# UT-Austin-RPL/FORGE

Measured on AMD Instinct MI355X. Metric: rendered views/sec (5 views, 128^2 px, 64^3 voxel), higher is better.
Workload: dtype f32; 1 GPU; BASELINE configs[1]: FORGE hot path, 1 scene(s)/GPU x 5 input views 256^2 -> 32^3x128 feature grid -> 64^3 render grid -> 5 views x 128^2 rays x 64 samples -> 5 RGB 256^2; HIP rotate, fp32-MFMA implicit-GEMM ResNet-50 trunk / conv1 / ConvGRU (Winograd F(2x2,3x3) x 3 depth taps) / heads / conv_rgb, HIP ray-march (no MIOpen/rocBLAS kernel in the step); eval BN, random-init seeded weights; scenes_per_gpu=1, views_in=5, views_out=5, feature_grid=32, render_grid=64, steps_in_flight=4, launch=hipGraph replay, 4 steps in flight on 4 HIP streams, parallelism=dp1 (scene-sharded, no data-path collective; 4-scalar RCC...

## Files before the change

### forge_amd/convops.py

```python
import collections
import ctypes
import functools
import os
from fractions import Fraction

import torch

from . import _lib, determinism

EPI_BIAS, EPI_AFFINE_ACT, EPI_GRU_GATES, EPI_GRU_OUT = 0, 1, 2, 3


_TAPS_CACHE = {}


def _taps_array(taps):
    key = tuple(tuple(t) for t in taps)
    arr = _TAPS_CACHE.get(key)
    if arr is None:
        flat = [int(v) for t in key for v in t]
        arr = _TAPS_CACHE[key] = (ctypes.c_int * len(flat))(*flat)
    return arr


# ... 23 lines not shown
    out = []
    for pz in ((0, 1) if nd == 3 else (0,)):
        for py in (0, 1):
            for px in (0, 1):
                taps, mats = [], []
                for dz, kz in (per_axis[pz] if nd == 3 else [(0, None)]):
                    for dy, ky in per_axis[py]:
                        for dx, kx in per_axis[px]:
                            taps.append((dz, dy, dx))
                            mats.append((wd[:, :, kz, ky, kx] if nd == 3 else wd[:, :, ky, kx]).t())
                out.append(((pz, py, px), taps, torch.stack(mats).contiguous()))
    return out


def convT_phases_merged(w, pad, nd):
    ph = convT_phases(w, pad, nd)
    taps = [t for _, tp, _ in ph for t in tp]
    return taps, torch.cat([wp for _, _, wp in ph], dim=0).contiguous()


def convT3d_k4s2p1_phases(w):
    return convT_phases(w, 1, 3)


def pack_conv2d_weight(w):
    co, ci, kh, kw = w.shape
    taps = [(0, ky - kh // 2, kx - kw // 2) for ky in range(kh) for kx in range(kw)]
    return w.detach().reshape(co, ci, kh * kw).permute(2, 0, 1).contiguous(), taps


def bn_affine(bn):
    scale = bn.weight.detach() / torch.sqrt(bn.running_var.detach() + bn.eps)
    shift = bn.bias.detach() - bn.running_mean.detach() * scale
    return scale.contiguous(), shift.contiguous()


class PackCache:

    def __init__(self):
        self._key = None
        self.val = None

    def clear(self):
        self._key = None
        self.val = None

    def key_of(self, sources):
        return tuple((t.data_ptr(), t._version, str(t.device)) for t in sources)

    def get(self, sources, build):
        key = self.key_of(sources)
        if key != self._key:
            self.val = build()
            self._key = key
        return self.val


class PackedModule(torch.nn.Module):

    def __init__(self):
        super().__init__()
        self.register_load_state_dict_post_hook(lambda module, incompatible_keys: module.invalidate_packed())

    def invalidate_packed(self):
        for v in self.__dict__.values():
            if isinstance(v, PackCache):
                v.clear()

    def train(self, mode=True):
        self.invalidate_packed()
        return super().train(mode)

    def _apply(self, fn, *args, **kwargs):
        self.invalidate_packed()
        return super()._apply(fn, *args, **kwargs)


def invalidate_packed(module):
    for m in module.modules():
        if isinstance(m, PackedModule):
            m.invalidate_packed()


class _ZeroArena:

    def __init__(self):
        self.task, self.device = -1, None
        self.pools = {}
        self.want = {}

    def _end(self):
        self.want = {k: p[2] for k, p in self.pools.items()}
        self.pools, self.task = {}, -1

    HAVE_HOOKS = hasattr(torch._C, "_current_graph_task_id") and hasattr(getattr(torch.autograd.Variable, "_execution_engine", None), "queue_callback")

    def zeros(self, shape, device):
        n = 1
        for d in shape:
            n *= int(d)
        nbytes = (n * 4 + 255) // 256 * 256
        if not self.HAVE_HOOKS:
            return torch.zeros(shape, dtype=torch.float32, device=device)
        task = torch._C._current_graph_task_id()
        if task < 0:
            return torch.zeros(shape, dtype=torch.float32, device=device)
        if task != self.task:
            if self.task >= 0:
                self._end()
            self.task, self.device = task, device
            torch.autograd.Variable._execution_engine.queue_callback(self._end_of(task))
        if device != self.device:
            return torch.zeros(shape, dtype=torch.float32, device=device)
        key = torch.cuda.current_stream(device).cuda_stream if torch.device(device).type == "cuda" else 0
        pool = self.pools.get(key)
        if pool is None:
            want = self.want.get(key, 0)
            pool = self.pools[key] = [torch.zeros(want // 4 + 64, dtype=torch.float32, device=device) if want else None, 0, 0]
        pool[2] += nbytes
        if pool[0] is None or pool[1] + nbytes > pool[0].numel() * 4:
            return torch.zeros(shape, dtype=torch.float32, device=device)
        out = pool[0][pool[1] // 4:pool[1] // 4 + n].view(shape)
        pool[1] += nbytes
        return out

    def _end_of(self, task):
        def cb():
            if self.task == task:
                self._end()
        return cb


GRAD_ZEROS = _ZeroArena()


def grad_zeros(shape, device, scratch=False):
    if scratch:
        return torch.zeros(tuple(shape), dtype=torch.float32, device=device)
    return GRAD_ZEROS.zeros(tuple(shape), device)


SPLITK_WS_BYTES = 128 << 20

TILE_NAMES = {"A": "128, 128, 8, 1", "B": "64, 128, 8, 1", "C": "128, 64, 8, 1", "D": "64, 64, 4, 1", "E": "128, 32, 4, 1"}

_PLAN_CACHE = {}


class _State:
    plan_override = None
    winograd = True
    wino_depth_nest = os.environ.get("FORGE_WINO_DEPTH_NEST", "1") != "0"
    wino_depth_nest4 = os.environ.get("FORGE_WINO_DEPTH_NEST4", "1") != "0"
    wino_h4 = os.environ.get("FORGE_WINO_H4", "1") != "0"
    conv_fast_epilogue = os.environ.get("FORGE_CONV_FAST_EPILOGUE", "1") != "0"


STATE = _State()


class force_plan:

    def __init__(self, tile=None, ksplit=None):
        self.val = (tile, ksplit)

    def __enter__(self):
        self.prev = STATE.plan_override
        STATE.plan_override = self.val
        return self

    def __exit__(self, *exc):
        STATE.plan_override = self.prev
        return False


_pushed_fast_epilogue = None


def _conv_lib():
    global _pushed_fast_epilogue
    L = _lib.lib()
    want = bool(STATE.conv_fast_epilogue)
    if want is not _pushed_fast_epilogue:
        L.forge_conv_fast_epilogue(int(want))
        _pushed_fast_epilogue = want
    return L


def conv_epilogue_is_direct(M, Cout, ldo, ldr=0, residual=False, ostride=1, same_grid=True, nphase=1, lift=0, ksplit=1, stats=False, epilogue=EPI_BIAS):
    fast = ctypes.c_int(0)
    _lib.check(_conv_lib().forge_conv_igemm_epilogue(int(M), int(Cout), int(ldo), int(ldr), int(bool(residual)), int(ostride), int(bool(same_grid)),
                                                     int(nphase), int(lift), int(ksplit), int(bool(stats)), int(epilogue), ctypes.byref(fast)),
               "forge_conv_igemm_epilogue")
    return bool(fast.value)


def conv_plan(M, Cout, Cin, ntaps, epilogue, ldo, nphase=1):
    key = (int(M), int(Cout), int(Cin), int(ntaps), int(nphase), int(epilogue), int(ldo) % 4 == 0)
    pl = _PLAN_CACHE.get(key)
    if pl is None:
        tile, ks = ctypes.c_int(0), ctypes.c_int(0)
        _lib.check(_lib.lib().forge_conv_igemm_plan(int(M), int(Cout), int(Cin), int(ntaps), int(nphase), int(epilogue), int(ldo), SPLITK_WS_BYTES,
                                                    ctypes.byref(tile), ctypes.byref(ks)), "forge_conv_igemm_plan")
        pl = _PLAN_CACHE[key] = (chr(tile.value), ks.value)
    ov = STATE.plan_override
    if ov is not None and pl[0] != "N":
        tile = ov[0] or pl[0]
        ks = ov[1] if ov[1] is not None else (pl[1] if ov[0] is None else 1)
        can_split = nphase == 1 and epilogue in (EPI_BIAS, EPI_AFFINE_ACT) and Cout % 4 == 0 and ldo % 4 == 0
        if ks > 1 and not (can_split and ks * M * Cout * 4 <= SPLITK_WS_BYTES and ks <= (ntaps // nphase) * (Cin // 32)):
            ks = 1
        return tile, ks
    return pl


MAX_OPERAND_BYTES = (1 << 31) - 1


@_lib.on_tensor_device
def conv_igemm(in1, C1, ld1, in2, C2, ld2, wp, bias, scale, shift, slope, residual, aux_h, aux_z, out, out2,
               grid, in_grid, Cout, ldo, taps, out_grid=None, istride=1, ostride=1, phase=(0, 0, 0), epilogue=EPI_BIAS,
               bs1=0, bs2=0, lift=0, out3=None, stats=None):
    n, D, H, W = grid
    Di, Hi, Wi = in_grid
    Do, Ho, Wo = out_grid if out_grid is not None else (D, H, W)
    if wp.shape != (len(taps), Cout, C1 + C2):
        raise ValueError("packed weight %s does not match taps=%d Cout=%d Cin=%d" % (tuple(wp.shape), len(taps), Cout, C1 + C2))
    in_rows, out_rows = Di * Hi * Wi, Do * Ho * Wo
    b1, b2 = (int(bs1) or in_rows), (int(bs2) or in_rows)
    span = lambda k, br, ld: ((k - 1) * br + in_rows) * ld * 4
    limit = MAX_OPERAND_BYTES
    nc = n
    while nc > 1 and (span(nc, b1, ld1) > limit or (in2 is not None and span(nc, b2, ld2) > limit)):
        nc = (nc + 1) // 2
    L, st, arr = _conv_lib(), _lib.current_stream(), _taps_array(taps)
    nphase = 1
    if tuple(phase) == (-1, -1, -1):
        nphase = 8 if Do == 2 * D else 4

    def off(t, floats):
        return None if t is None else ctypes.c_void_p(t.data_ptr() + 4 * floats)
    gate_w = Cout // 2 if epilogue == EPI_GRU_GATES else Cout
    for s0 in range(0, n, nc):
        k = min(nc, n - s0)
        orow = s0 * out_rows
        tile, ksplit = conv_plan(k * D * H * W, Cout, C1 + C2, len(taps), epilogue, ldo, nphase)
        if stats is not None and (ksplit > 1 or nc < n):
            raise RuntimeError("forge_amd: conv_igemm output statistics need an un-chunked launch without split-K (use conv_stats_buffer)")
        ws = torch.empty(ksplit * k * D * H * W * Cout, dtype=torch.float32, device=out.device) if ksplit > 1 else None
        o_ld = gate_w if epilogue == EPI_GRU_GATES else ldo
        _lib.check(L.forge_conv_igemm(
            off(in1, s0 * b1 * ld1), C1, ld1, int(bs1), off(in2, s0 * b2 * ld2), C2, ld2, int(bs2), _lib.ptr(wp), _lib.ptr(bias), _lib.ptr(scale),
            _lib.ptr(shift), float(slope), off(residual, orow * (Cout if (lift or epilogue in (EPI_GRU_GATES, EPI_GRU_OUT)) else ldo)),
            off(aux_h, orow * gate_w), off(aux_z, orow * Cout),
            off(out, orow * (Cout if lift else o_ld)), off(out2, orow * o_ld), off(out3, orow * o_ld), k, D, H, W, istride, Di, Hi, Wi, Cout, ldo,
            arr, len(taps), ostride, phase[0], phase[1], phase[2], Do, Ho, Wo, epilogue, int(lift), 0 if tile == "N" else ord(tile), ksplit,
            _lib.ptr(ws), 0 if ws is None else ws.numel() * 4, _lib.ptr(stats), st),
            "forge_conv_igemm")
    return out


TILE_BM = {"A": 128, "B": 64, "C": 128, "D": 64, "E": 128}


def stats_blocks(M, tile):
    bm = TILE_BM[tile]
    return ((int(M) + bm - 1) // bm) * (bm // 32)


def conv_stats_buffer(x1, in2, grid, in_grid, Cout, Cin, ntaps, ldo, device):
    n, D, H, W = grid
    M = n * D * H * W
    if Cout <= 16 or Cout % 4:
        return None
    tile, ksplit = conv_plan(M, Cout, Cin, ntaps, EPI_BIAS, ldo, 1)
    if ksplit > 1 or tile == "N":
        return None
    Di, Hi, Wi = in_grid
    if ((n - 1) * (Di * Hi * Wi) + Di * Hi * Wi) * max(x1.shape[-1], 0 if in2 is None else in2.shape[-1]) * 4 > MAX_OPERAND_BYTES:
        return None
    return torch.empty(stats_blocks(M, tile), 2, Cout, dtype=torch.float64, device=device)


def wino_pack_packed(wp, transpose=False):
    return wino_pack(WINO_FORMS["points"], wp, transpose)


def wino_pack_weight(w):
    return wino_pack_packed(pack_conv3d_weight(w))


def wino_conv_rows(x1, x2, U, bias, out, residual=None, V1=None):
    n, D, H, W, C1 = x1.shape
    return _wino_conv(x1, C1, _batch_stride_rows(x1), x2, 0 if x2 is None else x2.shape[-1], 0 if x2 is None else _batch_stride_rows(x2), U, bias, out,
                      residual, (n, D, H, W), V1=V1)


def _wino_conv(x1, C1, bs1, x2, C2, bs2, U, bias, out, residual, grid, V1=None):
    n, D, H, W = grid
    Cout = U.shape[2]
    if V1 is None:
        V1 = wino_input(x1, C1, C1, n, D, H, W, bs=bs1)
    V2 = None if x2 is None else wino_input(x2, C2, C2, n, D, H, W, bs=bs2)
    Mm = wino_gemm(V1, C1, V2, C2, U, None, n, D, H // 2, W // 2, Cout)
    return wino_output(Mm, bias, None, None, 1.0, residual, None, None, out, None, None, n, D, H, W, Cout, Cout, EPI_BIAS)


_ONE_ZERO = {}


def _one_zero(device, C):
    key = (str(device), C)
    v = _ONE_ZERO.get(key)
    if v is None:
        v = _ONE_ZERO[key] = (torch.ones(C, device=device), torch.zeros(C, device=device))
    return v


def conv3_launch(x1, C1, x2, C2, wp, bias, out, grid, Cout, bs1=0, residual=None, dgrad=False, U=None, wT=None):
    n, D, H, W = grid
    if wino_applies(TAPS_3x3x3, 1, n, D, H, W, C1, C2, Cout):
        return _wino_conv(x1, C1, bs1, x2, C2, 0, U if U is not None else wino_pack_packed(wp, transpose=dgrad), bias, out, residual, grid)
    w = (wT if wT is not None else wp.transpose(1, 2).contiguous()) if dgrad else wp
    taps = [(-a, -b, -c) for a, b, c in TAPS_3x3x3] if dgrad else TAPS_3x3x3
    if residual is None:
        return conv_igemm(x1, C1, C1, x2, C2, C2, w, bias, None, None, 1.0, None, None, None, out, None, grid, (D, H, W), Cout, Cout, taps,
                          epilogue=EPI_BIAS, bs1=bs1)
    one, zero = _one_zero(out.device, Cout)
    return conv_igemm(x1, C1, C1, x2, C2, C2, w, bias, one, zero, 1.0, residual, None, None, out, None, grid, (D, H, W), Cout, Cout, taps,
                      epilogue=EPI_AFFINE_ACT, bs1=bs1)


def wino_wgrad_applies(n, D, H, W, C1, C2, Cout, taps=None):
    return (wino_applies(TAPS_3x3x3 if taps is None else taps, 1, n, D, H, W, C1, C2, Cout) and C1 + C2 >= 128 and Cout >= 64 and (C2 == 0 or C1 % 128 == 0)
            and n * D * (H // 2) * (W // 2) * Cout * 4 <= MAX_OPERAND_BYTES)


@_lib.on_tensor_device
def conv3_wgrad(dy, x1, C1, x2, C2, dwp, grid, Cout, bs1=0, taps=None, dM=None):
    n, D, H, W = grid
    taps = TAPS_3x3x3 if taps is None else list(taps)
    if not wino_wgrad_applies(n, D, H, W, C1, C2, Cout, taps):
        return conv_wgrad(dy, x1, C1, x2, C2, dwp, grid, (D, H, W), Cout, taps, bs1=bs1)
    kd = len(taps) // 9
    L, st = _lib.lib(), _lib.current_stream()
    Ht, Wt = H // 2, W // 2
    R = n * D * Ht * Wt
    dev = dy.device
    V1 = wino_input(x1, C1, C1, n, D, H, W, bs=bs1)
    V2 = None if x2 is None else wino_input(x2, C2, C2, n, D, H, W)
    if dM is None:
        dM = torch.empty(16, R, Cout, dtype=torch.float32, device=dev)
        _lib.check(L.forge_wino_dy(_lib.ptr(dy), dy.shape[-1], _lib.ptr(dM), n, D, H, W, Cout, st), "forge_wino_dy")
    dU = grad_zeros((16, kd, Cout, C1 + C2), dev, scratch=True)
    determinism.launch("forge_wino_wgrad", (_lib.ptr(dM), _lib.ptr(V1), C1, 0, 0, _lib.ptr(V2), C2, 0, 0, _lib.ptr(dU), n, D, Ht, Wt, Cout, kd),
                       (C1, C2, n, D, Ht, Wt, Cout, kd), dev)
    _lib.check(L.forge_wino_dw(_lib.ptr(dU), _lib.ptr(dwp), Cout, C1 + C2, kd, st), "forge_wino_dw")
    return dwp


def wino_applies(taps, istride, n, D, H, W, C1, C2, Cout):
    tt = tuple(tuple(t) for t in taps)
    if not (wino_enabled() and istride == 1 and C1 % 32 == 0 and C2 % 32 == 0 and Cout % 8 == 0 and wino_fits(n, D, H, W, max(C1, C2, 1))):
        return False
    if len(tt) == 27 and tt == tuple(TAPS_3x3x3):
        return C1 + C2 >= 64 and Cout >= 32
    if len(tt) == 9 and tt == tuple(TAPS_3x3) and D == 1:
        return C2 == 0 and C1 >= WINO2D_MIN_C and Cout >= WINO2D_MIN_C
    return False


def wino_enabled():
    return STATE.winograd


class winograd:

    def __init__(self, on):
        self.on = bool(on)

    def __enter__(self):
        self.prev = STATE.winograd
        STATE.winograd = self.on
        return self

    def __exit__(self, *exc):
        STATE.winograd = self.prev
        return False


def wino_scene_chunk(b, D, H, W, C, views=1):
    nb = b
    while nb >= 1 and not wino_fits(nb, D, H, W, C, views=views):
        nb = (nb + 1) // 2 if nb > 1 else 0
    return nb


def wino_fits(n, D, H, W, C, views=1, nest4=False, form=None):
    form = form or WINO_FORMS["dn4" if nest4 else "points"]
    rows = n * views * D * (H // form.th) * (W // 2) * form.rows
    return H % form.th == 0 and W % 2 == 0 and rows * C * 4 <= MAX_OPERAND_BYTES


@_lib.on_tensor_device
def wino_input_dy(dy, C, n, D, H, W):
    R = n * D * (H // 2) * (W // 2)
    V = torch.empty(16, R, C, dtype=torch.float32, device=dy.device)
    dM = torch.empty(16, R, C, dtype=torch.float32, device=dy.device)
    _lib.check(_lib.lib().forge_wino_input_dy(_lib.ptr(dy), C, _lib.ptr(V), _lib.ptr(dM), n, D, H, W, C, _lib.current_stream()), "forge_wino_input_dy")
    return V, dM


def wino_half_applies(R, Cout, Cin):
    return STATE.plan_override is None and wino_gemm_tile(R, Cout, Cin) == "B"


def wino_depth_nest_applies(R, D, Ht, Wt, Cout, Cin):
    return (STATE.wino_depth_nest and STATE.plan_override is None and D % 2 == 0 and (Ht * Wt) % 64 == 0 and Cin % 32 == 0
            and R * Cout * 4 <= MAX_OPERAND_BYTES and wino_gemm_tile(R, Cout, Cin) == "B")


def wino_depth_nest4_applies(R, D, Ht, Wt, Cout, Cin):
    return STATE.wino_depth_nest4 and D % 4 == 0 and D >= 8 and wino_depth_nest_applies(R, D, Ht, Wt, Cout, Cin)


def wino_depth_nest4h_applies(R, D, Ht, Wt, Cout, Cin):
    return STATE.wino_h4 and wino_depth_nest4_applies(R, D, Ht, Wt, Cout, Cin)


WinoForm = collections.namedtuple("WinoForm", "name P gemm weights ushape input rows kloops applies tile metered points th", defaults=(16, 2))
_U4 = lambda kd, co_, ci_: (16, kd, co_, ci_)
WINO_FORMS = {f.name: f for f in (
    WinoForm("points", 16, "forge_wino_gemm", "forge_wino_weights", _U4, "forge_wino_input", 1, None, lambda R, D, Ht, Wt, Cout, Cin: True,
             True, True),
    WinoForm("half", 8, "forge_wino_gemm_half", "forge_wino_weights", _U4, "forge_wino_input", 1, None,
             lambda R, D, Ht, Wt, Cout, Cin: wino_half_applies(R, Cout, Cin), False, True),
    WinoForm("dn", 16, "forge_wino_gemm_dn", "forge_wino_weights_dn", lambda kd, co_, ci_: (16, 2, 2, co_, ci_), "forge_wino_input", 1, 2,
             lambda *a: wino_depth_nest_applies(*a), False, True),
    WinoForm("dn4", 16, "forge_wino_gemm_dn4", "forge_wino_weights_dn4", lambda kd, co_, ci_: (16, 6, co_, ci_), "forge_wino_input_dn4", Fraction(3, 2),
             Fraction(3, 2), lambda *a: wino_depth_nest4_applies(*a), False, False),
)}

WINO_DN4H = WinoForm("dn4h", 24, "forge_wino_gemm_dn4h", "forge_wino_weights_dn4h", lambda kd, co_, ci_: (24, 6, co_, ci_), "forge_wino_input_dn4h",
                     Fraction(3, 2), Fraction(3, 2), lambda *a: wino_depth_nest4h_applies(*a), False, False, 24, 4)


def wino_calls(form):
    if not form.metered:
        return functools.partial(wino_form_input, form), functools.partial(wino_form_gemm, form)
    return (lambda *a, **kw: wino_input(*a, **kw)), (lambda *a, **kw: wino_gemm(*a, **kw))


@_lib.on_tensor_device
def wino_pack(form, wp, transpose=False):
    T, co_, ci_ = wp.shape
    nest = form.kloops is not None
    assert T == 27 or (T == 9 and not nest)
    assert not (nest and transpose)
    kd = T // 9
    wp = wp.detach()
    wp = wp if wp.is_contiguous() else wp.contiguous()
    U = torch.empty(form.ushape(kd, ci_, co_) if transpose else form.ushape(kd, co_, ci_), dtype=torch.float32, device=wp.device)
    own = () if nest else (kd, 1 if transpose else 0)
    _lib.check(getattr(_lib.lib(), form.weights)(_lib.ptr(wp), _lib.ptr(U), co_, ci_, *own, _lib.current_stream()), form.weights)
    return U


@_lib.on_tensor_device
def wino_form_input(form, x, C, ld, n, D, H, W, bs=0, out=None, nsum=1, sum_stride=0):
    rows = int(n * D * (H // form.th) * (W // 2) * form.rows)
    V = out if out is not None else torch.empty(form.points, rows, C, dtype=torch.float32, device=x.device)
    if form.rows != 1 and (V.shape != (form.points, rows, C) or not V.is_contiguous()):
        raise ValueError("depth-nest operand buffer %s is not [%d][%d][%d]" % (tuple(V.shape), form.points, rows, C))
    _lib.check(getattr(_lib.lib(), form.input)(_lib.ptr(x), ld, int(bs), _lib.ptr(V), C, 0, n, D, H, W, C, int(nsum), int(sum_stride), _lib.current_stream()),
               form.input)
    return V


def wino_input(x, C, ld, n, D, H, W, bs=0, out=None, nsum=1, sum_stride=0):
    return wino_form_input(WINO_FORMS["points"], x, C, ld, n, D, H, W, bs=bs, out=out, nsum=nsum, sum_stride=sum_stride)


def _point_products(Mm, P, R, Cout, device):
    if Mm is None:
        Mm = torch.empty(P, R, Cout, dtype=torch.float32, device=device)
    if not (Mm.is_contiguous() and Mm.dtype == torch.float32 and Mm.numel() >= P * R * Cout):
        raise ValueError("point-product buffer %s %s%s cannot hold %d x %d x %d float32" % (
            tuple(Mm.shape), Mm.dtype, "" if Mm.is_contiguous() else " (not contiguous)", P, R, Cout))
    if Mm.shape != (P, R, Cout):
        Mm = Mm.as_strided((P, R, Cout), (R * Cout, Cout, 1))
    return Mm


@_lib.on_tensor_device
def wino_form_gemm(form, V1, C1, V2, C2, U, Mm, n, D, Ht, Wt, Cout, view=0, views=1):
    R = n * D * Ht * Wt
    vol = int(D * Ht * Wt * form.rows)
    nest = form.kloops is not None
    kd = 3 if nest else U.shape[1]
    if U.shape != form.ushape(kd, Cout, C1 + C2) or (kd not in (1, 3)) or (nest and not U.is_contiguous()):
        raise ValueError("%s weight %s does not match Cout=%d Cin=%d" % ("depth-nest" if nest else "transformed", tuple(U.shape), Cout, C1 + C2))
    if form.rows != 1 and (V1.shape[1] != n * views * vol or (V2 is not None and V2.shape[1] != n * vol)):
        raise ValueError("depth-nest operands %s / %s are not %s's %d (x %d views) rows per point" % (
            tuple(V1.shape), None if V2 is None else tuple(V2.shape), form.input, n * vol, views))
    Mm = _point_products(Mm, form.P, R, Cout, V1.device)
    tile = (ord(wino_gemm_tile(R, Cout, C1 + C2)),) if form.tile else ()
    p1 = ctypes.c_void_p(V1.data_ptr() + 4 * view * vol * C1)
    _lib.check(getattr(_conv_lib(), form.gemm)(p1, C1, C1, views * vol if views > 1 else 0, V1.shape[1] * C1, _lib.ptr(V2), C2, C2, 0,
                                               0 if V2 is None else V2.shape[1] * C2, _lib.ptr(U), _lib.ptr(Mm), n, D, Ht, Wt, Cout, kd,
                                               *tile, _lib.current_stream()), form.gemm)
    return Mm


def wino_gemm(V1, C1, V2, C2, U, Mm, n, D, Ht, Wt, Cout, view=0, views=1, half=None):
    if U.dim() == 5:
        form = "dn"
    else:
        if half is None:
            half = WINO_FORMS["half"].applies(n * D * Ht * Wt, D, Ht, Wt, Cout, C1 + C2)
        form = "half" if half else "points"
    return wino_form_gemm(WINO_FORMS[form], V1, C1, V2, C2, U, Mm, n, D, Ht, Wt, Cout, view=view, views=views)


def wino_gemm_tile(R, Cout, Cin):
    ov = STATE.plan_override
    if ov is not None and ov[0]:
        return ov[0]
    return chr(_lib.lib().forge_wino_gemm_tile(int(R), int(Cout), int(Cin)))


@_lib.on_tensor_device
def wino_output(Mm, bias, scale, shift, slope, residual, aux_h, aux_z, out, out2, out3, n, D, H, W, Cout, ldo, epilogue, Mm2=None, view=0, views=1):
    P = Mm.shape[0] if Mm.dim() == 3 else 0
    vol = D * (H // (WINO_DN4H.th if P == WINO_DN4H.P else 2)) * (W // 2)
    if P not in (8, 16, WINO_DN4H.P) or Mm.shape[1:] != (n * vol, Cout) or not Mm.is_contiguous():
        raise ValueError("point products %s do not match [8 | 16][%d][%d] (or the 24 points' rows)" % (tuple(Mm.shape), n * vol, Cout))
    if P == WINO_DN4H.P:
        if Mm2 is not None or residual is not None or H % 4 or epilogue not in (EPI_GRU_GATES, EPI_GRU_OUT):
            raise ValueError("24-point products take the GRU tails only, without a second addend or a residual, on H %% 4 == 0 (H=%d epilogue=%d)" % (H, epilogue))
        _lib.check(_lib.lib().forge_wino_output_dn4h(_lib.ptr(Mm), _lib.ptr(bias), _lib.ptr(scale), _lib.ptr(shift), _lib.ptr(aux_h), _lib.ptr(aux_z),
                                                     _lib.ptr(out), _lib.ptr(out2), _lib.ptr(out3), n, D, H, W, Cout, ldo, epilogue, _lib.current_stream()),
                   "forge_wino_output_dn4h")
        return out
    if Mm2 is not None and (Mm2.shape != (P, n * views * vol, Cout) or not Mm2.is_contiguous()):
        raise ValueError("second addend %s does not match [%d][%d][%d] (the form of Mm)" % (tuple(Mm2.shape), P, n * views * vol, Cout))
    p2 = None if Mm2 is None else ctypes.c_void_p(Mm2.data_ptr() + 4 * view * vol * Cout)
    fn, name = (_lib.lib().forge_wino_output_half, "forge_wino_output_half") if P == 8 else (_lib.lib().forge_wino_output, "forge_wino_output")
    _lib.check(fn(_lib.ptr(Mm), p2, views * vol, 0 if Mm2 is None else Mm2.shape[1] * Cout, _lib.ptr(bias), _lib.ptr(scale), _lib.ptr(shift), float(slope),
                  _lib.ptr(residual), _lib.ptr(aux_h), _lib.ptr(aux_z), _lib.ptr(out), _lib.ptr(out2), _lib.ptr(out3), n, D, H, W, Cout, ldo, epilogue,
                  _lib.current_stream()), name)
    return out


@_lib.on_tensor_device
def conv_wgrad(dy, x1, C1, x2, C2, dwp, grid, in_grid, Cout, taps, istride=1, bs1=0, bs2=0):
    if x2 is not None and C1 % 128:
        x1 = torch.cat([x1[..., :C1], x2[..., :C2]], dim=-1)
        C1, x2, C2, bs1, bs2 = C1 + C2, None, 0, 0, 0
    n, D, H, W = grid
    Di, Hi, Wi = in_grid
    in_rows, out_rows = Di * Hi * Wi, D * H * W
    ldy, ld1, ld2 = dy.shape[-1], x1.shape[-1], (0 if x2 is None else x2.shape[-1])
    b1, b2 = (int(bs1) or in_rows), (int(bs2) or in_rows)
    span = lambda k, br, ld, rows: ((k - 1) * br + rows) * ld * 4
    nc = n
    while nc > 1 and (span(nc, out_rows, ldy, out_rows) > MAX_OPERAND_BYTES or span(nc, b1, ld1, in_rows) > MAX_OPERAND_BYTES
                      or (x2 is not None and span(nc, b2, ld2, in_rows) > MAX_OPERAND_BYTES)):
        nc = (nc + 1) // 2
    off = lambda t, floats: None if t is None else ctypes.c_void_p(t.data_ptr() + 4 * floats)
    ta = _taps_array(taps)
    for s0 in range(0, n, nc):
        k = min(nc, n - s0)
        determinism.launch("forge_conv_wgrad", (off(dy, s0 * out_rows * ldy), ldy, off(x1, s0 * b1 * ld1), C1, ld1, int(bs1), off(x2, s0 * b2 * ld2), C2, ld2,
                                                int(bs2), _lib.ptr(dwp), k, D, H, W, istride, Di, Hi, Wi, Cout, ta, len(taps)),
                           (C1, C2, k, D, H, W, istride, Di, Hi, Wi, Cout, ta, len(taps)), dwp.device)
    return dwp


def _batch_stride_rows(x):
    n, D, H, W, C = x.shape
    if x.stride()[1:] != (H * W * C, W * C, C, 1):
        raise ValueError("conv_rows needs channels-last rows [n,D,H,W,C] dense within a batch element; got strides %s" % (x.stride(),))
    return 0 if (n == 1 or x.stride(0) == D * H * W * C) else x.stride(0) // C


@_lib.on_tensor_device
def colsum(x):
    C = x.shape[-1]
    rows = x.reshape(-1, C)
    if not (rows.is_cuda and rows.dtype == torch.float32):
        raise RuntimeError("forge_amd: colsum runs only on the MI355X HIP kernels (float32 cuda tensor); got %s on %s" % (rows.dtype, rows.device))
    if C % 4:
        if C > 32:
            raise RuntimeError("forge_amd: colsum needs C %% 4 == 0 or C <= 32 (got %d)" % C)
        rows = rows if rows.is_contiguous() else rows.contiguous()
    else:
        rows = rows if (rows.stride(1) == 1 and rows.stride(0) >= C and rows.stride(0) % 4 == 0) else rows.contiguous()
    out = torch.empty(C, dtype=torch.float32, device=rows.device)
    ws = torch.empty(_lib.lib().forge_bn_ws_doubles(C), dtype=torch.float64, device=rows.device)
    _lib.check(_lib.lib().forge_colsum(_lib.ptr(rows), rows.stride(0), _lib.ptr(out), _lib.ptr(ws), rows.shape[0], C, _lib.current_stream()), "forge_colsum")
    return out


class _ConvTapsRows(torch.autograd.Function):

    @staticmethod
    def forward(ctx, x1, x2, wp, bias, taps, istride, out_spatial, want_stats=False):
        n, Di, Hi, Wi, C1 = x1.shape
        C2 = 0 if x2 is None else x2.shape[-1]
        T, Cout, Cin = wp.shape
        D, H, W = out_spatial
        wpc = wp.detach().contiguous()
        out = torch.empty(n, D, H, W, Cout, dtype=torch.float32, device=x1.device)
        bs1 = _batch_stride_rows(x1)
        bs2 = 0 if x2 is None else _batch_stride_rows(x2)
        stats = None
        if (D, H, W) == (Di, Hi, Wi) and wino_applies(taps, istride, n, D, H, W, C1, C2, Cout):
            wino_conv_rows(x1, x2, wino_pack_packed(wpc), bias, out)
        else:
            if want_stats and bs1 == 0 and bs2 == 0:
                stats = conv_stats_buffer(x1, x2, (n, D, H, W), (Di, Hi, Wi), Cout, Cin, T, Cout, x1.device)
            conv_igemm(x1, C1, C1, x2, C2, C2, wpc, bias, None, None, 1.0, None, None, None, out, None,
                       (n, D, H, W), (Di, Hi, Wi), Cout, Cout, taps, istride=istride, epilogue=EPI_BIAS, bs1=bs1, bs2=bs2, stats=stats)
        ctx.save_for_backward(x1, x2, wpc)
        ctx.meta = (tuple(taps), istride, (D, H, W), bias is not None)
        if not want_stats:
            return out
        if stats is None:
            stats = torch.empty(0, dtype=torch.float64, device=x1.device)
        ctx.mark_non_differentiable(stats)
        return out, stats

    @staticmethod
    def backward(ctx, dy, _dstats=None):
        x1, x2, wp = ctx.saved_tensors
        taps, istride, (D, H, W), has_bias = ctx.meta
        n, Di, Hi, Wi, C1 = x1.shape
        C2 = 0 if x2 is None else x2.shape[-1]
        T, Cout, Cin = wp.shape
        dy = dy.contiguous()
        dx1 = dx2 = dwp = db = None
        need_dx = ctx.needs_input_grad[0] or ctx.needs_input_grad[1]
        same = (D, H, W) == (Di, Hi, Wi)
        wino_dx = need_dx and istride == 1 and Cout > 16 and same and wino_applies(taps, istride, n, D, H, W, Cout, 0, Cin)
        wino_dw = (ctx.needs_input_grad[2] and same and wino_applies(taps, istride, n, D, H, W, C1, C2, Cout)
                   and (x2 is None or _batch_stride_rows(x2) == 0) and wino_wgrad_applies(n, D, H, W, C1, C2, Cout, taps))
        Vdy = dMdy = None
        if wino_dx and wino_dw:
            Vdy, dMdy = wino_input_dy(dy.reshape(-1, Cout), Cout, n, D, H, W)
        if need_dx:
            wd = wp.transpose(1, 2).contiguous()
            if istride == 1 and Cout <= 16:
                assert (D, H, W) == (Di, Hi, Wi)
                if Cout < 16:
                    dyk = torch.nn.functional.pad(dy, (0, 16 - Cout))
                    wd = torch.nn.functional.pad(wd, (0, 16 - Cout))
                else:
                    dyk = dy
                dx = torch.empty(n, Di, Hi, Wi, Cin, dtype=torch.float32, device=dy.device)
                ntaps_ = [(-a, -b, -c) for a, b, c in taps]
                for j in range(0, Cin, 16):
                    nb = min(16, Cin - j)
                    conv_igemm(dyk, 16, 16, None, 0, 0, wd[:, j:j + nb].contiguous(), None, None, None, 1.0, None, None, None, dx[..., j:], None,
                               (n, D, H, W), (D, H, W), nb, Cin, ntaps_, epilogue=EPI_BIAS)
            elif istride == 1 and (D, H, W) == (Di, Hi, Wi) and wino_applies(taps, istride, n, D, H, W, Cout, 0, Cin):
                dx = torch.empty(n, Di, Hi, Wi, Cin, dtype=torch.float32, device=dy.device)
                wino_conv_rows(dy, None, wino_pack_packed(wp, transpose=True), None, dx, V1=Vdy)
            elif istride == 1:
                assert (D, H, W) == (Di, Hi, Wi)
                dx = torch.empty(n, Di, Hi, Wi, Cin, dtype=torch.float32, device=dy.device)
                conv_igemm(dy, Cout, Cout, None, 0, 0, wd, None, None, None, 1.0, None, None, None, dx, None, (n, D, H, W), (D, H, W), Cin, Cin,
                           [(-a, -b, -c) for a, b, c in taps], epilogue=EPI_BIAS)
            else:
                flat = D == 1 and Di == 1 and all(t[0] == 0 for t in taps)
                assert istride == 2 and Hi == 2 * H and Wi == 2 * W and (flat or Di == 2 * D), (istride, (D, H, W), (Di, Hi, Wi))
                dx = torch.zeros(n, Di, Hi, Wi, Cin, dtype=torch.float32, device=dy.device)
                for ph_z in ((0,) if flat else (0, 1)):
                    for ph_y in (0, 1):
                        for ph_x in (0, 1):
                            sel = [i for i, (tz, ty, tx) in enumerate(taps) if (flat or (tz - ph_z) % 2 == 0) and (ty - ph_y) % 2 == 0 and (tx - ph_x) % 2 == 0]
                            if not sel:
                                continue
                            ptaps = [(0 if flat else (ph_z - taps[i][0]) // 2, (ph_y - taps[i][1]) // 2, (ph_x - taps[i][2]) // 2) for i in sel]
                            conv_igemm(dy, Cout, Cout, None, 0, 0, torch.stack([wd[i] for i in sel]), None, None, None, 1.0, None, None, None, dx, None,
                                       (n, D, H, W), (D, H, W), Cin, Cin, ptaps, out_grid=(Di, Hi, Wi), ostride=2, phase=(ph_z, ph_y, ph_x),
                                       epilogue=EPI_BIAS)
            dx1 = dx[..., :C1] if ctx.needs_input_grad[0] else None
            dx2 = dx[..., C1:] if (x2 is not None and ctx.needs_input_grad[1]) else None
        if ctx.needs_input_grad[2]:
            dwp = grad_zeros(wp.shape, wp.device)
            if (D, H, W) == (Di, Hi, Wi) and wino_applies(taps, istride, n, D, H, W, C1, C2, Cout) and (x2 is None or _batch_stride_rows(x2) == 0):
                conv3_wgrad(dy, x1, C1, x2, C2, dwp, (n, D, H, W), Cout, bs1=_batch_stride_rows(x1), taps=taps, dM=dMdy)
            else:
                conv_wgrad(dy, x1, C1, x2, C2, dwp, (n, D, H, W), (Di, Hi, Wi), Cout, list(taps), istride=istride, bs1=_batch_stride_rows(x1),
                           bs2=0 if x2 is None else _batch_stride_rows(x2))
# ... 239 lines not shown
```

### forge_amd/csrc/conv_igemm.hip

```cpp
#include "common.h"
#include <cmath>
#include <type_traits>

namespace forge {

enum ConvEpilogue : int {
    EPI_BIAS = 0,
    EPI_AFFINE_ACT = 1,
    EPI_GRU_GATES = 2,
    EPI_GRU_OUT = 3,
};

constexpr int MAX_TAPS = 64;

struct ConvArgs {
    const float* in1; const float* in2;
    int C1, C2, ld1, ld2;
    long long bs1r, bs2r;
    long long span1, span2;
    const float* wp;
    const float* bias;
    const float* scale; const float* shift; float slope;
    const float* aux_h; const float* aux_z;
    float* out; float* out2; float* out3;
// ... 1064 lines not shown
        hipLaunchKernelGGL((conv_igemm_kernel<BMv, BNv, NWv>), dim3((unsigned)grid), dim3(NWv * 64), lds, st, a);          \
    } while (0)
    switch (tile) {
        case 'A': FORGE_LAUNCH_CONV(128, 128, 8); break;
        case 'B': FORGE_LAUNCH_CONV(64, 128, 8); break;
        case 'C': FORGE_LAUNCH_CONV(128, 64, 8); break;
        case 'E': FORGE_LAUNCH_CONV(128, 32, 4); break;
        default: FORGE_LAUNCH_CONV(64, 64, 4); break;
    }
#undef FORGE_LAUNCH_CONV
    return 0;
}

}

using namespace forge;

extern "C" int forge_conv_igemm_plan(long long M, int Cout, int Cin, int ntaps, int nphase, int epilogue, int ldo, long long splitk_ws_bytes,
                                     int* tile, int* ksplit) {
    FORGE_REQUIRE(tile && ksplit && M > 0 && Cout > 0 && Cin > 0 && ntaps > 0 && (nphase == 1 || nphase == 4 || nphase == 8) && ntaps % nphase == 0,
                  FORGE_EINVAL, "forge_conv_igemm_plan: bad argument");
    if (Cout <= 16) { *tile = 'N'; *ksplit = 1; return 0; }
    const ConvPlan pl = plan_conv(M * nphase, Cout, Cin, ntaps / nphase,
                                  nphase == 1 && splitk_ws_bytes > 0 && (epilogue == EPI_BIAS || epilogue == EPI_AFFINE_ACT) && Cout % 4 == 0 && ldo % 4 == 0,
                                  splitk_ws_bytes);
    *tile = pl.tile; *ksplit = pl.ksplit;
    return 0;
}

extern "C" int forge_conv_fast_epilogue(int on) {
    const int prev = g_conv_fast_epilogue;
    if (on >= 0) g_conv_fast_epilogue = on != 0;
    return prev;
}

extern "C" int forge_conv_igemm_epilogue(long long M, int Cout, int ldo, int ldr, int has_residual, int os, int same_grid, int nphase, int lift, int ksplit,
                                         int has_stats, int epilogue, int* fast) {
    FORGE_REQUIRE(fast && M > 0 && Cout > 0 && ldo > 0 && os >= 1 && nphase >= 1 && lift >= 0 && ksplit >= 1 && epilogue >= 0 && epilogue <= 3, FORGE_EINVAL,
                  "forge_conv_igemm_epilogue: bad argument");
    *fast = Cout > 16 && g_conv_fast_epilogue &&
            conv_fast_epilogue_applies(M, Cout, ldo, ldr, has_residual != 0, os, same_grid != 0, nphase, lift, ksplit, has_stats != 0, epilogue);
    return 0;
}

extern "C" int forge_conv_igemm(const float* in1, int C1, int ld1, long long bs1, const float* in2, int C2, int ld2, long long bs2,
                                const float* wp,
                                const float* bias, const float* scale, const float* shift, float slope, const float* residual,
                                const float* aux_h, const float* aux_z, float* out, float* out2, float* out3,
                                int n, int D, int H, int W, int is, int Di, int Hi, int Wi, int Cout, int ldo,
                                const int* taps, int ntaps, int os, int pz, int py, int px, int Do, int Ho, int Wo,
                                int epilogue, int lift, int tile, int ksplit, float* splitk_ws, long long splitk_ws_bytes, double* stats,
                                forge_stream_t stream) {
    FORGE_REQUIRE(in1 && wp && out && taps, FORGE_EINVAL, "forge_conv_igemm: null pointer argument");
    FORGE_REQUIRE(stats == nullptr || (epilogue == EPI_BIAS && ksplit <= 1 && Cout > 16 && !(pz < 0) && lift == 0), FORGE_EINVAL,
                  "forge_conv_igemm: output statistics need the plain bias epilogue of the wide kernel without split-K, phases or lift");
    FORGE_REQUIRE(n > 0 && D > 0 && H > 0 && W > 0 && Cout > 0 && ntaps > 0 && ntaps <= MAX_TAPS, FORGE_EINVAL,
                  "forge_conv_igemm: bad dims n=%d D=%d H=%d W=%d Cout=%d ntaps=%d", n, D, H, W, Cout, ntaps);
    const int kstep = Cout <= 16 ? 16 : 32;
    FORGE_REQUIRE(C1 > 0 && C1 % kstep == 0 && C2 >= 0 && C2 % kstep == 0, FORGE_ESHAPE,
                  "forge_conv_igemm: C1=%d / C2=%d must be multiples of the K-step %d (16 for Cout <= 16, else 32)", C1, C2, kstep);
    FORGE_REQUIRE((C2 == 0) == (in2 == nullptr), FORGE_EINVAL, "forge_conv_igemm: in2/C2 mismatch");
    FORGE_REQUIRE(epilogue >= 0 && epilogue <= 3, FORGE_EINVAL, "forge_conv_igemm: unknown epilogue %d", epilogue);
    FORGE_REQUIRE(epilogue != EPI_AFFINE_ACT || (scale && shift), FORGE_EINVAL, "forge_conv_igemm: affine epilogue needs scale/shift");
    FORGE_REQUIRE(epilogue != EPI_GRU_GATES || (aux_h && out2 && Cout % 2 == 0), FORGE_EINVAL, "forge_conv_igemm: GRU gate epilogue needs aux_h, out2");
    FORGE_REQUIRE(epilogue != EPI_GRU_OUT || (aux_h && aux_z), FORGE_EINVAL, "forge_conv_igemm: GRU out epilogue needs aux_h, aux_z");
    FORGE_REQUIRE(os >= 1 && Do > 0 && Ho > 0 && Wo > 0, FORGE_EINVAL, "forge_conv_igemm: bad output mapping");
    FORGE_REQUIRE(is >= 1 && Di > 0 && Hi > 0 && Wi > 0, FORGE_EINVAL, "forge_conv_igemm: bad input mapping");
    FORGE_REQUIRE(lift == 0 || (lift > 0 && epilogue == EPI_AFFINE_ACT && Cout % lift == 0 && D == 1 && os == 1 && Cout > 64), FORGE_EINVAL,
                  "forge_conv_igemm: lift needs the affine epilogue on a 2-D (D=1) conv with Cout %% lift == 0 and Cout > 64");
    FORGE_REQUIRE(ld1 >= C1 && ld1 % 4 == 0 && (C2 == 0 || (ld2 >= C2 && ld2 % 4 == 0)) && ldo >= 1, FORGE_EINVAL,
                  "forge_conv_igemm: row strides must cover the channels and keep 16-byte alignment");
    ConvArgs a;
    a.in1 = in1; a.in2 = in2; a.C1 = C1; a.C2 = C2; a.ld1 = ld1; a.ld2 = ld2;
    a.bs1r = bs1 > 0 ? bs1 : (long long)Di * Hi * Wi; a.bs2r = bs2 > 0 ? bs2 : (long long)Di * Hi * Wi;
    a.span1 = ((long long)(n - 1) * a.bs1r + (long long)Di * Hi * Wi) * ld1 * 4;
    a.span2 = in2 ? ((long long)(n - 1) * a.bs2r + (long long)Di * Hi * Wi) * ld2 * 4 : 0;
    FORGE_REQUIRE(a.span1 < (1ll << 31) && a.span2 < (1ll << 31) && (long long)ntaps * Cout * (C1 + C2) * 4 < (1ll << 31), FORGE_ESHAPE,
                  "forge_conv_igemm: an operand spans >= 2 GiB (32-bit buffer offsets); split the batch");
    a.is = is; a.Di = Di; a.Hi = Hi; a.Wi = Wi; a.residual = residual;
    a.ldr = (lift > 0 || epilogue == EPI_GRU_GATES || epilogue == EPI_GRU_OUT) ? Cout : ldo;
    a.lift = lift; a.ws = nullptr; a.ksplit = 1; a.stats = stats; a.flat_rows = a.fast_epi = 0;
    a.wp = wp; a.bias = bias; a.scale = scale; a.shift = shift; a.slope = slope;
    a.aux_h = aux_h; a.aux_z = aux_z; a.out = out; a.out2 = out2; a.out3 = out3; a.n = n; a.D = D; a.H = H; a.W = W; a.Cout = Cout; a.ldo = ldo;
    a.ntaps = ntaps; a.os = os; a.pz = pz; a.py = py; a.px = px; a.Do = Do; a.Ho = Ho; a.Wo = Wo; a.epi = epilogue;
    a.nphase = 1; a.tpp = ntaps; a.nbat = 1; a.pt1 = a.pt2 = a.ptw = a.pto = 0;
    if (pz < 0) {
        FORGE_REQUIRE(os == 2 && py < 0 && px < 0 && Ho == 2 * H && Wo == 2 * W && (Do == 2 * D || Do == D), FORGE_EINVAL,
                      "forge_conv_igemm: merged phases (pz = py = px = -1) need os = 2 and a doubled output grid");
        a.nphase = Do == 2 * D ? 8 : 4;
        FORGE_REQUIRE(ntaps % a.nphase == 0, FORGE_EINVAL, "forge_conv_igemm: merged phases need ntaps %% %d == 0", a.nphase);
        a.tpp = ntaps / a.nphase;
        a.pz = a.py = a.px = 0;
    }
    for (int k = 0; k < 3 * ntaps; ++k)
        FORGE_REQUIRE(taps[k] >= -128 && taps[k] <= 127, FORGE_EINVAL, "forge_conv_igemm: tap %d component %d = %d outside [-128, 127]", k / 3, k % 3, taps[k]);
    for (int t = 0; t < MAX_TAPS; ++t) {
        for (int k = 0; k < 3; ++k) a.tap[t][k] = (signed char)(t < ntaps ? taps[t * 3 + k] : 0);
        a.tap[t][3] = 0;
    }
    const long long M = (long long)n * D * H * W;
    FORGE_REQUIRE(M < (1ll << 31), FORGE_ESHAPE, "forge_conv_igemm: more than 2^31 GEMM rows; split the batch");
    FORGE_REQUIRE(out3 == nullptr || epilogue == EPI_GRU_GATES || epilogue == EPI_GRU_OUT, FORGE_EINVAL, "forge_conv_igemm: out3 is a GRU-epilogue output");
    hipStream_t st = (hipStream_t)stream;
    if (Cout <= 16) {
        FORGE_REQUIRE(epilogue == EPI_BIAS || epilogue == EPI_AFFINE_ACT, FORGE_EINVAL, "forge_conv_igemm: GRU epilogues need Cout > 16");
        const long long grid = (M + BM16 - 1) / BM16 * a.nphase;
        FORGE_REQUIRE(grid < (1ll << 31), FORGE_ESHAPE, "forge_conv_igemm: grid too large");
        int lines_r = 0;
        if (a.nphase == 1 && is == 1 && os == 1 && lift == 0 && Do == D && Ho == H && Wo == W && Di == D && Hi == H && Wi == W && pz == 0 && py == 0 && px == 0) {
            for (int r = 1; r <= 2 && !lines_r; ++r) {
                const int nt = 2 * r + 1;
                bool ok = ntaps % nt == 0 && W > r;
                for (int t = 0; ok && t < ntaps; ++t)
                    ok = taps[t * 3 + 2] == (t % nt) - r && taps[t * 3] == taps[(t - t % nt) * 3] && taps[t * 3 + 1] == taps[(t - t % nt) * 3 + 1];
                if (ok) lines_r = r;
            }
        }
        if (lines_r == 1) hipLaunchKernelGGL(conv_igemm_n16_lines_kernel<1>, dim3((unsigned)grid), dim3(NTHREADS), 0, st, a);
        else if (lines_r == 2) hipLaunchKernelGGL(conv_igemm_n16_lines_kernel<2>, dim3((unsigned)grid), dim3(NTHREADS), 0, st, a);
        else hipLaunchKernelGGL(conv_igemm_n16_kernel, dim3((unsigned)grid), dim3(NTHREADS), 0, st, a);
    } else {
        const bool can_split = a.nphase == 1 && splitk_ws && (epilogue == EPI_BIAS || epilogue == EPI_AFFINE_ACT) && Cout % 4 == 0 && ldo % 4 == 0;
        ConvPlan pl;
        if (tile == 0) {
            pl = plan_conv(M * a.nphase, Cout, C1 + C2, a.tpp, can_split, splitk_ws_bytes);
        } else {
            pl = ConvPlan{(char)tile, ksplit > 1 ? ksplit : 1};
            FORGE_REQUIRE(tile >= 'A' && tile <= 'E', FORGE_EINVAL, "forge_conv_igemm: tile '%c' is not one of A..E (0 = planned here)", (char)tile);
            FORGE_REQUIRE(pl.ksplit == 1 || (can_split && pl.ksplit <= 8 && (long long)pl.ksplit * M * Cout * 4 <= splitk_ws_bytes &&
                                             pl.ksplit <= a.tpp * ((C1 + C2) / BK)), FORGE_EINVAL,
                          "forge_conv_igemm: ksplit=%d needs epilogue 0/1 without phases, Cout, ldo %% 4 == 0 and a workspace of ksplit M Cout floats", pl.ksplit);
        }
        FORGE_REQUIRE(stats == nullptr || (tile != 0 && pl.ksplit == 1), FORGE_EINVAL,
                      "forge_conv_igemm: output statistics need an explicit tile ('A'..'E' from forge_conv_igemm_plan) and a plan without split-K");
        if (pl.ksplit > 1) { a.ksplit = pl.ksplit; a.ws = splitk_ws; }
        if (int rc = launch_conv_tile(a, pl.tile, st)) return rc;
        if (a.ksplit > 1) {
            const long long total = M * (Cout / 4);
            hipLaunchKernelGGL(conv_splitk_epilogue_kernel, dim3((unsigned)((total + 255) / 256)), dim3(256), 0, st, a);
        }
    }
    FORGE_LAUNCH_CHECK("forge_conv_igemm");
    return 0;
}

extern "C" int forge_wino_gemm_tile(long long R, int Cout, int Cin) {
    (void)Cin;
    if (Cout <= 64) return R < 2048 ? 'D' : 'C';
    return R < 2048 ? 'D' : 'B';
}

static int wino_gemm_impl(const float* V1, int C1, int ld1, long long bs1, long long pt1, const float* V2, int C2, int ld2, long long bs2,
                          long long pt2, const float* U, float* Mm, int n, int D, int Ht, int Wt, int Cout, int kd, int tile, int form, forge_stream_t stream) {
    const bool half = form == 1, dn = form == 2, dn4h = form == 4, dn4 = form == 3 || dn4h;
    const char* const name4 = dn4h ? "forge_wino_gemm_dn4h" : "forge_wino_gemm_dn4";
    FORGE_REQUIRE(tile == 0 || (tile >= 'A' && tile <= 'E'), FORGE_EINVAL, "forge_wino_gemm: tile must be 0 (default rule) or 'A'..'E'");
    FORGE_REQUIRE(V1 && U && Mm && (kd == 1 || kd == 3), FORGE_EINVAL, "forge_wino_gemm: null pointer argument / kd not 1 or 3");
    FORGE_REQUIRE(n > 0 && D > 0 && Ht > 0 && Wt > 0 && Cout > 16, FORGE_EINVAL, "forge_wino_gemm: bad dims n=%d D=%d Ht=%d Wt=%d Cout=%d (Cout > 16)", n,
                  D, Ht, Wt, Cout);
    FORGE_REQUIRE(C1 > 0 && C1 % BK == 0 && C2 >= 0 && C2 % BK == 0 && (C2 == 0) == (V2 == nullptr), FORGE_ESHAPE,
                  "forge_wino_gemm: C1=%d / C2=%d must be multiples of %d, V2 given iff C2 > 0", C1, C2, BK);
    FORGE_REQUIRE(ld1 >= C1 && ld1 % 4 == 0 && (C2 == 0 || (ld2 >= C2 && ld2 % 4 == 0)), FORGE_EINVAL, "forge_wino_gemm: bad row strides");
    FORGE_REQUIRE(!dn || (kd == 3 && D % 2 == 0 && ((long long)Ht * Wt) % 64 == 0), FORGE_EINVAL,
                  "forge_wino_gemm_dn: needs three depth taps, an even D and Ht Wt %% 64 == 0 (kd=%d D=%d Ht=%d Wt=%d)", kd, D, Ht, Wt);
    FORGE_REQUIRE(!dn4 || (kd == 3 && D % 4 == 0 && ((long long)Ht * Wt) % 64 == 0), FORGE_EINVAL,
                  "%s: needs three depth taps, D %% 4 == 0 and Ht Wt %% 64 == 0 (kd=%d D=%d Ht=%d Wt=%d)", name4, kd, D, Ht, Wt);
    FORGE_REQUIRE(!dn4h || D >= 8, FORGE_EINVAL, "forge_wino_gemm_dn4h: D=%d must be at least 8", D);
    ConvArgs a;
    memset(&a, 0, sizeof(a));
    const long long vol = (long long)D * Ht * Wt, R = (long long)n * vol, rows = dn4 ? vol / 4 * 6 : vol, Cin = C1 + C2;
    const int npos = dn4 ? 6 : dn ? 4 : kd;
    a.in1 = V1; a.in2 = V2; a.C1 = C1; a.C2 = C2; a.ld1 = ld1; a.ld2 = ld2; a.bs1r = bs1 > 0 ? bs1 : rows; a.bs2r = bs2 > 0 ? bs2 : rows;
    a.span1 = ((long long)(n - 1) * a.bs1r + rows) * ld1 * 4;
    a.span2 = V2 ? ((long long)(n - 1) * a.bs2r + rows) * ld2 * 4 : 0;
    if (dn4) {
        FORGE_REQUIRE(a.span1 < (1ll << 31) && a.span2 < (1ll << 31) && R * Cout * 4 < (1ll << 31) && 6ll * Cout * Cin * 4 < (1ll << 31), FORGE_EINVAL,
                      "%s: an operand or an output plane spans >= 2 GiB (32-bit buffer offsets); split the batch", name4);
    } else {
        FORGE_REQUIRE(a.span1 < (1ll << 31) && a.span2 < (1ll << 31) && R < (1ll << 31), FORGE_ESHAPE,
                      "forge_wino_gemm: an operand spans >= 2 GiB per Winograd point (32-bit buffer offsets); split the batch");
        FORGE_REQUIRE(!dn || (R * Cout * 4 < (1ll << 31) && 4ll * Cout * Cin * 4 < (1ll << 31)), FORGE_ESHAPE,
                      "forge_wino_gemm_dn: an output plane spans >= 2 GiB (32-bit buffer offsets); split the batch");
    }
    a.wp = U; a.slope = 1.f; a.out = Mm; a.n = n; a.D = D; a.H = Ht; a.W = Wt; a.is = 1; a.Di = D; a.Hi = Ht; a.Wi = Wt;
    a.Cout = Cout; a.ldo = Cout; a.ldr = Cout; a.ntaps = a.tpp = npos; a.os = 1; a.Do = D; a.Ho = Ht; a.Wo = Wt; a.nphase = 1; a.epi = EPI_BIAS;
    a.ksplit = 1; a.nbat = half ? 4 : dn4h ? 24 : 16;
    a.pt1 = pt1 > 0 ? pt1 : (long long)n * rows * ld1; a.pt2 = V2 ? (pt2 > 0 ? pt2 : (long long)n * rows * ld2) : 0;
    a.ptw = (long long)npos * Cout * Cin; a.pto = R * Cout;
    if (form == 0 || half) {
        if (kd == 3) { a.tap[0][0] = -1; a.tap[2][0] = 1; }
        if (!tile) tile = forge_wino_gemm_tile(R, Cout, C1 + C2);
    }
    if (int rc = launch_conv_tile(a, (char)tile, (hipStream_t)stream, dn4h ? 3 : form)) return rc;
    FORGE_LAUNCH_CHECK(dn4 ? name4 : dn ? "forge_wino_gemm_dn" : "forge_wino_gemm");
    return 0;
}

extern "C" int forge_wino_gemm(const float* V1, int C1, int ld1, long long bs1, long long pt1, const float* V2, int C2, int ld2, long long bs2,
                               long long pt2, const float* U, float* Mm, int n, int D, int Ht, int Wt, int Cout, int kd, int tile, forge_stream_t stream) {
    return wino_gemm_impl(V1, C1, ld1, bs1, pt1, V2, C2, ld2, bs2, pt2, U, Mm, n, D, Ht, Wt, Cout, kd, tile, 0, stream);
}

extern "C" int forge_wino_gemm_half(const float* V1, int C1, int ld1, long long bs1, long long pt1, const float* V2, int C2, int ld2, long long bs2,
                                    long long pt2, const float* U, float* Mm8, int n, int D, int Ht, int Wt, int Cout, int kd, forge_stream_t stream) {
    return wino_gemm_impl(V1, C1, ld1, bs1, pt1, V2, C2, ld2, bs2, pt2, U, Mm8, n, D, Ht, Wt, Cout, kd, 'B', 1, stream);
}

extern "C" int forge_wino_gemm_dn(const float* V1, int C1, int ld1, long long bs1, long long pt1, const float* V2, int C2, int ld2, long long bs2,
                                  long long pt2, const float* Ud, float* Mm, int n, int D, int Ht, int Wt, int Cout, int kd, forge_stream_t stream) {
    FORGE_REQUIRE(C1 > 0 && C1 % BK == 0 && C2 >= 0 && C2 % BK == 0, FORGE_EINVAL, "forge_wino_gemm_dn: C1=%d / C2=%d must be multiples of %d", C1, C2, BK);
    return wino_gemm_impl(V1, C1, ld1, bs1, pt1, V2, C2, ld2, bs2, pt2, Ud, Mm, n, D, Ht, Wt, Cout, kd, 'B', 2, stream);
}

extern "C" int forge_wino_gemm_dn4(const float* V1, int C1, int ld1, long long bs1, long long pt1, const float* V2, int C2, int ld2, long long bs2,
                                   long long pt2, const float* Ud, float* Mm, int n, int D, int Ht, int Wt, int Cout, int kd, forge_stream_t stream) {
    FORGE_REQUIRE(C1 > 0 && C1 % BK == 0 && C2 >= 0 && C2 % BK == 0, FORGE_EINVAL, "forge_wino_gemm_dn4: C1=%d / C2=%d must be multiples of %d", C1, C2, BK);
    return wino_gemm_impl(V1, C1, ld1, bs1, pt1, V2, C2, ld2, bs2, pt2, Ud, Mm, n, D, Ht, Wt, Cout, kd, 'B', 3, stream);
}

extern "C" int forge_wino_gemm_dn4h(const float* V1, int C1, int ld1, long long bs1, long long pt1, const float* V2, int C2, int ld2, long long bs2,
                                    long long pt2, const float* Ud, float* Mm, int n, int D, int Ht, int Wt, int Cout, int kd, forge_stream_t stream) {
    FORGE_REQUIRE(C1 > 0 && C1 % BK == 0 && C2 >= 0 && C2 % BK == 0, FORGE_EINVAL, "forge_wino_gemm_dn4h: C1=%d / C2=%d must be multiples of %d", C1, C2, BK);
    return wino_gemm_impl(V1, C1, ld1, bs1, pt1, V2, C2, ld2, bs2, pt2, Ud, Mm, n, D, Ht, Wt, Cout, kd, 'B', 4, stream);
}
```

### forge_amd/csrc/winograd.hip

```cpp
#include "common.h"

namespace forge {

__device__ __forceinline__ float4 add(float4 a, float4 b) { return make_float4(a.x + b.x, a.y + b.y, a.z + b.z, a.w + b.w); }
__device__ __forceinline__ float4 sub(float4 a, float4 b) { return make_float4(a.x - b.x, a.y - b.y, a.z - b.z, a.w - b.w); }
__device__ __forceinline__ float add(float a, float b) { return a + b; }
__device__ __forceinline__ float sub(float a, float b) { return a - b; }
__device__ __forceinline__ float4 fma4(float k, float4 a, float4 b) { return make_float4(fmaf(k, a.x, b.x), fmaf(k, a.y, b.y), fmaf(k, a.z, b.z), fmaf(k, a.w, b.w)); }

__device__ __forceinline__ void f43_six_lines(float p0, float p1, float p2, float p3, float p4, float p5, float& q0, float& q1, float& q2, float& q3, float& q4,
                                              float& q5) {
    const float a02 = p0 - p2, a24 = p2 - p4, s34 = p3 + p4, s12 = p1 + p2, d43 = p4 - p3, d12 = p1 - p2;
    const float d42 = p4 - p2, d31 = p3 - p1, d13 = p1 - p3, d35 = p3 - p5;
    q0 = fmaf(4.f, a02, -a24);
    q1 = fmaf(-4.f, s12, s34);
    q2 = fmaf(4.f, d12, d43);
    q3 = fmaf(2.f, d31, d42);
    q4 = fmaf(-2.f, d31, d42);
    q5 = fmaf(4.f, d13, -d35);
}

__device__ __forceinline__ void tile_decode(long long idx, int per, int cs, int Ht, int Wt, unsigned& r, int& c, int& tw, int& th, unsigned& t) {
    r = (unsigned)(idx / per);
    c = (int)(idx - (long long)r * per) << cs;
    unsigned q = r;
    t = q / (unsigned)Wt;
    tw = (int)(q - t * (unsigned)Wt); q = t; t = q / (unsigned)Ht;
    th = (int)(q - t * (unsigned)Ht);
}

template <typename T>
__device__ __forceinline__ void bt_cols_store(const T (&w)[4], float* vp, int i, long long ptv) {
    *reinterpret_cast<T*>(vp + (4 * i + 0) * ptv) = sub(w[0], w[2]);
    *reinterpret_cast<T*>(vp + (4 * i + 1) * ptv) = add(w[1], w[2]);
    *reinterpret_cast<T*>(vp + (4 * i + 2) * ptv) = sub(w[2], w[1]);
    *reinterpret_cast<T*>(vp + (4 * i + 3) * ptv) = sub(w[1], w[3]);
}

template <typename T, typename I>
__device__ __forceinline__ void bt_d_b_store(const T (&d)[4][4], float* V, I row, int ld, int c, long long ptv) {
    T w[4][4];
#pragma unroll
    for (int j = 0; j < 4; ++j) {
        w[0][j] = sub(d[0][j], d[2][j]);
        w[1][j] = add(d[1][j], d[2][j]);
        w[2][j] = sub(d[2][j], d[1][j]);
        w[3][j] = sub(d[1][j], d[3][j]);
    }
    float* vp = V + (long long)row * ld + c;
#pragma unroll
    for (int i = 0; i < 4; ++i) bt_cols_store(w[i], vp, i, ptv);
}

__device__ __forceinline__ void a_y_at_store(float4 y00, float4 y01, float4 y10, float4 y11, float* mp, long long ptm) {
    const float4 zero = make_float4(0.f, 0.f, 0.f, 0.f);
    const float4 s[4][2] = {{y00, y01}, {add(y00, y10), add(y01, y11)}, {sub(y00, y10), sub(y01, y11)}, {sub(zero, y10), sub(zero, y11)}};
#pragma unroll
    for (int i = 0; i < 4; ++i) {
        *reinterpret_cast<float4*>(mp + (4 * i + 0) * ptm) = s[i][0];
        *reinterpret_cast<float4*>(mp + (4 * i + 1) * ptm) = add(s[i][0], s[i][1]);
        *reinterpret_cast<float4*>(mp + (4 * i + 2) * ptm) = sub(s[i][0], s[i][1]);
        *reinterpret_cast<float4*>(mp + (4 * i + 3) * ptm) = sub(zero, s[i][1]);
    }
}

__device__ __forceinline__ double depth_row_f23(int k, double w0, double w1, double w2) {
    return k == 0 ? w0 : k == 1 ? 0.5 * (w0 + w1 + w2) : k == 2 ? 0.5 * (w0 - w1 + w2) : w2;
}
__device__ __forceinline__ double depth_row_f43(int k, double w0, double w1, double w2) {
    return k == 0 ? 0.25 * w0 : k == 1 ? -((w0 + w2) + w1) / 6.0 : k == 2 ? -((w0 + w2) - w1) / 6.0
         : k == 3 ? ((0.25 * w0 + w2) + 0.5 * w1) / 6.0 : k == 4 ? ((0.25 * w0 + w2) - 0.5 * w1) / 6.0 : w2;
}

template <int NH = 4, double (*HROW)(int, double, double, double) = depth_row_f23>
__device__ __forceinline__ void g_d_gt_store(const double (&d)[3][3], float* up, long long pt) {
    double g[NH][3];
#pragma unroll
    for (int b = 0; b < 3; ++b)
#pragma unroll
        for (int i = 0; i < NH; ++i) g[i][b] = HROW(i, d[0][b], d[1][b], d[2][b]);
#pragma unroll
    for (int i = 0; i < NH; ++i) {
        up[(4 * i + 0) * pt] = (float)g[i][0];
        up[(4 * i + 1) * pt] = (float)(0.5 * (g[i][0] + g[i][1] + g[i][2]));
        up[(4 * i + 2) * pt] = (float)(0.5 * (g[i][0] - g[i][1] + g[i][2]));
        up[(4 * i + 3) * pt] = (float)g[i][2];
    }
}

struct WinoInArgs {
    const float* in; int ld; long long bs;
    float* V; int ldv; long long ptv;
    int n, D, H, W, C;
    int nsum; long long ss;
    float* dM; long long ptm;
};

template <bool DY>
__global__ __launch_bounds__(256) void wino_input_kernel(const WinoInArgs a) {
    const int C4 = a.C >> 2, Ht = a.H >> 1, Wt = a.W >> 1;
    const long long idx = (long long)xcd_remap(blockIdx.x, gridDim.x) * 256 + threadIdx.x;
    const long long R = (long long)a.n * a.D * Ht * Wt;
    if (idx >= R * C4) return;
    unsigned r, t;
    int c, tw, th;
    tile_decode(idx, C4, 2, Ht, Wt, r, c, tw, th, t);
    const unsigned q = t; t = q / (unsigned)a.D;
    const int z = (int)(q - t * (unsigned)a.D);
    const float* base = a.in + ((long long)t * a.bs + (long long)z * a.H * a.W) * a.ld + c;
    float4 d[4][4];
#pragma unroll
    for (int i = 0; i < 4; ++i) {
        const int y = 2 * th - 1 + i;
#pragma unroll
        for (int j = 0; j < 4; ++j) {
            const int x = 2 * tw - 1 + j;
            const bool ok = (unsigned)y < (unsigned)a.H && (unsigned)x < (unsigned)a.W;
            float4 v = make_float4(0.f, 0.f, 0.f, 0.f);
            if (ok) {
                const float* p = base + ((long long)y * a.W + x) * a.ld;
                v = *reinterpret_cast<const float4*>(p);
                if (a.nsum > 1) {
                    for (int k = 1; k < a.nsum; ++k) v = add(v, *reinterpret_cast<const float4*>(p + (long long)k * a.ss * a.ld));
                    const float inv = 1.f / (float)a.nsum;
                    v = make_float4(v.x * inv, v.y * inv, v.z * inv, v.w * inv);
                }
            }
            d[i][j] = v;
        }
    }
    if constexpr (DY) a_y_at_store(d[1][1], d[1][2], d[2][1], d[2][2], a.dM + (long long)r * a.C + c, a.ptm);
    bt_d_b_store(d, a.V, r, a.ldv, c, a.ptv);
}

template <int TH>
__global__ __launch_bounds__(256) void wino_input_dn4_kernel(const WinoInArgs a) {
    constexpr int NR = TH + 2;
    const int Ht = TH == 4 ? a.H >> 2 : a.H >> 1, Wt = a.W >> 1, Dg = a.D >> 2;
    const long long idx = (long long)xcd_remap(blockIdx.x, gridDim.x) * 256 + threadIdx.x;
    const long long RG = (long long)a.n * Dg * Ht * Wt;
    if (idx >= RG * a.C) return;
    unsigned r, t;
    int c, tw, th;
    tile_decode(idx, a.C, 0, Ht, Wt, r, c, tw, th, t);
    const unsigned q = t; t = q / (unsigned)Dg;
    const int g = (int)(q - t * (unsigned)Dg);
    const long long HW = (long long)a.H * a.W;
    const float* base = a.in + (long long)t * a.bs * a.ld + c;
    const float inv = 1.f / (float)a.nsum;
    float d[6][NR][4];
#pragma unroll
    for (int i = 0; i < NR; ++i) {
        const int y = TH * th - 1 + i;
#pragma unroll
        for (int j = 0; j < 4; ++j) {
            const int x = 2 * tw - 1 + j;
            const bool ok = (unsigned)y < (unsigned)a.H && (unsigned)x < (unsigned)a.W;
            float p[6];
#pragma unroll
            for (int e = 0; e < 6; ++e) {
                const int z = 4 * g - 1 + e;
                float v = 0.f;
                if (ok && (unsigned)z < (unsigned)a.D) {
                    const float* s = base + ((long long)z * HW + (long long)y * a.W + x) * a.ld;
                    v = *s;
                    if (a.nsum > 1) {
                        for (int k = 1; k < a.nsum; ++k) v += s[(long long)k * a.ss * a.ld];
                        v *= inv;
                    }
                }
                p[e] = v;
            }
            f43_six_lines(p[0], p[1], p[2], p[3], p[4], p[5], d[0][i][j], d[1][i][j], d[2][i][j], d[3][i][j], d[4][i][j], d[5][i][j]);
        }
    }
    const long long HWt = (long long)Ht * Wt;
    float* vp = a.V + ((((long long)t * Dg + g) * 6) * HWt + (long long)th * Wt + tw) * a.ldv + c;
    if constexpr (TH == 4) {
#pragma unroll
        for (int k = 0; k < 6; ++k) {
#pragma unroll
            for (int j = 0; j < 4; ++j)
                f43_six_lines(d[k][0][j], d[k][1][j], d[k][2][j], d[k][3][j], d[k][4][j], d[k][5][j], d[k][0][j], d[k][1][j], d[k][2][j], d[k][3][j], d[k][4][j], d[k][5][j]);
#pragma unroll
            for (int i = 0; i < 6; ++i) bt_cols_store(d[k][i], vp + k * HWt * a.ldv, i, a.ptv);
        }
    } else {
#pragma unroll
        for (int k = 0; k < 6; ++k) bt_d_b_store(d[k], vp, k * HWt, a.ldv, 0, a.ptv);
    }
}

__global__ __launch_bounds__(256) void wino_weight_kernel(const float* __restrict__ wp, float* __restrict__ U, int Cout, int Cin, int KD, int transpose) {
    const int No = transpose ? Cin : Cout, Nc = transpose ? Cout : Cin;
    const long long idx = (long long)blockIdx.x * 256 + threadIdx.x, per = (long long)No * Nc;
    if (idx >= KD * per) return;
    const int kd = (int)(idx / per);
    const long long oc = idx - kd * per;
    const int o = (int)(oc / Nc), c = (int)(oc - (long long)o * Nc);
    double w[3][3];
#pragma unroll
    for (int a = 0; a < 3; ++a)
#pragma unroll
        for (int b = 0; b < 3; ++b) {
            const int tap = transpose ? ((KD - 1 - kd) * 3 + (2 - a)) * 3 + (2 - b) : (kd * 3 + a) * 3 + b;
            w[a][b] = (double)wp[((long long)tap * Cout + (transpose ? c : o)) * Cin + (transpose ? o : c)];
        }
    g_d_gt_store(w, U + ((long long)kd * No + o) * Nc + c, KD * per);
}

template <int K, double (*ROW)(int, double, double, double), int NH = 4, double (*HROW)(int, double, double, double) = depth_row_f23>
__global__ __launch_bounds__(256) void wino_weight_nest_kernel(const float* __restrict__ wp, float* __restrict__ U, int Cout, int Cin) {
    const long long idx = (long long)blockIdx.x * 256 + threadIdx.x, per = (long long)Cout * Cin;
    if (idx >= per) return;
    double w[3][3][3];
#pragma unroll
    for (int t = 0; t < 27; ++t) w[t / 9][(t / 3) % 3][t % 3] = (double)wp[t * per + idx];
#pragma unroll
    for (int k = 0; k < K; ++k) {
        double d[3][3];
#pragma unroll
        for (int a = 0; a < 3; ++a)
#pragma unroll
            for (int b = 0; b < 3; ++b) d[a][b] = ROW(k, w[0][a][b], w[1][a][b], w[2][a][b]);
        g_d_gt_store<NH, HROW>(d, U + k * per + idx, K * per);
    }
}

enum WinoEpilogue : int { W_BIAS = 0, W_AFFINE_ACT = 1, W_GRU_GATES = 2, W_GRU_OUT = 3 };

struct WinoOutArgs {
    const float* Mm; long long ptm;
    const float* Mm2; long long ptm2, bs2;
    const float* bias; const float* scale; const float* shift; float slope;
    const float* residual;
    const float* aux_h; const float* aux_z;
    float* out; float* out2; float* out3; int ldo;
    int n, D, H, W, Cout, epi;
};

template <int ROWS>
__device__ __forceinline__ void load_planes(float4 (&m)[ROWS][4], const float* Mm, long long ptm, const float* Mm2, long long ptm2, long long bs2, int Cout, unsigned R1, unsigned r, int c) {
    const float* mp = Mm + (long long)r * Cout + c;
#pragma unroll
    for (int i = 0; i < ROWS; ++i)
#pragma unroll
        for (int j = 0; j < 4; ++j) m[i][j] = *reinterpret_cast<const float4*>(mp + (4 * i + j) * ptm);
    if (Mm2) {
        const unsigned nn = r / R1;
        const float* mp2 = Mm2 + ((long long)nn * bs2 + (r - nn * R1)) * Cout + c;
#pragma unroll
        for (int i = 0; i < ROWS; ++i)
#pragma unroll
            for (int j = 0; j < 4; ++j) m[i][j] = add(m[i][j], *reinterpret_cast<const float4*>(mp2 + (4 * i + j) * ptm2));
    }
}

template <int EPI, bool HALF = false, int TH = 2>
__global__ __launch_bounds__(256) void wino_output_kernel(const WinoOutArgs a) {
    static_assert(TH == 2 || (TH == 4 && !HALF), "tiles of 2 x 2 voxels, or of 4 x 2 from the 24 points");
    const int C4 = a.Cout >> 2, Ht = TH == 4 ? a.H >> 2 : a.H >> 1, Wt = a.W >> 1;
    const long long idx = (long long)blockIdx.x * 256 + threadIdx.x;
    const long long R = (long long)a.n * a.D * Ht * Wt;
    if (idx >= R * C4) return;
    unsigned r, t;
    int c, tw, th;
    tile_decode(idx, C4, 2, Ht, Wt, r, c, tw, th, t);
    float4 s[TH][4];
    if constexpr (TH == 4) {
        const float* mp = a.Mm + (long long)r * a.Cout + c;
#pragma unroll
        for (int j = 0; j < 4; ++j) {
            float4 m[6];
#pragma unroll
            for (int i = 0; i < 6; ++i) m[i] = *reinterpret_cast<const float4*>(mp + (4 * i + j) * a.ptm);
            const float4 sl = add(m[1], m[2]), dl = sub(m[1], m[2]), Sl = add(m[3], m[4]), Dl = sub(m[3], m[4]);
            s[0][j] = add(add(sl, Sl), m[0]);
            s[1][j] = fma4(2.f, Dl, dl);
            s[2][j] = fma4(4.f, Sl, sl);
            s[3][j] = add(fma4(8.f, Dl, dl), m[5]);
        }
    } else if constexpr (HALF) {
        load_planes<2>(s, a.Mm, a.ptm, a.Mm2, a.ptm2, a.bs2, a.Cout, (unsigned)(a.D * Ht * Wt), r, c);
    } else {
        float4 m[4][4];
        load_planes<4>(m, a.Mm, a.ptm, a.Mm2, a.ptm2, a.bs2, a.Cout, (unsigned)(a.D * Ht * Wt), r, c);
#pragma unroll
        for (int j = 0; j < 4; ++j) {
            s[0][j] = add(add(m[0][j], m[1][j]), m[2][j]);
            s[1][j] = sub(sub(m[1][j], m[2][j]), m[3][j]);
        }
    }
    float4 y[TH][2];
#pragma unroll
    for (int i = 0; i < TH; ++i) {
        y[i][0] = add(add(s[i][0], s[i][1]), s[i][2]);
        y[i][1] = sub(sub(s[i][1], s[i][2]), s[i][3]);
    }
    float4 bias = make_float4(0.f, 0.f, 0.f, 0.f), sc = make_float4(1.f, 1.f, 1.f, 1.f), sh = bias;
    if (a.bias) bias = *reinterpret_cast<const float4*>(a.bias + c);
    if ((EPI == W_AFFINE_ACT || (EPI == W_GRU_OUT && a.out2)) && a.scale) {
        sc = *reinterpret_cast<const float4*>(a.scale + c);
        sh = *reinterpret_cast<const float4*>(a.shift + c);
    }
    const int Ch = a.Cout >> 1;
    const long long plane = (long long)t * a.H * a.W;
#pragma unroll
    for (int i = 0; i < TH; ++i)
#pragma unroll
        for (int j = 0; j < 2; ++j) {
            const long long orow = plane + (long long)(TH * th + i) * a.W + (2 * tw + j);
            float v[4] = {y[i][j].x + bias.x, y[i][j].y + bias.y, y[i][j].z + bias.z, y[i][j].w + bias.w};
            if (a.residual) {
                const float4 rr = *reinterpret_cast<const float4*>(a.residual + orow * a.Cout + c);
                v[0] += rr.x; v[1] += rr.y; v[2] += rr.z; v[3] += rr.w;
            }
            const float scv[4] = {sc.x, sc.y, sc.z, sc.w}, shv[4] = {sh.x, sh.y, sh.z, sh.w};
            if constexpr (EPI == W_BIAS) {
                *reinterpret_cast<float4*>(a.out + orow * a.ldo + c) = make_float4(v[0], v[1], v[2], v[3]);
            } else if constexpr (EPI == W_AFFINE_ACT) {
#pragma unroll
                for (int k = 0; k < 4; ++k) {
                    const float u = fmaf(v[k], scv[k], shv[k]);
                    v[k] = u > 0.f ? u : u * a.slope;
                }
                *reinterpret_cast<float4*>(a.out + orow * a.ldo + c) = make_float4(v[0], v[1], v[2], v[3]);
            } else if constexpr (EPI == W_GRU_GATES) {
                float g[4];
#pragma unroll
                for (int k = 0; k < 4; ++k) g[k] = 1.f / (1.f + expf(-v[k]));
                if (c < Ch) {
                    *reinterpret_cast<float4*>(a.out + orow * Ch + c) = make_float4(g[0], g[1], g[2], g[3]);
                } else {
                    const float4 h = *reinterpret_cast<const float4*>(a.aux_h + orow * Ch + (c - Ch));
                    *reinterpret_cast<float4*>(a.out2 + orow * Ch + (c - Ch)) = make_float4(h.x * g[0], h.y * g[1], h.z * g[2], h.w * g[3]);
                    if (a.out3) *reinterpret_cast<float4*>(a.out3 + orow * Ch + (c - Ch)) = make_float4(g[0], g[1], g[2], g[3]);
                }
            } else {
                const float4 z4 = *reinterpret_cast<const float4*>(a.aux_z + orow * a.Cout + c);
                const float4 h4 = *reinterpret_cast<const float4*>(a.aux_h + orow * a.Cout + c);
                const float zv[4] = {z4.x, z4.y, z4.z, z4.w}, hv[4] = {h4.x, h4.y, h4.z, h4.w};
                float cand[4], hn[4];
#pragma unroll
                for (int k = 0; k < 4; ++k) {
                    cand[k] = tanhf(v[k]);
                    hn[k] = hv[k] * (1.f - zv[k]) + cand[k] * zv[k];
                }
                *reinterpret_cast<float4*>(a.out + orow * a.ldo + c) = make_float4(hn[0], hn[1], hn[2], hn[3]);
                if (a.out2)
                    *reinterpret_cast<float4*>(a.out2 + orow * a.ldo + c) =
                        make_float4(fmaf(hn[0], scv[0], shv[0]), fmaf(hn[1], scv[1], shv[1]), fmaf(hn[2], scv[2], shv[2]), fmaf(hn[3], scv[3], shv[3]));
                if (a.out3) *reinterpret_cast<float4*>(a.out3 + orow * a.ldo + c) = make_float4(cand[0], cand[1], cand[2], cand[3]);
            }
        }
}

struct WinoDyArgs {
    const float* dy; int ldy;
    float* dM; long long ptm;
    int n, D, H, W, Cout;
};

__global__ __launch_bounds__(256) void wino_dy_kernel(const WinoDyArgs a) {
    const int C4 = a.Cout >> 2, Ht = a.H >> 1, Wt = a.W >> 1;
    const long long idx = (long long)blockIdx.x * 256 + threadIdx.x;
    const long long R = (long long)a.n * a.D * Ht * Wt;
    if (idx >= R * C4) return;
    unsigned r, t;
    int c, tw, th;
    tile_decode(idx, C4, 2, Ht, Wt, r, c, tw, th, t);
    const float* yp = a.dy + ((long long)t * a.H * a.W + (long long)(2 * th) * a.W + 2 * tw) * a.ldy + c;
    float4 y[2][2];
#pragma unroll
    for (int i = 0; i < 2; ++i)
#pragma unroll
        for (int j = 0; j < 2; ++j) y[i][j] = *reinterpret_cast<const float4*>(yp + ((long long)i * a.W + j) * a.ldy);
    a_y_at_store(y[0][0], y[0][1], y[1][0], y[1][1], a.dM + (long long)r * a.Cout + c, a.ptm);
}

__global__ __launch_bounds__(256) void wino_dw_kernel(const float* __restrict__ dU, float* __restrict__ dw, int Cout, int Cin, int KD) {
    const long long idx = (long long)blockIdx.x * 256 + threadIdx.x, per = (long long)Cout * Cin;
    if (idx >= KD * per) return;
    const int kd = (int)(idx / per);
    const long long oc = idx - kd * per;
    const long long pt = KD * per;
    float u[4][4];
#pragma unroll
    for (int i = 0; i < 4; ++i)
#pragma unroll
        for (int j = 0; j < 4; ++j) u[i][j] = dU[(4 * i + j) * pt + kd * per + oc];
    float g[3][4];
#pragma unroll
    for (int j = 0; j < 4; ++j) {
        g[0][j] = u[0][j] + 0.5f * (u[1][j] + u[2][j]);
        g[1][j] = 0.5f * (u[1][j] - u[2][j]);
        g[2][j] = 0.5f * (u[1][j] + u[2][j]) + u[3][j];
    }
#pragma unroll
    for (int a_ = 0; a_ < 3; ++a_) {
        float* o = dw + ((long long)((kd * 3 + a_) * 3) * per) + oc;
        o[0 * per] += g[a_][0] + 0.5f * (g[a_][1] + g[a_][2]);
        o[1 * per] += 0.5f * (g[a_][1] - g[a_][2]);
        o[2 * per] += 0.5f * (g[a_][1] + g[a_][2]) + g[a_][3];
    }
}

}

using namespace forge;

extern "C" int forge_wino_dy(const float* dy, int ldy, float* dM, int n, int D, int H, int W, int Cout, forge_stream_t stream) {
    FORGE_REQUIRE(dy && dM, FORGE_EINVAL, "forge_wino_dy: null pointer argument");
    FORGE_REQUIRE(n > 0 && D > 0 && H > 0 && W > 0 && H % 2 == 0 && W % 2 == 0 && Cout > 0 && Cout % 4 == 0 && ldy >= Cout && ldy % 4 == 0, FORGE_ESHAPE,
                  "forge_wino_dy: n=%d D=%d H=%d W=%d Cout=%d ldy=%d (H, W even; Cout, ldy multiples of 4)", n, D, H, W, Cout, ldy);
    WinoDyArgs a;
    const long long R = (long long)n * D * (H / 2) * (W / 2);
    a.dy = dy; a.ldy = ldy; a.dM = dM; a.ptm = R * Cout; a.n = n; a.D = D; a.H = H; a.W = W; a.Cout = Cout;
    FORGE_REQUIRE(R < (1ll << 31), FORGE_ESHAPE, "forge_wino_dy: more than 2^31 tiles; split the batch");
    const long long total = R * (Cout / 4), grid = (total + 255) / 256;
    FORGE_REQUIRE(grid < (1ll << 31), FORGE_ESHAPE, "forge_wino_dy: grid too large");
    hipLaunchKernelGGL(wino_dy_kernel, dim3((unsigned)grid), dim3(256), 0, (hipStream_t)stream, a);
    FORGE_LAUNCH_CHECK("forge_wino_dy");
    return 0;
}

extern "C" int forge_wino_dw(const float* dU, float* dw, int Cout, int Cin, int kd, forge_stream_t stream) {
    FORGE_REQUIRE(dU && dw && Cout > 0 && Cin > 0 && (kd == 1 || kd == 3), FORGE_EINVAL, "forge_wino_dw: bad argument (kd = 1 or 3)");
    const long long total = (long long)kd * Cout * Cin;
    hipLaunchKernelGGL(wino_dw_kernel, dim3((unsigned)((total + 255) / 256)), dim3(256), 0, (hipStream_t)stream, dU, dw, Cout, Cin, kd);
    FORGE_LAUNCH_CHECK("forge_wino_dw");
    return 0;
}

template <typename K, typename... A>
static int wino_weights_launch(const char* name, K kernel, long long total, forge_stream_t stream, A... args) {
    hipLaunchKernelGGL(kernel, dim3((unsigned)((total + 255) / 256)), dim3(256), 0, (hipStream_t)stream, args...);
    FORGE_LAUNCH_CHECK(name);
    return 0;
}

extern "C" int forge_wino_weights(const float* wp, float* U, int Cout, int Cin, int kd, int transpose, forge_stream_t stream) {
    FORGE_REQUIRE(wp && U && Cout > 0 && Cin > 0 && (kd == 1 || kd == 3), FORGE_EINVAL, "forge_wino_weights: bad argument (kd = 1 or 3)");
    return wino_weights_launch("forge_wino_weights", wino_weight_kernel, (long long)kd * Cout * Cin, stream, wp, U, Cout, Cin, kd, transpose);
}

extern "C" int forge_wino_weights_dn(const float* wp, float* Ud, int Cout, int Cin, forge_stream_t stream) {
    FORGE_REQUIRE(wp && Ud && Cout > 0 && Cin > 0, FORGE_EINVAL, "forge_wino_weights_dn: bad argument");
    return wino_weights_launch("forge_wino_weights_dn", wino_weight_nest_kernel<4, depth_row_f23>, (long long)Cout * Cin, stream, wp, Ud, Cout, Cin);
}

extern "C" int forge_wino_weights_dn4(const float* wp, float* Ud, int Cout, int Cin, forge_stream_t stream) {
    FORGE_REQUIRE(wp && Ud && Cout > 0 && Cin > 0, FORGE_EINVAL, "forge_wino_weights_dn4: bad argument");
    return wino_weights_launch("forge_wino_weights_dn4", wino_weight_nest_kernel<6, depth_row_f43>, (long long)Cout * Cin, stream, wp, Ud, Cout, Cin);
}

extern "C" int forge_wino_weights_dn4h(const float* wp, float* Ud, int Cout, int Cin, forge_stream_t stream) {
    FORGE_REQUIRE(wp && Ud && Cout > 0 && Cin > 0, FORGE_EINVAL, "forge_wino_weights_dn4h: bad argument");
    return wino_weights_launch("forge_wino_weights_dn4h", wino_weight_nest_kernel<6, depth_row_f43, 6, depth_row_f43>, (long long)Cout * Cin, stream, wp, Ud, Cout, Cin);
}

enum WinoInKind { IN_PLAIN, IN_DN4, IN_DY, IN_DN4H };

static int wino_input_impl(const char* name, WinoInKind kind, const float* in, int ld, long long bs, float* V, int ldv, long long ptv, float* dM, int n, int D, int H,
                           int W, int C, int nsum, long long sum_stride, forge_stream_t stream) {
    const bool dn4 = kind == IN_DN4 || kind == IN_DN4H;
    const int th = kind == IN_DN4H ? 4 : 2;
    FORGE_REQUIRE(in && V && (kind != IN_DY || dM), FORGE_EINVAL, "%s: null pointer argument", name);
    FORGE_REQUIRE(nsum >= 1 && (nsum == 1 || sum_stride > 0), FORGE_EINVAL, "%s: nsum >= 1, and a positive sum_stride (rows) with nsum > 1", name);
    FORGE_REQUIRE(!dn4 || (D > 0 && D % 4 == 0), FORGE_EINVAL, "%s: D=%d must be a multiple of 4", name, D);
    FORGE_REQUIRE(kind != IN_DN4H || (D >= 8 && H > 0 && H % 4 == 0), FORGE_EINVAL, "%s: D=%d H=%d (D >= 8; H a multiple of 4)", name, D, H);
    const bool ok = n > 0 && D > 0 && H > 0 && W > 0 && H % 2 == 0 && W % 2 == 0 && C > 0 && C % 4 == 0 && ld >= C && ld % 4 == 0 && ldv >= C && ldv % 4 == 0;
    if (kind == IN_DY)
        FORGE_REQUIRE(ok, FORGE_ESHAPE, "%s: n=%d D=%d H=%d W=%d C=%d ld=%d (H, W even; C, ld multiples of 4)", name, n, D, H, W, C, ld);
    FORGE_REQUIRE(ok, FORGE_ESHAPE, "%s: n=%d D=%d H=%d W=%d C=%d ld=%d ldv=%d (H, W even; C, ld, ldv multiples of 4)", name, n, D, H, W, C, ld, ldv);
    WinoInArgs a;
    a.in = in; a.ld = ld; a.bs = bs > 0 ? bs : (long long)D * H * W; a.V = V; a.ldv = ldv; a.n = n; a.D = D; a.H = H; a.W = W; a.C = C;
    a.nsum = nsum; a.ss = sum_stride;
    const long long R = (long long)n * (dn4 ? D / 4 : D) * (H / th) * (W / 2), rows = dn4 ? 6 * R : R;
    a.ptv = ptv > 0 ? ptv : rows * ldv;
    a.dM = dM; a.ptm = dM ? R * C : 0;
    FORGE_REQUIRE(rows < (1ll << 31), FORGE_ESHAPE, dn4 ? "%s: more than 2^31 operand rows; split the batch" : "%s: more than 2^31 tiles; split the batch", name);
    const long long total = R * (dn4 ? C : C / 4), grid = (total + 255) / 256;
    FORGE_REQUIRE(grid < (1ll << 31), FORGE_ESHAPE, "%s: grid too large", name);
    const dim3 g((unsigned)grid), b(256);
    if (kind == IN_DN4H) hipLaunchKernelGGL(wino_input_dn4_kernel<4>, g, b, 0, (hipStream_t)stream, a);
    else if (dn4) hipLaunchKernelGGL(wino_input_dn4_kernel<2>, g, b, 0, (hipStream_t)stream, a);
    else if (kind == IN_DY) hipLaunchKernelGGL(wino_input_kernel<true>, g, b, 0, (hipStream_t)stream, a);
    else hipLaunchKernelGGL(wino_input_kernel<false>, g, b, 0, (hipStream_t)stream, a);
    FORGE_LAUNCH_CHECK(name);
    return 0;
}

extern "C" int forge_wino_input(const float* in, int ld, long long bs, float* V, int ldv, long long ptv, int n, int D, int H, int W, int C,
                                int nsum, long long sum_stride, forge_stream_t stream) {
    return wino_input_impl("forge_wino_input", IN_PLAIN, in, ld, bs, V, ldv, ptv, nullptr, n, D, H, W, C, nsum, sum_stride, stream);
}

extern "C" int forge_wino_input_dn4(const float* in, int ld, long long bs, float* V6, int ldv, long long ptv, int n, int D, int H, int W, int C,
                                    int nsum, long long sum_stride, forge_stream_t stream) {
    return wino_input_impl("forge_wino_input_dn4", IN_DN4, in, ld, bs, V6, ldv, ptv, nullptr, n, D, H, W, C, nsum, sum_stride, stream);
}

extern "C" int forge_wino_input_dn4h(const float* in, int ld, long long bs, float* V, int ldv, long long ptv, int n, int D, int H, int W, int C,
                                     int nsum, long long sum_stride, forge_stream_t stream) {
    return wino_input_impl("forge_wino_input_dn4h", IN_DN4H, in, ld, bs, V, ldv, ptv, nullptr, n, D, H, W, C, nsum, sum_stride, stream);
}

extern "C" int forge_wino_input_dy(const float* dy, int ld, float* V, float* dM, int n, int D, int H, int W, int C, forge_stream_t stream) {
    return wino_input_impl("forge_wino_input_dy", IN_DY, dy, ld, 0, V, C, 0, dM, n, D, H, W, C, 1, 0, stream);
}

static int wino_output_impl(const float* Mm, const float* Mm2, long long bs2, long long pt2, const float* bias, const float* scale, const float* shift, float slope, const float* residual,
                            const float* aux_h, const float* aux_z, float* out, float* out2, float* out3, int n, int D, int H, int W, int Cout,
                            int ldo, int epilogue, bool half, forge_stream_t stream) {
    FORGE_REQUIRE(Mm && out, FORGE_EINVAL, "forge_wino_output: null pointer argument");
    FORGE_REQUIRE(n > 0 && D > 0 && H > 0 && W > 0 && H % 2 == 0 && W % 2 == 0 && Cout > 0 && Cout % 8 == 0 && ldo % 4 == 0, FORGE_ESHAPE,
                  "forge_wino_output: n=%d D=%d H=%d W=%d Cout=%d ldo=%d (H, W even; Cout multiple of 8; ldo of 4)", n, D, H, W, Cout, ldo);
    FORGE_REQUIRE(epilogue >= 0 && epilogue <= 3, FORGE_EINVAL, "forge_wino_output: unknown epilogue %d", epilogue);
    FORGE_REQUIRE(epilogue == W_GRU_GATES ? ldo == Cout / 2 : ldo >= Cout, FORGE_ESHAPE,
                  "forge_wino_output: ldo=%d (epilogues 0, 1, 3: ldo >= Cout=%d; epilogue 2: ldo == Cout / 2)", ldo, Cout);
    FORGE_REQUIRE(epilogue != W_AFFINE_ACT || (scale && shift), FORGE_EINVAL, "forge_wino_output: affine epilogue needs scale/shift");
    FORGE_REQUIRE(epilogue != W_GRU_GATES || (aux_h && out2), FORGE_EINVAL, "forge_wino_output: GRU gate epilogue needs aux_h, out2");
    FORGE_REQUIRE(epilogue != W_GRU_OUT || (aux_h && aux_z && (!out2 || (scale && shift))), FORGE_EINVAL,
                  "forge_wino_output: GRU out epilogue needs aux_h, aux_z (and scale/shift with out2)");
    FORGE_REQUIRE(out3 == nullptr || epilogue == W_GRU_GATES || epilogue == W_GRU_OUT, FORGE_EINVAL, "forge_wino_output: out3 is a GRU-epilogue output");
    WinoOutArgs a;
    const long long R = (long long)n * D * (H / 2) * (W / 2);
    a.Mm = Mm; a.ptm = R * Cout; a.Mm2 = Mm2; a.bs2 = bs2 > 0 ? bs2 : (long long)D * (H / 2) * (W / 2); a.ptm2 = pt2 > 0 ? pt2 : R * Cout; a.bias = bias; a.scale = scale; a.shift = shift; a.slope = slope; a.residual = residual; a.aux_h = aux_h; a.aux_z = aux_z;
    a.out = out; a.out2 = out2; a.out3 = out3; a.ldo = ldo; a.n = n; a.D = D; a.H = H; a.W = W; a.Cout = Cout; a.epi = epilogue;
    FORGE_REQUIRE(R < (1ll << 31), FORGE_ESHAPE, "forge_wino_output: more than 2^31 tiles; split the batch");
    const long long total = R * (Cout / 4), grid = (total + 255) / 256;
    FORGE_REQUIRE(grid < (1ll << 31), FORGE_ESHAPE, "forge_wino_output: grid too large");
    const dim3 g((unsigned)grid), b(256);
    hipStream_t st = (hipStream_t)stream;
    if (half) {
        switch (epilogue) {
            case W_BIAS: hipLaunchKernelGGL((wino_output_kernel<W_BIAS, true>), g, b, 0, st, a); break;
            case W_AFFINE_ACT: hipLaunchKernelGGL((wino_output_kernel<W_AFFINE_ACT, true>), g, b, 0, st, a); break;
            case W_GRU_GATES: hipLaunchKernelGGL((wino_output_kernel<W_GRU_GATES, true>), g, b, 0, st, a); break;
            default: hipLaunchKernelGGL((wino_output_kernel<W_GRU_OUT, true>), g, b, 0, st, a); break;
        }
    } else {
        switch (epilogue) {
            case W_BIAS: hipLaunchKernelGGL(wino_output_kernel<W_BIAS>, g, b, 0, st, a); break;
            case W_AFFINE_ACT: hipLaunchKernelGGL(wino_output_kernel<W_AFFINE_ACT>, g, b, 0, st, a); break;
            case W_GRU_GATES: hipLaunchKernelGGL(wino_output_kernel<W_GRU_GATES>, g, b, 0, st, a); break;
            default: hipLaunchKernelGGL(wino_output_kernel<W_GRU_OUT>, g, b, 0, st, a); break;
        }
    }
    FORGE_LAUNCH_CHECK("forge_wino_output");
    return 0;
}

extern "C" int forge_wino_output(const float* Mm, const float* Mm2, long long bs2, long long pt2, const float* bias, const float* scale, const float* shift, float slope, const float* residual,
                                 const float* aux_h, const float* aux_z, float* out, float* out2, float* out3, int n, int D, int H, int W, int Cout,
                                 int ldo, int epilogue, forge_stream_t stream) {
    return wino_output_impl(Mm, Mm2, bs2, pt2, bias, scale, shift, slope, residual, aux_h, aux_z, out, out2, out3, n, D, H, W, Cout, ldo, epilogue, false, stream);
}

extern "C" int forge_wino_output_half(const float* Mm8, const float* Mm2_8, long long bs2, long long pt2, const float* bias, const float* scale, const float* shift, float slope,
                                      const float* residual, const float* aux_h, const float* aux_z, float* out, float* out2, float* out3, int n, int D, int H, int W,
                                      int Cout, int ldo, int epilogue, forge_stream_t stream) {
    return wino_output_impl(Mm8, Mm2_8, bs2, pt2, bias, scale, shift, slope, residual, aux_h, aux_z, out, out2, out3, n, D, H, W, Cout, ldo, epilogue, true, stream);
}

extern "C" int forge_wino_output_dn4h(const float* Mm, const float* bias, const float* scale, const float* shift, const float* aux_h, const float* aux_z, float* out,
                                      float* out2, float* out3, int n, int D, int H, int W, int Cout, int ldo, int epilogue, forge_stream_t stream) {
    FORGE_REQUIRE(Mm && out && aux_h, FORGE_EINVAL, "forge_wino_output_dn4h: null pointer argument");
    FORGE_REQUIRE(n > 0 && D > 0 && H > 0 && W > 0 && H % 4 == 0 && W % 2 == 0 && Cout > 0 && Cout % 8 == 0 && ldo % 4 == 0, FORGE_ESHAPE,
                  "forge_wino_output_dn4h: n=%d D=%d H=%d W=%d Cout=%d ldo=%d (H multiple of 4, W even; Cout multiple of 8; ldo of 4)", n, D, H, W, Cout, ldo);
    FORGE_REQUIRE(epilogue == W_GRU_GATES || epilogue == W_GRU_OUT, FORGE_EINVAL, "forge_wino_output_dn4h: epilogue %d is not a GRU tail (2, 3)", epilogue);
    FORGE_REQUIRE(epilogue == W_GRU_GATES ? ldo == Cout / 2 : ldo >= Cout, FORGE_ESHAPE,
                  "forge_wino_output_dn4h: ldo=%d (epilogue 3: ldo >= Cout=%d; epilogue 2: ldo == Cout / 2)", ldo, Cout);
    FORGE_REQUIRE(epilogue != W_GRU_GATES || out2, FORGE_EINVAL, "forge_wino_output_dn4h: GRU gate epilogue needs out2");
    FORGE_REQUIRE(epilogue != W_GRU_OUT || (aux_z && (!out2 || (scale && shift))), FORGE_EINVAL,
                  "forge_wino_output_dn4h: GRU out epilogue needs aux_z (and scale/shift with out2)");
    WinoOutArgs a;
    const long long R = (long long)n * D * (H / 4) * (W / 2);
    a.Mm = Mm; a.ptm = R * Cout; a.Mm2 = nullptr; a.bs2 = 0; a.ptm2 = 0; a.bias = bias; a.scale = scale; a.shift = shift; a.slope = 1.f; a.residual = nullptr;
    a.aux_h = aux_h; a.aux_z = aux_z; a.out = out; a.out2 = out2; a.out3 = out3; a.ldo = ldo; a.n = n; a.D = D; a.H = H; a.W = W; a.Cout = Cout; a.epi = epilogue;
    FORGE_REQUIRE(R < (1ll << 31), FORGE_ESHAPE, "forge_wino_output_dn4h: more than 2^31 tiles; split the batch");
    const long long total = R * (Cout / 4), grid = (total + 255) / 256;
    FORGE_REQUIRE(grid < (1ll << 31), FORGE_ESHAPE, "forge_wino_output_dn4h: grid too large");
    const dim3 g((unsigned)grid), b(256);
    if (epilogue == W_GRU_GATES) hipLaunchKernelGGL((wino_output_kernel<W_GRU_GATES, false, 4>), g, b, 0, (hipStream_t)stream, a);
    else hipLaunchKernelGGL((wino_output_kernel<W_GRU_OUT, false, 4>), g, b, 0, (hipStream_t)stream, a);
    FORGE_LAUNCH_CHECK("forge_wino_output_dn4h");
    return 0;
}
```

### forge_amd/flopmeter.py

```python
import torch

from . import _lib
from .convops import WINO_DN4H, WINO_FORMS


def _v(a):
    return a.value if hasattr(a, "value") else a


def _igemm(a):
    C1, C2 = _v(a[1]), _v(a[5])
    n, D, H, W, Cout, ntaps = _v(a[19]), _v(a[20]), _v(a[21]), _v(a[22]), _v(a[27]), _v(a[30])
    return 2.0 * n * D * H * W * Cout * ntaps * (C1 + C2)


def _wino_counter(form):
    def count(a):
        loops = _v(a[17]) if form.kloops is None else form.kloops
        return float(2 * form.points * _v(a[12]) * _v(a[13]) * _v(a[14]) * _v(a[15]) * _v(a[16]) * loops * (_v(a[1]) + _v(a[6])))
    return count


def _wgrad(a):
    return 2.0 * _v(a[11]) * _v(a[12]) * _v(a[13]) * _v(a[14]) * _v(a[19]) * _v(a[21]) * (_v(a[3]) + _v(a[7]))


def _wino_wgrad(a):
    return 2.0 * 16 * _v(a[10]) * _v(a[11]) * _v(a[12]) * _v(a[13]) * _v(a[14]) * _v(a[15]) * (_v(a[2]) + _v(a[6]))


def _attention(a):
    return 4.0 * _v(a[5]) * _v(a[6]) * _v(a[7]) * _v(a[8])


def _attention_lse(a):
    return 4.0 * _v(a[6]) * _v(a[7]) * _v(a[8]) * _v(a[9])


def _attention_bwd(a):
    dv = _v(a[9])
    return (16.0 if dv else 14.0) * _v(a[11]) * _v(a[12]) * _v(a[13]) * _v(a[14])


def _attention_mh(a):
    return 4.0 * _v(a[5]) * _v(a[6]) * _v(a[7]) * _v(a[8]) * _v(a[9])


def _attention_mh_bwd(a):
    return (16.0 if _v(a[8]) else 14.0) * _v(a[10]) * _v(a[11]) * _v(a[12]) * _v(a[13]) * _v(a[14])


def _token_fwd(a):
    return 2.0 * _v(a[13]) * _v(a[14]) * _v(a[15])


def _token_bwd(a):
    dxn = _v(a[9]) or _v(a[12]) or _v(a[13])
    return 2.0 * _v(a[16]) * _v(a[17]) * _v(a[18]) * ((1 if dxn else 0) + (1 if _v(a[10]) else 0))


_ENTRIES = {"forge_conv_igemm": _igemm, **{f.gemm: _wino_counter(f) for f in (*WINO_FORMS.values(), WINO_DN4H)}, "forge_conv_wgrad": _wgrad, "forge_wino_wgrad": _wino_wgrad,
            "forge_attention_fwd": _attention, "forge_attention_fwd_lse": _attention_lse, "forge_attention_bwd": _attention_bwd,
            "forge_attention_mh_fwd": _attention_mh, "forge_attention_mh_bwd": _attention_mh_bwd,
            "forge_token_linear_fwd": _token_fwd, "forge_token_linear_bwd": _token_bwd}
_wino_gemm, _wino_gemm_dn, _wino_gemm_dn4 = (_ENTRIES[WINO_FORMS[k].gemm] for k in ("points", "dn", "dn4"))


class FlopMeter:
    def __init__(self):
        self.flops = {k: 0.0 for k in _ENTRIES}
        self.launches = {k: 0 for k in _ENTRIES}

    def __enter__(self):
        self._lib = _lib.lib()
        self._orig = {}
        for name, fn in _ENTRIES.items():
            orig = getattr(self._lib, name)
            self._orig[name] = orig

            def wrapped(*a, _orig=orig, _fn=fn, _name=name):
                self.flops[_name] += _fn(a)
                self.launches[_name] += 1
                return _orig(*a)
            setattr(self._lib, name, wrapped)
        return self

    def __exit__(self, *exc):
        for name, orig in self._orig.items():
            setattr(self._lib, name, orig)
        return False

    @property
    def gflop(self):
        return sum(self.flops.values()) / 1e9

    def summary(self):
        return {"executed_gflop": self.gflop, "launches": dict(self.launches), "gflop_by_entry": {k: v / 1e9 for k, v in self.flops.items()}}


def stage_replay_ms(model, sample, dev, iters=20):
    from . import geo_utils
    from .graph import GraphedCall
    """{stage: ms per replay} for FORGE's inference step on `sample` (b scenes, 5 input views, V cameras)."""
    e3 = model.encoder_3d
    b = sample["images"].shape[0]
    t = 5
    with torch.no_grad():
        img = sample["images"][:, :t].reshape(b * t, 3, 256, 256).contiguous()
        lifted = e3._trunk_hip(img)
        feats = e3._conv1_hip(lifted).reshape(b, t, 128, 32, 32, 32)
        poses = sample["cam_poses_cv2_canonicalized"][:, :t].contiguous()
        rotated = model.rotate(voxels=feats, camPoses_cv2=poses, grid_size=32, order="distance")
        fused = e3.fuse(rotated)
        fv, dv = e3.heads(fused)
        V = sample["K_cv2"].shape[1]
        cams = geo_utils.camera_dict(sample["cam_extrinsics_cv2_canonicalized"], sample["K_cv2"])
        v2v = model._view2vol(b, V, dev)
    stages = {
        "encoder_resnet": lambda: e3._trunk_hip(img),
        "encoder_conv1": lambda: e3._conv1_hip(lifted),
        "rotate": lambda: model.rotate(voxels=feats, camPoses_cv2=poses, grid_size=32, order="distance"),
        "fuse": lambda: e3.fuse(rotated),
        "heads": lambda: e3.heads(fused),
        "render(+conv_rgb)": lambda: model.render(cams, fv, dv, return_origin_proj=True, view2vol=v2v),
    }
    out = {}
    for name, fn in stages.items():
        def call(fn=fn):
            with torch.no_grad():
                return fn()
        g = GraphedCall(call, dev, warmup=2)
        g()
        torch.cuda.synchronize()
        a, bq = torch.cuda.Event(enable_timing=True), torch.cuda.Event(enable_timing=True)
        a.record()
        for _ in range(iters):
            g()
        bq.record()
        torch.cuda.synchronize()
        out[name] = a.elapsed_time(bq) / iters
        del g
    return out
```

### forge_amd/fusion.py

```python
import torch
import torch.nn as nn

from . import _lib, convops as co, determinism


def hip_inference(module, x):
    return x.is_cuda and x.dtype == torch.float32 and not module.training and not torch.is_grad_enabled()


def frozen_eval(module, x):
    return (x.is_cuda and x.dtype == torch.float32 and not module.training and torch.is_grad_enabled()
            and not any(p.requires_grad for p in module.parameters()))


def affine_act_bwd(dy, y, scale, slope, out=None):
    C = dy.shape[-1]
    M = dy.numel() // C
    if out is None:
        out = torch.empty(dy.shape, dtype=torch.float32, device=dy.device)
    _lib.check(_lib.lib().forge_affine_act_bwd(_lib.ptr(dy), dy.stride(-2), _lib.ptr(y), y.stride(-2), _lib.ptr(scale), float(slope), _lib.ptr(out),
                                               out.stride(-2), M, C, _lib.current_stream()), "forge_affine_act_bwd")
    return out


# ... 23 lines not shown
        ws = stats if pre else torch.empty(L.forge_bn_ws_doubles(C), dtype=torch.float64, device=dev)
        _lib.check(L.forge_bn_train_fwd(p(x), x.stride(0), p(gamma), p(beta), float(eps), float(slope), p(y), C, p(mean), p(invstd), p(running_mean),
                                        p(running_var), float(momentum), p(ws), M, C, p(res), ldres, p(nbt), pre, st()), "forge_bn_train_fwd")
    else:
        import torch.distributed as tdist
        if pre:
            ws = stats.reshape(-1)
        else:
            ws = torch.empty(L.forge_bn_ws_doubles(C) + 1, dtype=torch.float64, device=dev)
        _lib.check(L.forge_bn_sync_stats(p(x), x.stride(0), p(ws), M, C, pre, st()), "forge_bn_sync_stats")
        tot = ws[:2 * C + 1]
        tot[2 * C:].fill_(float(M))
        tdist.all_reduce(tot, op=tdist.ReduceOp.SUM, group=group)
        _lib.check(L.forge_bn_sync_fwd_apply(p(x), x.stride(0), p(gamma), p(beta), float(eps), float(slope), p(y), C, p(mean), p(invstd),
                                             p(running_mean), p(running_var), float(momentum), p(tot), 0, M, C, p(res), ldres, p(nbt), st()),
                   "forge_bn_sync_fwd_apply")
        count = tot[2 * C:].clone()
    return y, (x, gamma, beta, mean, invstd, y if res is not None else None, count, float(slope), group)


@_lib.on_tensor_device
def bn_rows_bwd(saved, dy, need_dres=False):
    x, gamma, beta, mean, invstd, y, count, slope, group = saved
    M, C = x.shape
    dev = x.device
    L, p, st = _lib.lib(), _lib.ptr, _lib.current_stream
    dy = dy if _rows_ok(dy, C) else dy.contiguous()
    dx = torch.empty(M, C, dtype=torch.float32, device=dev)
    dres = torch.empty(M, C, dtype=torch.float32, device=dev) if (y is not None and need_dres) else None
    dg = torch.empty(C, dtype=torch.float32, device=dev) if gamma is not None else None
    db = torch.empty(C, dtype=torch.float32, device=dev) if beta is not None else None
    if group is None:
        ws = torch.empty(L.forge_bn_ws_doubles(C), dtype=torch.float64, device=dev)
        _lib.check(L.forge_bn_train_bwd(p(dy), dy.stride(0), p(x), x.stride(0), p(gamma), p(beta), p(mean), p(invstd), slope, p(dx), C, p(dg), p(db), p(ws),
                                        M, C, p(y), C, p(dres), C, st()), "forge_bn_train_bwd")
    else:
        import torch.distributed as tdist
        ws = torch.empty(L.forge_bn_ws_doubles(C) + 1, dtype=torch.float64, device=dev)
        _lib.check(L.forge_bn_sync_bwd_reduce(p(dy), dy.stride(0), p(x), x.stride(0), p(gamma), p(beta), p(mean), p(invstd), slope, p(dg), p(db), p(ws),
                                              M, C, p(y), C, st()), "forge_bn_sync_bwd_reduce")
        tot = ws[:2 * C]
        tdist.all_reduce(tot, op=tdist.ReduceOp.SUM, group=group)
        ws[2 * C:2 * C + 1].copy_(count)
        _lib.check(L.forge_bn_sync_bwd_apply(p(dy), dy.stride(0), p(x), x.stride(0), p(gamma), p(beta), p(mean), p(invstd), slope, p(dx), C, p(ws),
                                             0, M, C, p(y), C, p(dres), C, st()), "forge_bn_sync_bwd_apply")
    return dx, dg, db, dres


class _BNTrainRows(torch.autograd.Function):

    @staticmethod
    def forward(ctx, x, gamma, beta, running_mean, running_var, momentum, eps, slope, residual, nbt, group, stats=None):
        y, saved = bn_rows_fwd(x, gamma, beta, running_mean, running_var, momentum, eps, slope, residual, nbt, group, stats)
        tensors = tuple(saved[:7])
        ctx.save_for_backward(*tensors)
        ctx.slope, ctx.group = saved[7], saved[8]
        return y

    @staticmethod
    def backward(ctx, dy):
        dx, dg, db, dres = bn_rows_bwd(tuple(ctx.saved_tensors) + (ctx.slope, ctx.group), dy, need_dres=ctx.needs_input_grad[8])
        return dx, dg, db, None, None, None, None, None, dres, None, None, None


class _BNEvalRows(torch.autograd.Function):

    @staticmethod
    @_lib.on_tensor_device
    def forward(ctx, x, gamma, beta, running_mean, running_var, eps, slope, residual):
        M, C = x.shape
        L, p = _lib.lib(), _lib.ptr
        y = torch.empty(M, C, dtype=torch.float32, device=x.device)
        mean, invstd = torch.empty(C, dtype=torch.float32, device=x.device), torch.empty(C, dtype=torch.float32, device=x.device)
        res = None if residual is None else (residual if _rows_ok(residual, C) else residual.contiguous())
        _lib.check(L.forge_bn_eval_fwd(p(x), x.stride(0), p(gamma), p(beta), p(running_mean), p(running_var), float(eps), float(slope), p(y), C, p(mean),
                                       p(invstd), M, C, p(res), 0 if res is None else res.stride(0), _lib.current_stream()), "forge_bn_eval_fwd")
        ctx.save_for_backward(x, gamma, beta, mean, invstd, y if res is not None else None)
        ctx.slope = float(slope)
        return y

    @staticmethod
    @_lib.on_tensor_device
    def backward(ctx, dy):
        x, gamma, beta, mean, invstd, y = ctx.saved_tensors
        M, C = x.shape
        L, p, st = _lib.lib(), _lib.ptr, _lib.current_stream
        dy = dy if _rows_ok(dy, C) else dy.contiguous()
        dx = torch.empty(M, C, dtype=torch.float32, device=x.device)
        dres = torch.empty(M, C, dtype=torch.float32, device=x.device) if (y is not None and ctx.needs_input_grad[7]) else None
        dg = torch.empty(C, dtype=torch.float32, device=x.device) if gamma is not None else None
        db = torch.empty(C, dtype=torch.float32, device=x.device) if beta is not None else None
        if dg is not None or db is not None:
            ws = torch.empty(L.forge_bn_ws_doubles(C), dtype=torch.float64, device=x.device)
            _lib.check(L.forge_bn_sync_bwd_reduce(p(dy), dy.stride(0), p(x), x.stride(0), p(gamma), p(beta), p(mean), p(invstd), ctx.slope, p(dg), p(db), p(ws),
                                                  M, C, p(y), C, st()), "forge_bn_sync_bwd_reduce")
        zero = torch.zeros(2 * C, dtype=torch.float64, device=x.device)
        _lib.check(L.forge_bn_sync_bwd_apply(p(dy), dy.stride(0), p(x), x.stride(0), p(gamma), p(beta), p(mean), p(invstd), ctx.slope, p(dx), C, p(zero),
                                             M, M, C, p(y), C, p(dres), C, st()), "forge_bn_sync_bwd_apply")
        return dx, dg, db, None, None, None, None, dres


def _sync_world(bn):
    import torch.distributed as tdist
    if not (isinstance(bn, nn.SyncBatchNorm) and tdist.is_available() and tdist.is_initialized()):
        return 1
    return tdist.get_world_size(bn.process_group)


def _bn_group(bn):
    if _sync_world(bn) <= 1:
        return None
    import torch.distributed as tdist
    return bn.process_group if bn.process_group is not None else tdist.group.WORLD


def bn_hip_train(bn, rows):
    return (bn.training and rows.is_cuda and rows.dtype == torch.float32 and rows.shape[-1] % 4 == 0
            and (bn.momentum is not None or not bn.track_running_stats))


def bn_module_args(bn):
    track = bn.track_running_stats and bn.running_mean is not None
    return (bn.running_mean if track else None, bn.running_var if track else None, bn.momentum if bn.momentum is not None else 0.0, bn.eps,
            bn.num_batches_tracked if (track and bn.num_batches_tracked is not None) else None, _bn_group(bn))


def bn_act_rows(bn, rows, slope=1.0, residual=None, stats=None):
    C = rows.shape[-1]
    require_hip_input("BatchNorm on channels-last rows", rows)
    if C % 4:
        raise RuntimeError("forge_amd: the HIP BatchNorm kernels need a channel count that is a multiple of 4 (got %d)" % C)
    if bn.training and bn.momentum is None and bn.track_running_stats:
        raise RuntimeError("forge_amd: BatchNorm with momentum=None (cumulative moving average) is not implemented by the HIP kernels "
                           "(the reference's modules use the default momentum 0.1)")
    if not bn.training and bn.track_running_stats and bn.running_mean is not None:
        x = rows.reshape(-1, C)
        x = x if _rows_ok(x, C) else x.contiguous()
        res = None if residual is None else residual.reshape(-1, C)
        return _BNEvalRows.apply(x, bn.weight, bn.bias, bn.running_mean, bn.running_var, bn.eps, slope, res).reshape(rows.shape)
    if bn_hip_train(bn, rows) or not bn.track_running_stats or bn.running_mean is None:
        x = rows.reshape(-1, C)
        x = x if _rows_ok(x, C) else x.contiguous()
        rm, rv, mom, eps, nbt, group = bn_module_args(bn)
        res = None if residual is None else residual.reshape(-1, C)
        args = (x, bn.weight, bn.bias, rm, rv, mom, eps, slope, res, nbt)
        y = _BNTrainRows.apply(*args, group, stats if (stats is not None and stats.numel() and x.data_ptr() == rows.data_ptr()) else None)
        return y.reshape(rows.shape)
    raise RuntimeError("forge_amd: unsupported BatchNorm configuration %r" % (bn,))


def _step_scratch(R, C, dev, form=None, conv0=None):
    F = co.WINO_FORMS
    P2, P1 = ((form or F["half" if co.wino_half_applies(R, c, C) else "points"]) for c in (2 * C, C))
    need = [f.P * (R * 2 // f.th) * c for f, c in ((P2, 2 * C), (P1, C))]
    if form is not None:
        need.append((conv0 or F["half" if co.wino_half_applies(R, C, C) else "points"]).P * R * C)
    return torch.empty(max(need), dtype=torch.float32, device=dev)


def require_hip_input(what, x, channels=None):
    if not (torch.is_tensor(x) and x.is_cuda and x.dtype == torch.float32):
        raise RuntimeError("forge_amd: %s runs only on the MI355X HIP kernels and needs a float32 tensor on a cuda/HIP device (got %s on %s); "
                           "there is no CPU or stock-PyTorch path" % (what, getattr(x, "dtype", type(x)), getattr(x, "device", "?")))
    if channels is not None and channels % 32:
        raise RuntimeError("forge_amd: %s needs a channel count that is a multiple of the GEMM K-step 32 (got %d)" % (what, channels))


class _GRUCellRows(torch.autograd.Function):

    @staticmethod
    @_lib.on_tensor_device
    def forward(ctx, x, h, wg, bg, wo, bo):
        b, D, H, W, C = h.shape
        Cx = x.shape[-1]
        M = b * D * H * W
        dev = h.device
        h = h.contiguous()
        wgc, woc = wg.detach().contiguous(), wo.detach().contiguous()
        bsx = co._batch_stride_rows(x)
        grid = (b, D, H, W)
        new = lambda c: torch.empty(b, D, H, W, c, dtype=torch.float32, device=dev)
        g = new(2 * C)
        co.conv3_launch(x, Cx, h, C, wgc, bg, g, grid, 2 * C, bs1=bsx)
        z, r, hr = new(C), new(C), new(C)
        L, p, st = _lib.lib(), _lib.ptr, _lib.current_stream
        _lib.check(L.forge_gru_gates_fwd(p(g), p(h), p(z), p(r), p(hr), M, C, st()), "forge_gru_gates_fwd")
        cand = new(C)
        co.conv3_launch(x, Cx, hr, C, woc, bo, cand, grid, C, bs1=bsx)
        hn = new(C)
        _lib.check(L.forge_gru_state_fwd(p(cand), p(h), p(z), p(hn), M, C, st()), "forge_gru_state_fwd")
        ctx.save_for_backward(x, h, z, r, hr, cand, wgc, woc)
        ctx.has_bias = (bg is not None, bo is not None)
        return hn

    @staticmethod
    @_lib.on_tensor_device
    def backward(ctx, dhn):
        x, h, z, r, hr, cand, wg, wo = ctx.saved_tensors
        b, D, H, W, C = h.shape
        Cx = x.shape[-1]
        M = b * D * H * W
        dev = h.device
        grid = (b, D, H, W)
        bsx = co._batch_stride_rows(x)
        new = lambda c: torch.empty(b, D, H, W, c, dtype=torch.float32, device=dev)
        L, p, st = _lib.lib(), _lib.ptr, _lib.current_stream
        dhn = dhn.contiguous()
        dh, dz, dc = new(C), new(C), new(C)
        _lib.check(L.forge_gru_state_bwd(p(dhn), C, p(h), p(z), p(cand), p(dh), p(dz), p(dc), M, C, None, 0, 0, 0, st()), "forge_gru_state_bwd")
        dxh = new(Cx + C)
        co.conv3_launch(dc, C, None, 0, wo, None, dxh, grid, Cx + C, dgrad=True)
        dwo = dbo = dwg = dbg = None
        if ctx.needs_input_grad[4]:
            dwo = co.grad_zeros(wo.shape, wo.device)
            co.conv3_wgrad(dc, x, Cx, hr, C, dwo, grid, C, bs1=bsx)
        if ctx.has_bias[1] and ctx.needs_input_grad[5]:
            dbo = co.colsum(dc.reshape(M, C))
        dg = new(2 * C)
        _lib.check(L.forge_gru_gates_bwd(p(dz), _lib.ptr(dxh[..., Cx:]), Cx + C, p(h), p(z), p(r), p(dg), p(dh), None, 0, M, C, None, 0, 0, 0, st()), "forge_gru_gates_bwd")
        dxh2 = new(Cx + C)
        co.conv3_launch(dg, 2 * C, None, 0, wg, None, dxh2, grid, Cx + C, dgrad=True)
        if ctx.needs_input_grad[2]:
            dwg = co.grad_zeros(wg.shape, wg.device)
            co.conv3_wgrad(dg, x, Cx, h, C, dwg, grid, 2 * C, bs1=bsx)
        if ctx.has_bias[0] and ctx.needs_input_grad[3]:
            dbg = co.colsum(dg.reshape(M, 2 * C))
        dx = (dxh[..., :Cx] + dxh2[..., :Cx]) if ctx.needs_input_grad[0] else None
        dh_total = (dh + dxh2[..., Cx:]) if ctx.needs_input_grad[1] else None
        return dx, dh_total, dwg, dbg, dwo, dbo


class _GRUCellPreRows(torch.autograd.Function):

    @staticmethod
    @_lib.on_tensor_device
    def forward(ctx, gx, cx, h, wgh, bg, woh, bo):
        b, D, H, W, C = h.shape
        M = b * D * H * W
        dev = h.device
        h, gx, cx = h.contiguous(), gx.contiguous(), cx.contiguous()
        wg, wo = wgh.detach().contiguous(), woh.detach().contiguous()
        grid = (b, D, H, W)
        new = lambda c: torch.empty(b, D, H, W, c, dtype=torch.float32, device=dev)
        L, p, st = _lib.lib(), _lib.ptr, _lib.current_stream
        g = new(2 * C)
        co.conv3_launch(h, C, None, 0, wg, bg, g, grid, 2 * C, residual=gx)
        z, r, hr = new(C), new(C), new(C)
        _lib.check(L.forge_gru_gates_fwd(p(g), p(h), p(z), p(r), p(hr), M, C, st()), "forge_gru_gates_fwd")
        cand = new(C)
        co.conv3_launch(hr, C, None, 0, wo, bo, cand, grid, C, residual=cx)
        hn = new(C)
        _lib.check(L.forge_gru_state_fwd(p(cand), p(h), p(z), p(hn), M, C, st()), "forge_gru_state_fwd")
        ctx.save_for_backward(h, z, r, hr, cand, wg, wo)
        ctx.has_bias = (bg is not None, bo is not None)
        return hn

    @staticmethod
    @_lib.on_tensor_device
    def backward(ctx, dhn):
        h, z, r, hr, cand, wg, wo = ctx.saved_tensors
        b, D, H, W, C = h.shape
        M = b * D * H * W
        dev = h.device
        grid = (b, D, H, W)
        new = lambda c: torch.empty(b, D, H, W, c, dtype=torch.float32, device=dev)
        L, p, st = _lib.lib(), _lib.ptr, _lib.current_stream
        dhn = dhn.contiguous()
        dh, dz, dc = new(C), new(C), new(C)
        _lib.check(L.forge_gru_state_bwd(p(dhn), C, p(h), p(z), p(cand), p(dh), p(dz), p(dc), M, C, None, 0, 0, 0, st()), "forge_gru_state_bwd")
        dhr = new(C)
        co.conv3_launch(dc, C, None, 0, wo, None, dhr, grid, C, dgrad=True)
        dwo = dbo = dwg = dbg = None
        if ctx.needs_input_grad[5]:
            dwo = co.grad_zeros(wo.shape, wo.device)
            co.conv3_wgrad(dc, hr, C, None, 0, dwo, grid, C)
        if ctx.has_bias[1] and ctx.needs_input_grad[6]:
            dbo = co.colsum(dc.reshape(M, C))
        dg = new(2 * C)
        _lib.check(L.forge_gru_gates_bwd(p(dz), p(dhr), C, p(h), p(z), p(r), p(dg), p(dh), None, 0, M, C, None, 0, 0, 0, st()), "forge_gru_gates_bwd")
        dh_total = new(C)
        co.conv3_launch(dg, 2 * C, None, 0, wg, None, dh_total, grid, C, residual=dh, dgrad=True)
        if ctx.needs_input_grad[3]:
            dwg = co.grad_zeros(wg.shape, wg.device)
            co.conv3_wgrad(dg, h, C, None, 0, dwg, grid, 2 * C)
        if ctx.has_bias[0] and ctx.needs_input_grad[4]:
            dbg = co.colsum(dg.reshape(M, 2 * C))
        return (dg if ctx.needs_input_grad[0] else None), (dc if ctx.needs_input_grad[1] else None), dh_total, dwg, dbg, dwo, dbo


def view_run(g):
    g = list(g)
    return g == list(range(g[0], g[0] + len(g)))


def _view_mean(xr, grp):
    C = xr.shape[-1]
    if view_run(grp):
        return xr[:, grp[0]:grp[0] + len(grp)].mean(dim=1).reshape(-1, C)
    return torch.stack([xr[:, ti] for ti in grp], dim=1).mean(dim=1).reshape(-1, C)


def _wino_view_mean(xr, grp, out):
    b, t, D, H, W, C = xr.shape
    vol = D * H * W
    if view_run(grp):
        return co.wino_input(xr[:, grp[0]:], C, C, b, D, H, W, bs=t * vol, out=out, nsum=len(grp), sum_stride=vol)
    return co.wino_input(_view_mean(xr, grp), C, C, b, D, H, W, out=out)


def _input_products(Vx, U, n, geo, Cout):
    b, D, H, W = geo
    C = Vx.shape[-1]
    R = b * D * (H // 2) * (W // 2)
    return co.wino_gemm(Vx, C, None, 0, U, None, n, D, H // 2, W // 2, Cout, half=co.wino_half_applies(R, Cout, C))


def _h0_wino(p, xr, grp, V, Mm, t0, h, wk="_U"):
    b, t, D, H, W, C = xr.shape
    gemm = lambda k: co.wino_gemm(V, C, None, 0, p[k + wk], Mm, b, D, H // 2, W // 2, C)
    _wino_view_mean(xr, grp, V)
    Mp = gemm("fc0")
    co.wino_output(Mp, p["fc0_b"], *p["bn1"], 0.01, None, None, None, t0, None, None, b, D, H, W, C, C, co.EPI_AFFINE_ACT)
    co.wino_input(t0, C, C, b, D, H, W, out=V)
    Mp = gemm("fc3")
    co.wino_output(Mp, p["fc3_b"], *p["bn4"], 0.01, None, None, None, h, None, None, b, D, H, W, C, C, co.EPI_AFFINE_ACT)


def _h0_direct(p, xr, grp, t0, h):
    b, t, D, H, W, C = xr.shape
    grid, taps = (b, D, H, W), co.TAPS_3x3x3
    co.conv_igemm(_view_mean(xr, grp), C, C, None, 0, 0, p["fc0_w"], p["fc0_b"], *p["bn1"], 0.01, None, None, None, t0, None, grid, grid[1:], C, C,
                  taps, epilogue=co.EPI_AFFINE_ACT)
    co.conv_igemm(t0, C, C, None, 0, 0, p["fc3_w"], p["fc3_b"], *p["bn4"], 0.01, None, None, None, h, None, grid, grid[1:], C, C, taps,
                  epilogue=co.EPI_AFFINE_ACT)


def _wino_step(geo, x, view, views, wg, wo, V, Mm, h, z, hr, hn, out=None, r=None, cand=None, calls=None, th=2):
    b, D, H, W = geo
    C = h.shape[-1]
    transform, gemm = calls or co.wino_calls(co.WINO_FORMS["points"])

    def conv(src, U, Cout, i):
        Vs = transform(src, C, C, b, D, H, W, out=V)
        if isinstance(x, tuple):
            return Vs, gemm(Vs, C, None, 0, U, Mm, b, D, H // th, W // 2, Cout), dict(Mm2=x[i], view=view, views=views)
        return Vs, gemm(x, C, Vs, C, U, Mm, b, D, H // th, W // 2, Cout, view=view, views=views), {}

    Vh, G, add = conv(h, wg[0], 2 * C, 0)
    co.wino_output(G, wg[1], None, None, 1.0, None, h, None, z, hr, r, *geo, 2 * C, C, co.EPI_GRU_GATES, **add)
    Vhr, S, add = conv(hr, wo[0], C, 1)
    co.wino_output(S, *wo[1:], 1.0, None, h, z, hn, out, cand, *geo, C, C, co.EPI_GRU_OUT, **add)
    return Vh, Vhr


def _direct_step(grid, x, wg, wo, h, z, hr, hn, out=None, r=None, cand=None, bs=0):
    C = h.shape[-1]
    ig, taps = grid[1:], co.TAPS_3x3x3
    split = isinstance(x, tuple)
    operands = lambda src, i: ((src, C, C, None, 0, 0), x[i]) if split else ((x, C, C, src, C, C), None)
    ops, res = operands(h, 0)
    co.conv_igemm(*ops, *wg, None, None, 1.0, res, h, None, z, hr, grid, ig, 2 * C, C, taps, epilogue=co.EPI_GRU_GATES, bs1=bs, out3=r)
    ops, res = operands(hr, 1)
    co.conv_igemm(*ops, *wo, 1.0, res, h, z, hn, out, grid, ig, C, C, taps, epilogue=co.EPI_GRU_OUT, bs1=bs, out3=cand)


_WKEY = {None: "_U", co.WINO_FORMS["dn"]: "_Ud", co.WINO_FORMS["dn4"]: "_Ud4", co.WINO_DN4H: "_Ud4h"}
_PACKS = ((None, ("gate", "out", "fc0", "fc3")), (co.WINO_FORMS["dn"], ("gate", "out", "fc0", "fc3")), (co.WINO_FORMS["dn4"], ("gate", "out")),
          (co.WINO_DN4H, ("gate", "out")))


def _fuse_eval(gru, xr, groups, wino, split, h0=None, keep=None, const0=None):
    b, t, D, H, W, C = xr.shape
    dev, M, vol = xr.device, b * D * H * W, D * H * W
    geo = (b, D, H, W)
    new = lambda c=C: torch.empty(M, c, dtype=torch.float32, device=dev)
    step, conv0 = None, None
    if wino:
        R = b * D * (H // 2) * (W // 2)
        F = co.WINO_FORMS
        both = lambda form: H % form.th == 0 and all(form.applies(R * 2 // form.th, D, H // form.th, W // 2, c, 2 * C) for c in (2 * C, C))
        fits = lambda form: co.wino_fits(b, D, H, W, C, views=t, form=form)
        if not split and keep is None and const0 is None and both(F["dn"]):
            step = F["dn4"] if both(F["dn4"]) and fits(F["dn4"]) else F["dn"]
            if step is F["dn4"] and both(co.WINO_DN4H) and fits(co.WINO_DN4H):
                step = co.WINO_DN4H
            conv0 = F["dn"] if F["dn"].applies(R, D, H // 2, W // 2, C, C) else None
    p = gru._packed_halves(wino) if (split or const0 is not None) else gru._packed_wino(step) if wino else gru._packed()
    wk = _WKEY[step] if wino else "_w"
    weights = lambda half: ((p["gate" + wk + half], p["gate_b"]), (p["out" + wk + half], p["out_b"], *p["norm"]))
    wg, wo = weights("h" if split else "")
    if wino:
        calls = co.wino_calls(step or F["points"])
        X = calls[0](xr, C, C, b * t, D, H, W)
        if split:
            X = (_input_products(X, p["gate_Ux"], b * t, geo, 2 * C), _input_products(X, p["out_Ux"], b * t, geo, C))
        Vs = torch.empty(step.points, int(R * 2 // step.th * step.rows), C, dtype=torch.float32, device=dev) if step else torch.empty(16, R, C, dtype=torch.float32, device=dev)
        V = Vs.reshape(-1)[:16 * R * C].view(16, R, C)
        Mm = _step_scratch(R, C, dev, step, conv0)
    elif split:
        X = {}
        for ti in sorted({ti for g in groups for ti in g}):
            X[ti] = (new(2 * C), new())
            for k, dst in zip(("gate_wx", "out_wx"), X[ti]):
                co.conv_igemm(xr[:, ti], C, C, None, 0, 0, p[k], None, None, None, 1.0, None, None, None, dst, None, geo, geo[1:], dst.shape[1],
                              dst.shape[1], co.TAPS_3x3x3, epilogue=co.EPI_BIAS, bs1=t * vol)
    outs = []
    for grp in groups:
        grp = list(grp)
        t0, h, out = new(), new(), new()
        if h0 is not None:
            h.copy_(h0.permute(0, 2, 3, 4, 1).reshape(M, C))
        elif wino:
            _h0_wino(p, xr, grp, V, Mm, t0, h, _WKEY[conv0])
        else:
            _h0_direct(p, xr, grp, t0, h)
        if keep is not None:
            keep.append(t0)
        if const0 is not None and "MXg0" not in const0:
            Vx0 = co.wino_input(xr[:, 0], C, C, b, D, H, W, bs=t * vol)
            const0["MXg0"], const0["MXc0"] = _input_products(Vx0, p["gate_Ux"], b, geo, 2 * C), _input_products(Vx0, p["out_Ux"], b, geo, C)
        z, hr, hn, r, cand = new(), new(), t0, None, None
        for k, ti in enumerate(grp):
            if keep is not None:
                z, hr, r, hn, cand = new(), new(), new(), new(), new()
            last = out if k == len(grp) - 1 else None
            if not wino:
                _direct_step(geo, X[ti] if split else xr[:, ti], wg, wo, h, z, hr, hn, last, r, cand, bs=0 if split else t * vol)
            elif const0 is not None and k == 0:
                _wino_step(geo, (const0["MXg0"], const0["MXc0"]), 0, 1, *weights("h"), V, Mm, h, z, hr, hn, last, r, cand)
            else:
                _wino_step(geo, X, ti, t, wg, wo, Vs, Mm, h, z, hr, hn, last, r, cand, calls=calls, th=step.th if step else 2)
            if keep is not None:
                keep += [h, z, r, cand]
            h, hn = hn, h
        outs.append(out.reshape(b, D, H, W, C).permute(0, 4, 1, 2, 3))
    return outs


def _eval_chunks(x, fuse):
    b, t, C, D, H, W = x.shape
    xr = x.permute(0, 1, 3, 4, 5, 2)
    xr = xr if xr.is_contiguous() else xr.contiguous()
    nb = co.wino_scene_chunk(b, D, H, W, C, views=t) if co.wino_enabled() else 0
    parts = [fuse(xr[i:i + (nb or b)], nb > 0, i, i + (nb or b)) for i in range(0, b, nb or b)]
    return parts[0] if len(parts) == 1 else [torch.cat(o, dim=0) for o in zip(*parts)]


class _FuseFrozen(torch.autograd.Function):

    @staticmethod
    @_lib.on_tensor_device
    def forward(ctx, x, gru, skip_dx0=False, const0=None):
        ctx.skip_dx0 = bool(skip_dx0)
        b, t, C, D, H, W = x.shape
        xr = x.permute(0, 1, 3, 4, 5, 2)
        xr = xr if xr.is_contiguous() else xr.contiguous()
        wino = co.wino_enabled() and co.wino_fits(b, D, H, W, C, views=t)
        saved = []
        out = _fuse_eval(gru, xr, [range(t)], wino, False, keep=saved, const0=const0 if (wino and skip_dx0) else None)[0]
        ctx.gru, ctx.shape = gru, (b, t, C, D, H, W)
        ctx.save_for_backward(*saved)
        return out

    @staticmethod
    @_lib.on_tensor_device
    def backward(ctx, dout):
        gru = ctx.gru
        b, t, C, D, H, W = ctx.shape
        saved = ctx.saved_tensors
        t0, steps = saved[0], [saved[1 + 4 * i:5 + 4 * i] for i in range(t)]
        p = gru._packed_T()
        dev, M = dout.device, b * D * H * W
        grid = (b, D, H, W)
        new = lambda c=C: torch.empty(M, c, dtype=torch.float32, device=dev)
        L, ptr, st = _lib.lib(), _lib.ptr, _lib.current_stream
        dgrad = lambda dy, Cdy, k, dst, Cdst, residual=None: co.conv3_launch(dy, Cdy, None, 0, p[k + "_w"], None, dst, grid, Cdst, residual=residual,
                                                                           dgrad=True, U=p[k + "_UT"], wT=p[k + "_wT"])
        dr = dout.permute(0, 2, 3, 4, 1)
        dr = (dr if dr.is_contiguous() else dr.contiguous()).reshape(M, C)
        dhn = dr * p["norm_scale"]
        ld_dhn = C
        dx = torch.empty(b, t, D, H, W, C, dtype=torch.float32, device=dev)
        for ti in reversed(range(t)):
            h, z, r, cand = steps[ti]
            dh, dz, dc, dg = new(), new(), new(), new(2 * C)
            _lib.check(L.forge_gru_state_bwd(ptr(dhn), ld_dhn, ptr(h), ptr(z), ptr(cand), ptr(dh), ptr(dz), ptr(dc), M, C, None, 0, 0, 0, st()), "forge_gru_state_bwd")
            if ti == 0 and ctx.skip_dx0:
                dhr = dgrad(dc, C, "out_h", new(), C)
                dhp = new()
                _lib.check(L.forge_gru_gates_bwd(ptr(dz), ptr(dhr), C, ptr(h), ptr(z), ptr(r), ptr(dg), ptr(dh), ptr(dhp), C, M, C, None, 0, 0, 0, st()),
                           "forge_gru_gates_bwd")
                toth = dgrad(dg, 2 * C, "gate_h", new(), C, residual=dhp)
                dx[:, 0].zero_()
                dhn, ld_dhn = toth, C
                continue
            dxh = new(2 * C)
            dgrad(dc, C, "out", dxh, 2 * C)
            _lib.check(L.forge_gru_gates_bwd(ptr(dz), ptr(dxh[:, C:]), 2 * C, ptr(h), ptr(z), ptr(r), ptr(dg), ptr(dh), ptr(dxh[:, C:]), 2 * C, M, C,
                                             None, 0, 0, 0, st()), "forge_gru_gates_bwd")
            tot = new(2 * C)
            dgrad(dg, 2 * C, "gate", tot, 2 * C, residual=dxh)
            dx[:, ti] = tot.view(b, D, H, W, 2 * C)[..., :C]
            dhn, ld_dhn = tot[:, C:], 2 * C
        h0 = steps[0][0]
        g = torch.empty(M, C, dtype=torch.float32, device=dev)
        affine_act_bwd(dhn, h0, p["bn4_scale"], 0.01, out=g)
        g2 = new()
        dgrad(g, C, "fc3", g2, C)
        affine_act_bwd(g2, t0, p["bn1_scale"], 0.01, out=g)
        dgrad(g, C, "fc0", g2, C)
        dx.add_(g2.reshape(b, 1, D, H, W, C), alpha=1.0 / t)
        return dx.permute(0, 1, 5, 2, 3, 4), None, None, None


def _flatten_saved(obj, tensors):
    if torch.is_tensor(obj):
        tensors.append(obj)
        return ("t", len(tensors) - 1)
    if isinstance(obj, (list, tuple)):
        return ("l" if isinstance(obj, list) else "u", [_flatten_saved(o, tensors) for o in obj])
    if isinstance(obj, dict):
        return ("d", [(k, _flatten_saved(v, tensors)) for k, v in obj.items()])
    return ("c", obj)


def _unflatten_saved(spec, tensors):
    kind, val = spec
    if kind == "t":
        return tensors[val]
    if kind in ("l", "u"):
        items = [_unflatten_saved(v, tensors) for v in val]
        return items if kind == "l" else tuple(items)
    if kind == "d":
        return {k: _unflatten_saved(v, tensors) for k, v in val}
    return val


class _FuseGroupsTrain(torch.autograd.Function):

    @staticmethod
    @_lib.on_tensor_device
    def forward(ctx, x, Wg, bg, Wo, bo, w0, b0, g1, be1, w3, b3, g4, be4, gn, bn_, gru, groups):
        b, t, C, D, H, W = x.shape
        xr = x.detach().permute(0, 1, 3, 4, 5, 2)
        xr = xr if xr.is_contiguous() else xr.contiguous()
        dev, M, Ht, Wt = x.device, b * D * H * W, H // 2, W // 2
        R1 = D * Ht * Wt
        R = b * R1
        geo = (b, D, H, W)
        fc, norm = gru.fusion_conv, gru.fusion_norm
        new = lambda c=C: torch.empty(M, c, dtype=torch.float32, device=dev)
        pk = lambda w: co.pack_conv3d_weight(w)
        wpg, wpo = pk(Wg), pk(Wo)
        packs = {"gx": wpg[:, :, :C].contiguous(), "gh": wpg[:, :, C:].contiguous(), "ox": wpo[:, :, :C].contiguous(), "oh": wpo[:, :, C:].contiguous(),
                 "f0": pk(w0), "f3": pk(w3)}
        U = {k: co.wino_pack_packed(v) for k, v in packs.items()}
        Vx = co.wino_input(xr, C, C, b * t, D, H, W)
        MX = (_input_products(Vx, U["gx"], b * t, geo, 2 * C), _input_products(Vx, U["ox"], b * t, geo, C))
        Mm = _step_scratch(R, C, dev)
        bnargs = lambda m: bn_module_args(m)
        outs, saved_groups = [], []
        for grp in groups:
            grp = list(grp)
            Vm = _wino_view_mean(xr, grp, torch.empty(16, R, C, dtype=torch.float32, device=dev))
            a0 = new()
            Mp = co.wino_gemm(Vm, C, None, 0, U["f0"], Mm, b, D, Ht, Wt, C)
            co.wino_output(Mp, b0, None, None, 1.0, None, None, None, a0, None, None, *geo, C, C, co.EPI_BIAS)
            rm, rv, mom, eps, nbt, group = bnargs(fc[1])
            t0, sv1 = bn_rows_fwd(a0, g1, be1, rm, rv, mom, eps, 0.01, None, nbt, group)
            Vt0 = co.wino_input(t0, C, C, b, D, H, W)
            a1 = new()
            Mp = co.wino_gemm(Vt0, C, None, 0, U["f3"], Mm, b, D, Ht, Wt, C)
            co.wino_output(Mp, b3, None, None, 1.0, None, None, None, a1, None, None, *geo, C, C, co.EPI_BIAS)
            rm, rv, mom, eps, nbt, group = bnargs(fc[4])
            h, sv4 = bn_rows_fwd(a1, g4, be4, rm, rv, mom, eps, 0.01, None, nbt, group)
            steps = []
            for ti in grp:
                z, hr, r, hn, cand = new(), new(), new(), new(), new()
                Vh, Vhr = _wino_step(geo, MX, ti, t, (U["gh"], bg), (U["oh"], bo, None, None), None, Mm, h, z, hr, hn, r=r, cand=cand)
                steps.append((ti, h, z, r, cand, Vh, Vhr))
                h = hn
            rm, rv, mom, eps, nbt, group = bnargs(norm)
            out, svn = bn_rows_fwd(h, gn, bn_, rm, rv, mom, eps, 1.0, None, nbt, group)
            outs.append(out.reshape(b, D, H, W, C).permute(0, 4, 1, 2, 3))
# ... 289 lines not shown
```

### include/forge_hip.h

```cpp
#ifndef FORGE_HIP_H
#define FORGE_HIP_H

#ifdef __cplusplus
extern "C" {
#endif

typedef void* forge_stream_t;

#define FORGE_EINVAL (-1)
#define FORGE_ESHAPE (-2)

int forge_version(void);
const char* forge_last_error(void);

int forge_rotate_fwd(const float* vox, const float* xf, const int* mode, float* out,
                     int n, int C, int D, int H, int W, forge_stream_t stream);

int forge_rotate_fwd_slots(const float* vox, const float* xf, const int* mode, const int* dst_slot, float* out,
                           int n, int C, int D, int H, int W, forge_stream_t stream);

int forge_rotate_xf_from_poses(const float* poses, float* xf, int* mode, int* slot, const float* dist, int B, int t, float half_extent,
                               forge_stream_t stream);

int forge_pose_chain_fwd(const float* rot, const float* trans, const float* can_pose, const float* can_extr, const float* K, float half_extent,
                         int b, int t, float* xf, int* mode, int* slot, float* cam16, float* poses, float* origin, float* jac, forge_stream_t stream);
int forge_pose_chain_bwd(const float* jac, const float* dxf, const float* dcam, float* drot, float* dtrans, int b, int t, forge_stream_t stream);

int forge_rotate_bwd(const float* dout, const float* vox, const float* xf, const int* mode,
                     float* dvox, float* dxf, int n, int C, int D, int H, int W,
                     forge_stream_t stream);
int forge_rotate_bwd_slots(const float* dout, const float* vox, const float* xf, const int* mode, const int* src_slot,
                           float* dvox, float* dxf, int n, int C, int D, int H, int W, forge_stream_t stream);

int forge_render_fwd(const float* feat, const float* dens, const float* cam, const int* view2vol,
                     float* out_feat, float* out_opac, float* out_depth,
                     int V, int nvol, int C, int D, int H, int W, int Hr, int Wr, int S,
                     float zmin, float zmax, float hx, float hy, float hz,
                     forge_stream_t stream);

int forge_pack_cameras(const float* R, long long r0, long long r1, long long r2, const float* T, long long t0, long long t1,
                       const float* K, long long k0, long long k1, long long k2, float* cam16, float* origin, int V, forge_stream_t stream);

long long forge_render_bwd_ws_bytes(int V, int C, int Hr, int Wr, int S, int want_cam);
int forge_render_bwd(const float* feat, const float* dens, const float* cam, const int* view2vol,
                     const float* g_feat, const float* g_opac, const float* g_depth,
                     float* dfeat, float* ddens, float* dcam,
                     int V, int nvol, int C, int D, int H, int W, int Hr, int Wr, int S,
                     float zmin, float zmax, float hx, float hy, float hz,
                     void* ws, long long ws_bytes, forge_stream_t stream);

int forge_resize_bilinear_fwd(const float* in, float* out, int P, int Hi, int Wi, int Ho, int Wo, forge_stream_t stream);
int forge_resize_bilinear_bwd(const float* g, float* din, int P, int Hi, int Wi, int Ho, int Wo, forge_stream_t stream);

int forge_conv_igemm(const float* in1, int C1, int ld1, long long bs1, const float* in2, int C2, int ld2, long long bs2,
                     const float* wp,
                     const float* bias, const float* scale, const float* shift, float slope, const float* residual,
                     const float* aux_h, const float* aux_z, float* out, float* out2, float* out3,
                     int n, int D, int H, int W, int is, int Di, int Hi, int Wi, int Cout, int ldo,
                     const int* taps, int ntaps, int os, int pz, int py, int px, int Do, int Ho, int Wo,
                     int epilogue, int lift, int tile, int ksplit, float* splitk_ws, long long splitk_ws_bytes, double* stats, forge_stream_t stream);

int forge_conv_igemm_plan(long long M, int Cout, int Cin, int ntaps, int nphase, int epilogue, int ldo, long long splitk_ws_bytes,
                          int* tile, int* ksplit);

int forge_conv_igemm_epilogue(long long M, int Cout, int ldo, int ldr, int has_residual, int os, int same_grid, int nphase, int lift, int ksplit,
                              int has_stats, int epilogue, int* fast);
int forge_conv_fast_epilogue(int on);

int forge_wino_weights(const float* wp, float* U, int Cout, int Cin, int kd, int transpose, forge_stream_t stream);
int forge_wino_dy(const float* dy, int ldy, float* dM, int n, int D, int H, int W, int Cout, forge_stream_t stream);
int forge_wino_wgrad(const float* dMm, const float* V1, int C1, long long bs1, long long pt1, const float* V2, int C2, long long bs2,
                     long long pt2, float* dU, int n, int D, int Ht, int Wt, int Cout, int kd, forge_stream_t stream);
int forge_wino_dw(const float* dU, float* dw, int Cout, int Cin, int kd, forge_stream_t stream);
int forge_wino_input(const float* in, int ld, long long bs, float* V, int ldv, long long ptv, int n, int D, int H, int W, int C,
                     int nsum , long long sum_stride,
                     forge_stream_t stream);
int forge_wino_input_dy(const float* dy, int ld, float* V, float* dM, int n, int D, int H, int W, int C, forge_stream_t stream);
int forge_wino_gemm(const float* V1, int C1, int ld1, long long bs1, long long pt1, const float* V2, int C2, int ld2, long long bs2,
                    long long pt2, const float* U, float* Mm, int n, int D, int Ht, int Wt, int Cout, int kd, int tile ,
                    forge_stream_t stream);
int forge_wino_gemm_half(const float* V1, int C1, int ld1, long long bs1, long long pt1, const float* V2, int C2, int ld2, long long bs2,
                         long long pt2, const float* U, float* Mm8, int n, int D, int Ht, int Wt, int Cout, int kd, forge_stream_t stream);
int forge_wino_output_half(const float* Mm8, const float* Mm2_8 , long long bs2, long long pt2, const float* bias, const float* scale,
                           const float* shift, float slope, const float* residual, const float* aux_h, const float* aux_z, float* out, float* out2, float* out3,
                           int n, int D, int H, int W, int Cout, int ldo, int epilogue, forge_stream_t stream);
int forge_wino_gemm_dn(const float* V1, int C1, int ld1, long long bs1, long long pt1, const float* V2, int C2, int ld2, long long bs2,
                       long long pt2, const float* Ud, float* Mm, int n, int D, int Ht, int Wt, int Cout, int kd, forge_stream_t stream);
int forge_wino_weights_dn(const float* wp, float* Ud, int Cout, int Cin, forge_stream_t stream);
int forge_wino_input_dn4(const float* in, int ld, long long bs, float* V6, int ldv, long long ptv, int n, int D, int H, int W, int C,
                         int nsum, long long sum_stride, forge_stream_t stream);
int forge_wino_weights_dn4(const float* wp, float* Ud, int Cout, int Cin, forge_stream_t stream);
int forge_wino_gemm_dn4(const float* V1, int C1, int ld1, long long bs1, long long pt1, const float* V2, int C2, int ld2, long long bs2,
                        long long pt2, const float* Ud, float* Mm, int n, int D, int Ht, int Wt, int Cout, int kd, forge_stream_t stream);
int forge_wino_input_dn4h(const float* in, int ld, long long bs, float* V, int ldv, long long ptv, int n, int D, int H, int W, int C,
                          int nsum, long long sum_stride, forge_stream_t stream);
int forge_wino_weights_dn4h(const float* wp, float* Ud, int Cout, int Cin, forge_stream_t stream);
int forge_wino_gemm_dn4h(const float* V1, int C1, int ld1, long long bs1, long long pt1, const float* V2, int C2, int ld2, long long bs2,
                         long long pt2, const float* Ud, float* Mm, int n, int D, int Ht, int Wt, int Cout, int kd, forge_stream_t stream);
int forge_wino_output_dn4h(const float* Mm, const float* bias, const float* scale, const float* shift, const float* aux_h, const float* aux_z, float* out,
                           float* out2, float* out3, int n, int D, int H, int W, int Cout, int ldo, int epilogue, forge_stream_t stream);
int forge_wino_gemm_tile(long long R, int Cout, int Cin);
int forge_wino_output(const float* Mm, const float* Mm2, long long bs2, long long pt2, const float* bias, const float* scale, const float* shift, float slope, const float* residual,
                      const float* aux_h, const float* aux_z, float* out, float* out2, float* out3, int n, int D, int H, int W, int Cout,
                      int ldo, int epilogue, forge_stream_t stream);

int forge_conv_wgrad(const float* dy, int ldy, const float* x1, int C1, int ld1, long long bs1, const float* x2, int C2, int ld2,
                     long long bs2, float* dw, int n, int D, int H, int W, int is, int Di, int Hi, int Wi, int Cout,
                     const int* taps, int ntaps, forge_stream_t stream);

int forge_conv_direct_fwd(const float* in, int ld_in, const float* w, const float* bias, float slope, float* out, int ld_out,
                          int n, int D, int H, int W, int Cin, int Cout, const int* taps, int ntaps, forge_stream_t stream);
int forge_conv_direct_dgrad(const float* dy, int ld_dy, const float* w, float* dx, int ld_dx,
                            int n, int D, int H, int W, int Cin, int Cout, const int* taps, int ntaps, forge_stream_t stream);
int forge_conv_direct_wgrad(const float* dy, int ld_dy, const float* x, int ld_x, float* dw,
                            int n, int D, int H, int W, int Cin, int Cout, const int* taps, int ntaps, forge_stream_t stream);

int forge_conv_wgrad_det(const float* dy, int ldy, const float* x1, int C1, int ld1, long long bs1, const float* x2, int C2, int ld2,
                         long long bs2, float* dw, int n, int D, int H, int W, int is, int Di, int Hi, int Wi, int Cout,
                         const int* taps, int ntaps, int accumulate, void* ws, long long ws_bytes, forge_stream_t stream);
long long forge_conv_wgrad_det_ws_bytes(int C1, int C2, int n, int D, int H, int W, int is, int Di, int Hi, int Wi, int Cout,
                                        const int* taps, int ntaps);
int forge_conv_wgrad_plan(int C1, int C2, int n, int D, int H, int W, int is, int Di, int Hi, int Wi, int Cout, const int* taps, int ntaps,
                          int det, long long* plan);
int forge_wino_wgrad_det(const float* dMm, const float* V1, int C1, long long bs1, long long pt1, const float* V2, int C2, long long bs2,
                         long long pt2, float* dU, int n, int D, int Ht, int Wt, int Cout, int kd, int accumulate, void* ws, long long ws_bytes,
                         forge_stream_t stream);
long long forge_wino_wgrad_det_ws_bytes(int C1, int C2, int n, int D, int Ht, int Wt, int Cout, int kd);
int forge_conv_direct_wgrad_det(const float* dy, int ld_dy, const float* x, int ld_x, float* dw, int n, int D, int H, int W, int Cin, int Cout,
                                const int* taps, int ntaps, int accumulate, void* ws, long long ws_bytes, forge_stream_t stream);
long long forge_conv_direct_wgrad_det_ws_bytes(int n, int D, int H, int W, int Cin, int Cout, int ntaps);
int forge_rotate_bwd_det(const float* dout, const float* vox, const float* xf, const int* mode, float* dvox, float* dxf,
                         int n, int C, int D, int H, int W, int accumulate, void* ws, long long ws_bytes, forge_stream_t stream);
long long forge_rotate_bwd_det_ws_bytes(int n, int C, int D, int H, int W);
int forge_rotate_bwd_slots_det(const float* dout, const float* vox, const float* xf, const int* mode, const int* src_slot,
                               float* dvox, float* dxf, int n, int C, int D, int H, int W, int accumulate, void* ws, long long ws_bytes,
                               forge_stream_t stream);
long long forge_rotate_bwd_slots_det_ws_bytes(int n, int C, int D, int H, int W);

int forge_gru_gates_fwd(const float* g, const float* h, float* z, float* r, float* hr, long long M, int C, forge_stream_t stream);
int forge_gru_state_fwd(float* c_cand, const float* h, const float* z, float* hn, long long M, int C, forge_stream_t stream);
int forge_gru_state_bwd(const float* dhn, int ld_dhn, const float* h, const float* z, const float* cand, float* dh, float* dz, float* dc,
                        long long M, int C, float* dc_acc, long long acc_bs, long long vol, int acc_mode, forge_stream_t stream);
int forge_gru_gates_bwd(const float* dz, const float* dhr, int ld_dhr, const float* h, const float* z, const float* r,
                        float* dg, float* dh, float* dh_out, int ld_dh_out, long long M, int C, float* dg_acc, long long acc_bs, long long vol,
                        int acc_mode, forge_stream_t stream);

int forge_bn_ws_doubles(int C);
int forge_colsum(const float* x, int ldx, float* out, double* ws, long long M, int C, forge_stream_t stream);
int forge_bn_train_fwd(const float* x, int ldx, const float* gamma, const float* beta, float eps, float slope, float* y, int ldy,
                       float* mean, float* invstd, float* running_mean, float* running_var, float momentum, double* ws,
                       long long M, int C, const float* res, int ldres, long long* num_batches_tracked,
                       int nblk_pre ,
                       forge_stream_t stream);
int forge_bn_train_bwd(const float* dy, int lddy, const float* x, int ldx, const float* gamma, const float* beta, const float* mean,
                       const float* invstd, float slope, float* dx, int lddx, float* dgamma, float* dbeta, double* ws, long long M, int C,
                       const float* y, int ldy, float* dres, int lddres, forge_stream_t stream);
int forge_bn_sync_stats(const float* x, int ldx, double* ws, long long M, int C, int nblk_pre , forge_stream_t stream);
int forge_bn_sync_fwd_apply(const float* x, int ldx, const float* gamma, const float* beta, float eps, float slope, float* y, int ldy,
                            float* mean, float* invstd, float* running_mean, float* running_var, float momentum, const double* totals,
                            long long M_total, long long M, int C, const float* res, int ldres, long long* num_batches_tracked, forge_stream_t stream);
int forge_bn_eval_fwd(const float* x, int ldx, const float* gamma, const float* beta, const float* running_mean, const float* running_var,
                      float eps, float slope, float* y, int ldy, float* mean, float* invstd, long long M, int C, const float* res, int ldres,
                      forge_stream_t stream);
int forge_bn_sync_bwd_reduce(const float* dy, int lddy, const float* x, int ldx, const float* gamma, const float* beta, const float* mean,
                             const float* invstd, float slope, float* dgamma, float* dbeta, double* ws, long long M, int C,
                             const float* y, int ldy, forge_stream_t stream);
int forge_bn_sync_bwd_apply(const float* dy, int lddy, const float* x, int ldx, const float* gamma, const float* beta, const float* mean,
                            const float* invstd, float slope, float* dx, int lddx, const double* totals, long long M_total, long long M, int C,
                            const float* y, int ldy, float* dres, int lddres, forge_stream_t stream);

int forge_affine_act_bwd(const float* dy, int ld_dy, const float* y, int ld_y, const float* scale, float slope, float* dx, int ld_dx,
                         long long M, int C, forge_stream_t stream);

int forge_attention_fwd(const float* q, const float* k, const float* v, long long v_batch_rows, float* out, int B, int Nq, int Nk, int d,
                        forge_stream_t stream);

int forge_attention_fwd_lse(const float* q, const float* k, const float* v, long long v_batch_rows, float* out, float* lse, int B, int Nq, int Nk,
                            int d, forge_stream_t stream);
int forge_attention_bwd(const float* q, const float* k, const float* v, long long v_batch_rows, const float* out, const float* lse,
                        const float* dout, float* dq, float* dk, float* dv, float* delta_ws, int B, int Nq, int Nk, int d, forge_stream_t stream);

int forge_attention_mh_fwd(const float* q, const float* k, const float* v, float* out, float* lse, int B, int H, int Nq, int Nk, int d,
                           long long q_bs, long long q_rs, long long k_bs, long long k_rs, long long v_bs, long long v_rs, long long out_bs,
                           long long out_rs, float scale, forge_stream_t stream);
int forge_attention_mh_bwd(const float* q, const float* k, const float* v, const float* out, const float* lse, const float* dout, float* dq,
                           float* dk, float* dv, float* delta_ws, int B, int H, int Nq, int Nk, int d, long long q_bs, long long q_rs,
                           long long k_bs, long long k_rs, long long v_bs, long long v_rs, long long out_bs, long long out_rs, float scale,
                           forge_stream_t stream);

#define FORGE_TOKEN_ACT_NONE 0
#define FORGE_TOKEN_ACT_GELU 1
int forge_token_linear_fwd(const float* x, long long ldx, const float* w, const float* bias, const float* gamma, const float* beta, float eps,
                           const float* residual, long long ldr, float* y, long long ldy, float* pre, float* stats, int R, int K, int N, int act,
                           forge_stream_t stream);
int forge_layer_norm_fwd(const float* x, long long ldx, const float* gamma, const float* beta, float eps, float* y, long long ldy, float* stats,
                         int R, int K, forge_stream_t stream);
int forge_token_rows_plan(int R, int K, int N, int* chunks, int* chunk_rows);
long long forge_token_linear_bwd_ws_bytes(int R, int K, int N, int ln);
int forge_token_linear_bwd(const float* dy, long long lddy, const float* x, long long ldx, const float* w, const float* gamma, const float* beta,
                           const float* stats, const float* pre, float* dx, float* dw, float* dbias, float* dgamma, float* dbeta, float* ws,
                           long long ws_bytes, int R, int K, int N, int act, forge_stream_t stream);
long long forge_layer_norm_bwd_ws_bytes(int R, int K);
int forge_layer_norm_bwd(const float* dy, long long lddy, const float* x, long long ldx, const float* gamma, const float* stats, float* dx,
                         float* dgamma, float* dbeta, float* ws, long long ws_bytes, int R, int K, forge_stream_t stream);

int forge_im2col_nchw(const float* img, float* out, int N, int C, int H, int W, int kh, int kw, int stride, int pad,
                      int Kpad, forge_stream_t stream);
int forge_maxpool2d_nhwc(const float* in, float* out, int N, int H, int W, int C, int k, int stride, int pad,
                         forge_stream_t stream);

int forge_sse_groups_blocks(void);
int forge_sse_groups_fwd(const float* pred, long long sn, long long sc, long long sh, long long sw, const float* target,
                         float* partial, int B, int Vp, int Vt, int gsize, int C, int H, int W, forge_stream_t stream);
int forge_sse_groups_bwd(const float* pred, long long sn, long long sc, long long sh, long long sw, const float* target,
                         const float* coef, float* dpred, int B, int Vp, int Vt, int gsize, int C, int H, int W, forge_stream_t stream);

int forge_adam_small(float* param, const float* grad, float* exp_avg, float* exp_avg_sq, float* step, int n, float lr, float beta1, float beta2,
                     float eps, forge_stream_t stream);

int forge_vgg_prep_fwd(const float* a, long long a_sn, long long a_sc, long long a_sh, long long a_sw, const float* b, long long b_sn,
                       long long b_sc, long long b_sh, long long b_sw, const float* mean, const float* std, float* rows, int N, int C,
                       int Hi, int Wi, int Ho, int Wo, int resize, forge_stream_t stream);
int forge_vgg_prep_bwd(const float* g, int ldg, const float* std, float* din, long long sn, long long sc, long long sh, long long sw,
                       int N, int C, int Hi, int Wi, int Ho, int Wo, int resize, forge_stream_t stream);
int forge_l1_partial_blocks(void);
int forge_l1_partial(const float* x, const float* y, long long n, float* partial, forge_stream_t stream);
int forge_vgg_tap_bwd(const float* x, const float* y, const float* g_next, const float* coef, float* d_pre, int N, int H, int W, int C,
                      forge_stream_t stream);

int forge_metric_blocks(void);
int forge_ssim_tiles(int H, int W);
int forge_psnr(const float* a, long long a_sn, long long a_sc, long long a_sh, long long a_sw, const float* b, long long b_sn, long long b_sc,
               long long b_sh, long long b_sw, int N, int C, int H, int W, double data_range, double* partial, double* out, forge_stream_t stream);
int forge_ssim(const float* a, long long a_sn, long long a_sc, long long a_sh, long long a_sw, const float* b, long long b_sn, long long b_sc,
               long long b_sh, long long b_sw, int N, int C, int H, int W, double data_range, double* partial, double* out, forge_stream_t stream);
int forge_lpips_tap(const float* f, int N, int HW, int C, const float* w, double* partial, forge_stream_t stream);
int forge_lpips_finalize(const double* partial, int N, int hw0, int hw1, int hw2, int hw3, int hw4, float* out, forge_stream_t stream);

int forge_pose_sync(const float* P, const float* conf, const int* pairs, int B, int N, int E, int squares, int center, double rank_tol,
                    float* out, double* sv, int* status, forge_stream_t stream);

#define FORGE_MESH_OVERFLOW 1
#define FORGE_MESH_TABLE_INTS 154
int forge_mesh_case_table(int* table, int capacity);
long long forge_mesh_workspace_bytes(int n, int D, int H, int W);
int forge_mesh_count(const float* density, int n, int D, int H, int W, float level, void* workspace, long long workspace_bytes, int* counts,
                     forge_stream_t stream);
int forge_mesh_emit(const float* density, const float* features, int n, int C, int D, int H, int W, float level, float volume_size,
                    const void* workspace, long long workspace_bytes, const int* counts, const int* offsets, int max_vertices, int max_faces,
                    float* vertices, float* normals, int* faces, float* vertex_features, int* status, forge_stream_t stream);

int forge_mesh_bake(const float* vertices, const float* normals, const int* counts, const int* offsets, int n, int max_vertices,
                    const float* density, int D, int H, int W, float hx, float hy, float hz, const float* images, const float* view_weight,
// ... 88 lines not shown
```

Measured before the change: 1073 views/s.

## Add F(4x4) width-and-height Winograd form with depth nesting for ConvGRU

Adds a new depth-nested Winograd form (dn4hw) that uses 4x4 output tiles in both H and W, with 36 transform points instead of 24, plus new input, weight, GEMM and output kernels. It is chosen for the ConvGRU step when dn4h already applies, the channel count is large enough and the shapes fit. The aim is to cut the multiply work and operand rows per output in the GRU convolutions. The trade-off is more transform work, larger operand buffers and possibly more numerical error from the F(4,3) transform in fp32.

```diff
diff --git a/forge_amd/convops.py b/forge_amd/convops.py
--- a/forge_amd/convops.py
+++ b/forge_amd/convops.py
@@ -199,6 +199,7 @@
     winograd = True
     wino_depth_nest = os.environ.get("FORGE_WINO_DEPTH_NEST", "1") != "0"
     wino_depth_nest4 = os.environ.get("FORGE_WINO_DEPTH_NEST4", "1") != "0"
+    wino_w4 = os.environ.get("FORGE_WINO_W4", "1") != "0"
     wino_h4 = os.environ.get("FORGE_WINO_H4", "1") != "0"
     conv_fast_epilogue = os.environ.get("FORGE_CONV_FAST_EPILOGUE", "1") != "0"
 
@@ -445,8 +446,8 @@
 
 def wino_fits(n, D, H, W, C, views=1, nest4=False, form=None):
     form = form or WINO_FORMS["dn4" if nest4 else "points"]
-    rows = n * views * D * (H // form.th) * (W // 2) * form.rows
-    return H % form.th == 0 and W % 2 == 0 and rows * C * 4 <= MAX_OPERAND_BYTES
+    rows = n * views * D * (H // form.th) * (W // form.tw) * form.rows
+    return H % form.th == 0 and W % form.tw == 0 and rows * C * 4 <= MAX_OPERAND_BYTES
 
 
 @_lib.on_tensor_device
@@ -475,7 +476,14 @@
     return STATE.wino_h4 and wino_depth_nest4_applies(R, D, Ht, Wt, Cout, Cin)
 
 
-WinoForm = collections.namedtuple("WinoForm", "name P gemm weights ushape input rows kloops applies tile metered points th", defaults=(16, 2))
+WINO_W4_MIN_C = 64
+
+
+def wino_depth_nest4hw_applies(R, D, Ht, Wt, Cout, Cin):
+    return STATE.wino_w4 and Cin // 2 >= WINO_W4_MIN_C and wino_depth_nest4h_applies(R, D, Ht, Wt, Cout, Cin)
+
+
+WinoForm = collections.namedtuple("WinoForm", "name P gemm weights ushape input rows kloops applies tile metered points th tw", defaults=(16, 2, 2))
 _U4 = lambda kd, co_, ci_: (16, kd, co_, ci_)
 WINO_FORMS = {f.name: f for f in (
     WinoForm("points", 16, "forge_wino_gemm", "forge_wino_weights", _U4, "forge_wino_input", 1, None, lambda R, D, Ht, Wt, Cout, Cin: True,
@@ -490,6 +498,10 @@
 
 WINO_DN4H = WinoForm("dn4h", 24, "forge_wino_gemm_dn4h", "forge_wino_weights_dn4h", lambda kd, co_, ci_: (24, 6, co_, ci_), "forge_wino_input_dn4h",
                      Fraction(3, 2), Fraction(3, 2), lambda *a: wino_depth_nest4h_applies(*a), False, False, 24, 4)
+
+WINO_DN4HW = WinoForm("dn4hw", 36, "forge_wino_gemm_dn4hw", "forge_wino_weights_dn4hw", lambda kd, co_, ci_: (36, 6, co_, ci_), "forge_wino_input_dn4hw",
+                      Fraction(3, 2), Fraction(3, 2), lambda *a: wino_depth_nest4hw_applies(*a), False, False, 36, 4, 4)
+_WINO_OUT = {f.P: f for f in (WINO_DN4H, WINO_DN4HW)}
 
 
 def wino_calls(form):
@@ -515,7 +527,7 @@
 
 @_lib.on_tensor_device
 def wino_form_input(form, x, C, ld, n, D, H, W, bs=0, out=None, nsum=1, sum_stride=0):
-    rows = int(n * D * (H // form.th) * (W // 2) * form.rows)
+    rows = int(n * D * (H // form.th) * (W // form.tw) * form.rows)
     V = out if out is not None else torch.empty(form.points, rows, C, dtype=torch.float32, device=x.device)
     if form.rows != 1 and (V.shape != (form.points, rows, C) or not V.is_contiguous()):
         raise ValueError("depth-nest operand buffer %s is not [%d][%d][%d]" % (tuple(V.shape), form.points, rows, C))
@@ -579,15 +591,18 @@
 @_lib.on_tensor_device
 def wino_output(Mm, bias, scale, shift, slope, residual, aux_h, aux_z, out, out2, out3, n, D, H, W, Cout, ldo, epilogue, Mm2=None, view=0, views=1):
     P = Mm.shape[0] if Mm.dim() == 3 else 0
-    vol = D * (H // (WINO_DN4H.th if P == WINO_DN4H.P else 2)) * (W // 2)
-    if P not in (8, 16, WINO_DN4H.P) or Mm.shape[1:] != (n * vol, Cout) or not Mm.is_contiguous():
-        raise ValueError("point products %s do not match [8 | 16][%d][%d] (or the 24 points' rows)" % (tuple(Mm.shape), n * vol, Cout))
-    if P == WINO_DN4H.P:
-        if Mm2 is not None or residual is not None or H % 4 or epilogue not in (EPI_GRU_GATES, EPI_GRU_OUT):
-            raise ValueError("24-point products take the GRU tails only, without a second addend or a residual, on H %% 4 == 0 (H=%d epilogue=%d)" % (H, epilogue))
-        _lib.check(_lib.lib().forge_wino_output_dn4h(_lib.ptr(Mm), _lib.ptr(bias), _lib.ptr(scale), _lib.ptr(shift), _lib.ptr(aux_h), _lib.ptr(aux_z),
-                                                     _lib.ptr(out), _lib.ptr(out2), _lib.ptr(out3), n, D, H, W, Cout, ldo, epilogue, _lib.current_stream()),
-                   "forge_wino_output_dn4h")
+    own = _WINO_OUT.get(P)
+    th, tw = (own.th, own.tw) if own else (2, 2)
+    vol = D * (H // th) * (W // tw)
+    if P not in (8, 16, *_WINO_OUT) or Mm.shape[1:] != (n * vol, Cout) or not Mm.is_contiguous():
+        raise ValueError("point products %s do not match [8 | 16][%d][%d] (or the 24 / 36 points' rows)" % (tuple(Mm.shape), n * vol, Cout))
+    if own:
+        if Mm2 is not None or residual is not None or H % th or W % tw or epilogue not in (EPI_GRU_GATES, EPI_GRU_OUT):
+            raise ValueError("%d-point products take the GRU tails only, without a second addend or a residual, on H %% %d == 0, W %% %d == 0 (H=%d W=%d epilogue=%d)"
+                             % (P, th, tw, H, W, epilogue))
+        name = "forge_wino_output_" + own.name
+        _lib.check(getattr(_lib.lib(), name)(_lib.ptr(Mm), _lib.ptr(bias), _lib.ptr(scale), _lib.ptr(shift), _lib.ptr(aux_h), _lib.ptr(aux_z),
+                                             _lib.ptr(out), _lib.ptr(out2), _lib.ptr(out3), n, D, H, W, Cout, ldo, epilogue, _lib.current_stream()), name)
         return out
     if Mm2 is not None and (Mm2.shape != (P, n * views * vol, Cout) or not Mm2.is_contiguous()):
         raise ValueError("second addend %s does not match [%d][%d][%d] (the form of Mm)" % (tuple(Mm2.shape), P, n * views * vol, Cout))
diff --git a/forge_amd/csrc/conv_igemm.hip b/forge_amd/csrc/conv_igemm.hip
--- a/forge_amd/csrc/conv_igemm.hip
+++ b/forge_amd/csrc/conv_igemm.hip
@@ -1240,8 +1240,8 @@
 
 static int wino_gemm_impl(const float* V1, int C1, int ld1, long long bs1, long long pt1, const float* V2, int C2, int ld2, long long bs2,
                           long long pt2, const float* U, float* Mm, int n, int D, int Ht, int Wt, int Cout, int kd, int tile, int form, forge_stream_t stream) {
-    const bool half = form == 1, dn = form == 2, dn4h = form == 4, dn4 = form == 3 || dn4h;
-    const char* const name4 = dn4h ? "forge_wino_gemm_dn4h" : "forge_wino_gemm_dn4";
+    const bool half = form == 1, dn = form == 2, dn4hw = form == 5, dn4h = form == 4 || dn4hw, dn4 = form == 3 || dn4h;
+    const char* const name4 = dn4hw ? "forge_wino_gemm_dn4hw" : dn4h ? "forge_wino_gemm_dn4h" : "forge_wino_gemm_dn4";
     FORGE_REQUIRE(tile == 0 || (tile >= 'A' && tile <= 'E'), FORGE_EINVAL, "forge_wino_gemm: tile must be 0 (default rule) or 'A'..'E'");
     FORGE_REQUIRE(V1 && U && Mm && (kd == 1 || kd == 3), FORGE_EINVAL, "forge_wino_gemm: null pointer argument / kd not 1 or 3");
     FORGE_REQUIRE(n > 0 && D > 0 && Ht > 0 && Wt > 0 && Cout > 16, FORGE_EINVAL, "forge_wino_gemm: bad dims n=%d D=%d Ht=%d Wt=%d Cout=%d (Cout > 16)", n,
@@ -1253,7 +1253,7 @@
                   "forge_wino_gemm_dn: needs three depth taps, an even D and Ht Wt %% 64 == 0 (kd=%d D=%d Ht=%d Wt=%d)", kd, D, Ht, Wt);
     FORGE_REQUIRE(!dn4 || (kd == 3 && D % 4 == 0 && ((long long)Ht * Wt) % 64 == 0), FORGE_EINVAL,
                   "%s: needs three depth taps, D %% 4 == 0 and Ht Wt %% 64 == 0 (kd=%d D=%d Ht=%d Wt=%d)", name4, kd, D, Ht, Wt);
-    FORGE_REQUIRE(!dn4h || D >= 8, FORGE_EINVAL, "forge_wino_gemm_dn4h: D=%d must be at least 8", D);
+    FORGE_REQUIRE(!dn4h || D >= 8, FORGE_EINVAL, "%s: D=%d must be at least 8", name4, D);
     ConvArgs a;
     memset(&a, 0, sizeof(a));
     const long long vol = (long long)D * Ht * Wt, R = (long long)n * vol, rows = dn4 ? vol / 4 * 6 : vol, Cin = C1 + C2;
@@ -1272,7 +1272,7 @@
     }
     a.wp = U; a.slope = 1.f; a.out = Mm; a.n = n; a.D = D; a.H = Ht; a.W = Wt; a.is = 1; a.Di = D; a.Hi = Ht; a.Wi = Wt;
     a.Cout = Cout; a.ldo = Cout; a.ldr = Cout; a.ntaps = a.tpp = npos; a.os = 1; a.Do = D; a.Ho = Ht; a.Wo = Wt; a.nphase = 1; a.epi = EPI_BIAS;
-    a.ksplit = 1; a.nbat = half ? 4 : dn4h ? 24 : 16;
+    a.ksplit = 1; a.nbat = half ? 4 : dn4hw ? 36 : dn4h ? 24 : 16;
     a.pt1 = pt1 > 0 ? pt1 : (long long)n * rows * ld1; a.pt2 = V2 ? (pt2 > 0 ? pt2 : (long long)n * rows * ld2) : 0;
     a.ptw = (long long)npos * Cout * Cin; a.pto = R * Cout;
     if (form == 0 || half) {
@@ -1311,3 +1311,9 @@
     FORGE_REQUIRE(C1 > 0 && C1 % BK == 0 && C2 >= 0 && C2 % BK == 0, FORGE_EINVAL, "forge_wino_gemm_dn4h: C1=%d / C2=%d must be multiples of %d", C1, C2, BK);
     return wino_gemm_impl(V1, C1, ld1, bs1, pt1, V2, C2, ld2, bs2, pt2, Ud, Mm, n, D, Ht, Wt, Cout, kd, 'B', 4, stream);
 }
+
+extern "C" int forge_wino_gemm_dn4hw(const float* V1, int C1, int ld1, long long bs1, long long pt1, const float* V2, int C2, int ld2, long long bs2,
+                                     long long pt2, const float* Ud, float* Mm, int n, int D, int Ht, int Wt, int Cout, int kd, forge_stream_t stream) {
+    FORGE_REQUIRE(C1 > 0 && C1 % BK == 0 && C2 >= 0 && C2 % BK == 0, FORGE_EINVAL, "forge_wino_gemm_dn4hw: C1=%d / C2=%d must be multiples of %d", C1, C2, BK);
+    return wino_gemm_impl(V1, C1, ld1, bs1, pt1, V2, C2, ld2, bs2, pt2, Ud, Mm, n, D, Ht, Wt, Cout, kd, 'B', 5, stream);
+}
diff --git a/forge_amd/csrc/winograd.hip b/forge_amd/csrc/winograd.hip
--- a/forge_amd/csrc/winograd.hip
+++ b/forge_amd/csrc/winograd.hip
@@ -72,13 +72,20 @@
          : k == 3 ? ((0.25 * w0 + w2) + 0.5 * w1) / 6.0 : k == 4 ? ((0.25 * w0 + w2) - 0.5 * w1) / 6.0 : w2;
 }
 
-template <int NH = 4, double (*HROW)(int, double, double, double) = depth_row_f23>
+template <int NH = 4, double (*HROW)(int, double, double, double) = depth_row_f23, int NW = 4>
 __device__ __forceinline__ void g_d_gt_store(const double (&d)[3][3], float* up, long long pt) {
     double g[NH][3];
 #pragma unroll
     for (int b = 0; b < 3; ++b)
 #pragma unroll
         for (int i = 0; i < NH; ++i) g[i][b] = HROW(i, d[0][b], d[1][b], d[2][b]);
+    if constexpr (NW == 6) {
+#pragma unroll
+        for (int i = 0; i < NH; ++i)
+#pragma unroll
+            for (int j = 0; j < 6; ++j) up[(6 * i + j) * pt] = (float)depth_row_f43(j, g[i][0], g[i][1], g[i][2]);
+        return;
+    }
 #pragma unroll
     for (int i = 0; i < NH; ++i) {
         up[(4 * i + 0) * pt] = (float)g[i][0];
@@ -191,6 +198,77 @@
     }
 }
 
+template <int KP, bool MEAN>
+__device__ __forceinline__ void wino_input_dn4hw_body(const WinoInArgs& a, long long idx) {
+    const int Ht = a.H >> 2, Wt = a.W >> 2, Dg = a.D >> 2;
+    unsigned r, t;
+    int c, tw, th;
+    tile_decode(idx, a.C, 0, Ht, Wt, r, c, tw, th, t);
+    const unsigned q = t; t = q / (unsigned)Dg;
+    const int g = (int)(q - t * (unsigned)Dg);
+    const float* base = a.in + (long long)t * a.bs * a.ld + c;
+    const float inv = 1.f / (float)a.nsum;
+    constexpr int K0 = KP == 0 ? 0 : 2 * KP - 1, K1 = KP == 0 ? 5 : 2 * KP;
+    const int kpos[2] = {K0, K1};
+    float d[2][6][6];
+    unsigned oz[6], oy[6], ox[6];
+#pragma unroll
+    for (int e = 0; e < 6; ++e) {
+        oz[e] = (unsigned)min(max(4 * g - 1 + e, 0), a.D - 1) * (unsigned)(a.H * a.W) * (unsigned)a.ld;
+        oy[e] = (unsigned)min(max(4 * th - 1 + e, 0), a.H - 1) * (unsigned)a.W * (unsigned)a.ld;
+        ox[e] = (unsigned)min(max(4 * tw - 1 + e, 0), a.W - 1) * (unsigned)a.ld;
+    }
+#pragma unroll
+    for (int j = 0; j < 6; ++j) {
+        const int x = 4 * tw - 1 + j;
+#pragma unroll
+        for (int i = 0; i < 6; ++i) {
+            const int y = 4 * th - 1 + i;
+            const bool ok = (unsigned)y < (unsigned)a.H && (unsigned)x < (unsigned)a.W;
+            float p[6], o[6];
+#pragma unroll
+            for (int e = 0; e < 6; ++e) {
+                const int z = 4 * g - 1 + e;
+                const float* s = base + (oz[e] + oy[i] + ox[j]);
+                float v = *s;
+                if constexpr (MEAN) {
+                    for (int k = 1; k < a.nsum; ++k) v += s[(long long)k * a.ss * a.ld];
+                    v *= inv;
+                }
+                p[e] = __int_as_float(__float_as_int(v) & (ok && (unsigned)z < (unsigned)a.D ? -1 : 0));
+            }
+            f43_six_lines(p[0], p[1], p[2], p[3], p[4], p[5], o[0], o[1], o[2], o[3], o[4], o[5]);
+            d[0][i][j] = o[K0];
+            d[1][i][j] = o[K1];
+        }
+#pragma unroll
+        for (int k = 0; k < 2; ++k)
+            f43_six_lines(d[k][0][j], d[k][1][j], d[k][2][j], d[k][3][j], d[k][4][j], d[k][5][j], d[k][0][j], d[k][1][j], d[k][2][j], d[k][3][j], d[k][4][j], d[k][5][j]);
+    }
+    const long long HWt = (long long)Ht * Wt;
+    float* vp = a.V + ((((long long)t * Dg + g) * 6) * HWt + (long long)th * Wt + tw) * a.ldv + c;
+#pragma unroll
+    for (int k = 0; k < 2; ++k) {
+#pragma unroll
+        for (int i = 0; i < 6; ++i) {
+            float v[6];
+            f43_six_lines(d[k][i][0], d[k][i][1], d[k][i][2], d[k][i][3], d[k][i][4], d[k][i][5], v[0], v[1], v[2], v[3], v[4], v[5]);
+#pragma unroll
+            for (int j = 0; j < 6; ++j) vp[kpos[k] * HWt * a.ldv + (6 * i + j) * a.ptv] = v[j];
+        }
+    }
+}
+
+template <bool MEAN>
+__global__ __launch_bounds__(192) void wino_input_dn4hw_kernel(const WinoInArgs a) {
+    const long long idx = (long long)xcd_remap(blockIdx.x, gridDim.x) * 64 + (threadIdx.x & 63);
+    if (idx >= (long long)a.n * (a.D >> 2) * (a.H >> 2) * (a.W >> 2) * a.C) return;
+    const int kp = __builtin_amdgcn_readfirstlane((int)(threadIdx.x >> 6));
+    if (kp == 0) wino_input_dn4hw_body<0, MEAN>(a, idx);
+    else if (kp == 1) wino_input_dn4hw_body<1, MEAN>(a, idx);
+    else wino_input_dn4hw_body<2, MEAN>(a, idx);
+}
+
 __global__ __launch_bounds__(256) void wino_weight_kernel(const float* __restrict__ wp, float* __restrict__ U, int Cout, int Cin, int KD, int transpose) {
     const int No = transpose ? Cin : Cout, Nc = transpose ? Cout : Cin;
     const long long idx = (long long)blockIdx.x * 256 + threadIdx.x, per = (long long)No * Nc;
@@ -209,7 +287,7 @@
     g_d_gt_store(w, U + ((long long)kd * No + o) * Nc + c, KD * per);
 }
 
-template <int K, double (*ROW)(int, double, double, double), int NH = 4, double (*HROW)(int, double, double, double) = depth_row_f23>
+template <int K, double (*ROW)(int, double, double, double), int NH = 4, double (*HROW)(int, double, double, double) = depth_row_f23, int NW = 4>
 __global__ __launch_bounds__(256) void wino_weight_nest_kernel(const float* __restrict__ wp, float* __restrict__ U, int Cout, int Cin) {
     const long long idx = (long long)blockIdx.x * 256 + threadIdx.x, per = (long long)Cout * Cin;
     if (idx >= per) return;
@@ -223,7 +301,7 @@
         for (int a = 0; a < 3; ++a)
 #pragma unroll
             for (int b = 0; b < 3; ++b) d[a][b] = ROW(k, w[0][a][b], w[1][a][b], w[2][a][b]);
-        g_d_gt_store<NH, HROW>(d, U + k * per + idx, K * per);
+        g_d_gt_store<NH, HROW, NW>(d, U + k * per + idx, K * per);
     }
 }
 
@@ -355,6 +433,95 @@
         }
 }
 
+template <int EPI, int NI, int NJ>
+__device__ __forceinline__ void wino_tail(const WinoOutArgs& a, const float4 (&y)[NI][NJ], unsigned t, int y0, int x0, int c) {
+    float4 bias = make_float4(0.f, 0.f, 0.f, 0.f), sc = make_float4(1.f, 1.f, 1.f, 1.f), sh = bias;
+    if (a.bias) bias = *reinterpret_cast<const float4*>(a.bias + c);
+    if (EPI == W_GRU_OUT && a.out2 && a.scale) {
+        sc = *reinterpret_cast<const float4*>(a.scale + c);
+        sh = *reinterpret_cast<const float4*>(a.shift + c);
+    }
+    const int Ch = a.Cout >> 1;
+    const long long plane = (long long)t * a.H * a.W;
+#pragma unroll
+    for (int i = 0; i < NI; ++i)
+#pragma unroll
+        for (int j = 0; j < NJ; ++j) {
+            const long long orow = plane + (long long)(y0 + i) * a.W + (x0 + j);
+            float v[4] = {y[i][j].x + bias.x, y[i][j].y + bias.y, y[i][j].z + bias.z, y[i][j].w + bias.w};
+            const float scv[4] = {sc.x, sc.y, sc.z, sc.w}, shv[4] = {sh.x, sh.y, sh.z, sh.w};
+            if constexpr (EPI == W_GRU_GATES) {
+                float g[4];
+#pragma unroll
+                for (int k = 0; k < 4; ++k) g[k] = 1.f / (1.f + expf(-v[k]));
+                if (c < Ch) {
+                    *reinterpret_cast<float4*>(a.out + orow * Ch + c) = make_float4(g[0], g[1], g[2], g[3]);
+                } else {
+                    const float4 h = *reinterpret_cast<const float4*>(a.aux_h + orow * Ch + (c - Ch));
+                    *reinterpret_cast<float4*>(a.out2 + orow * Ch + (c - Ch)) = make_float4(h.x * g[0], h.y * g[1], h.z * g[2], h.w * g[3]);
+                    if (a.out3) *reinterpret_cast<float4*>(a.out3 + orow * Ch + (c - Ch)) = make_float4(g[0], g[1], g[2], g[3]);
+                }
+            } else {
+                const float4 z4 = *reinterpret_cast<const float4*>(a.aux_z + orow * a.Cout + c);
+                const float4 h4 = *reinterpret_cast<const float4*>(a.aux_h + orow * a.Cout + c);
+                const float zv[4] = {z4.x, z4.y, z4.z, z4.w}, hv[4] = {h4.x, h4.y, h4.z, h4.w};
+                float cand[4], hn[4];
+#pragma unroll
+                for (int k = 0; k < 4; ++k) {
+                    cand[k] = tanhf(v[k]);
+                    hn[k] = hv[k] * (1.f - zv[k]) + cand[k] * zv[k];
+                }
+                *reinterpret_cast<float4*>(a.out + orow * a.ldo + c) = make_float4(hn[0], hn[1], hn[2], hn[3]);
+                if (a.out2)
+                    *reinterpret_cast<float4*>(a.out2 + orow * a.ldo + c) =
+                        make_float4(fmaf(hn[0], scv[0], shv[0]), fmaf(hn[1], scv[1], shv[1]), fmaf(hn[2], scv[2], shv[2]), fmaf(hn[3], scv[3], shv[3]));
+                if (a.out3) *reinterpret_cast<float4*>(a.out3 + orow * a.ldo + c) = make_float4(cand[0], cand[1], cand[2], cand[3]);
+            }
+        }
+}
+
+template <int EPI, int RH>
+__device__ __forceinline__ void wino_output_dn4hw_body(const WinoOutArgs& a, long long idx) {
+    const int C4 = a.Cout >> 2, Ht = a.H >> 2, Wt = a.W >> 2;
+    unsigned r, t;
+    int c, tw, th;
+    tile_decode(idx, C4, 2, Ht, Wt, r, c, tw, th, t);
+    const float* mp = a.Mm + (long long)r * a.Cout + c;
+    float4 s[2][6];
+#pragma unroll
+    for (int j = 0; j < 6; ++j) {
+        float4 m[6];
+#pragma unroll
+        for (int i = RH; i < 5 + RH; ++i) m[i] = *reinterpret_cast<const float4*>(mp + (6 * i + j) * a.ptm);
+        const float4 sl = add(m[1], m[2]), dl = sub(m[1], m[2]), Sl = add(m[3], m[4]), Dl = sub(m[3], m[4]);
+        if constexpr (RH == 0) {
+            s[0][j] = add(add(sl, Sl), m[0]);
+            s[1][j] = fma4(2.f, Dl, dl);
+        } else {
+            s[0][j] = fma4(4.f, Sl, sl);
+            s[1][j] = add(fma4(8.f, Dl, dl), m[5]);
+        }
+    }
+    float4 y[2][4];
+#pragma unroll
+    for (int i = 0; i < 2; ++i) {
+        const float4 sl = add(s[i][1], s[i][2]), dl = sub(s[i][1], s[i][2]), Sl = add(s[i][3], s[i][4]), Dl = sub(s[i][3], s[i][4]);
+        y[i][0] = add(add(sl, Sl), s[i][0]);
+        y[i][1] = fma4(2.f, Dl, dl);
+        y[i][2] = fma4(4.f, Sl, sl);
+        y[i][3] = add(fma4(8.f, Dl, dl), s[i][5]);
+    }
+    wino_tail<EPI>(a, y, t, 4 * th + 2 * RH, 4 * tw, c);
+}
+
+template <int EPI>
+__global__ __launch_bounds__(256) void wino_output_dn4hw_kernel(const WinoOutArgs a) {
+    const long long idx = (long long)blockIdx.x * 128 + (threadIdx.x & 127);
+    if (idx >= (long long)a.n * a.D * (a.H >> 2) * (a.W >> 2) * (a.Cout >> 2)) return;
+    if (__builtin_amdgcn_readfirstlane((int)(threadIdx.x >> 7)) == 0) wino_output_dn4hw_body<EPI, 0>(a, idx);
+    else wino_output_dn4hw_body<EPI, 1>(a, idx);
+}
+
 struct WinoDyArgs {
     const float* dy; int ldy;
     float* dM; long long ptm;
@@ -459,16 +626,23 @@
     return wino_weights_launch("forge_wino_weights_dn4h", wino_weight_nest_kernel<6, depth_row_f43, 6, depth_row_f43>, (long long)Cout * Cin, stream, wp, Ud, Cout, Cin);
 }
 
-enum WinoInKind { IN_PLAIN, IN_DN4, IN_DY, IN_DN4H };
+extern "C" int forge_wino_weights_dn4hw(const float* wp, float* Ud, int Cout, int Cin, forge_stream_t stream) {
+    FORGE_REQUIRE(wp && Ud && Cout > 0 && Cin > 0, FORGE_EINVAL, "forge_wino_weights_dn4hw: bad argument");
+    return wino_weights_launch("forge_wino_weights_dn4hw", wino_weight_nest_kernel<6, depth_row_f43, 6, depth_row_f43, 6>, (long long)Cout * Cin, stream, wp, Ud, Cout, Cin);
+}
+
+enum WinoInKind { IN_PLAIN, IN_DN4, IN_DY, IN_DN4H, IN_DN4HW };
 
 static int wino_input_impl(const char* name, WinoInKind kind, const float* in, int ld, long long bs, float* V, int ldv, long long ptv, float* dM, int n, int D, int H,
                            int W, int C, int nsum, long long sum_stride, forge_stream_t stream) {
-    const bool dn4 = kind == IN_DN4 || kind == IN_DN4H;
-    const int th = kind == IN_DN4H ? 4 : 2;
+    const bool h4 = kind == IN_DN4H || kind == IN_DN4HW, dn4 = kind == IN_DN4 || h4;
+    const int th = h4 ? 4 : 2, tw = kind == IN_DN4HW ? 4 : 2;
     FORGE_REQUIRE(in && V && (kind != IN_DY || dM), FORGE_EINVAL, "%s: null pointer argument", name);
     FORGE_REQUIRE(nsum >= 1 && (nsum == 1 || sum_stride > 0), FORGE_EINVAL, "%s: nsum >= 1, and a positive sum_stride (rows) with nsum > 1", name);
     FORGE_REQUIRE(!dn4 || (D > 0 && D % 4 == 0), FORGE_EINVAL, "%s: D=%d must be a multiple of 4", name, D);
-    FORGE_REQUIRE(kind != IN_DN4H || (D >= 8 && H > 0 && H % 4 == 0), FORGE_EINVAL, "%s: D=%d H=%d (D >= 8; H a multiple of 4)", name, D, H);
+    FORGE_REQUIRE(!h4 || (D >= 8 && H > 0 && H % 4 == 0), FORGE_EINVAL, "%s: D=%d H=%d (D >= 8; H a multiple of 4)", name, D, H);
+    FORGE_REQUIRE(kind != IN_DN4HW || (W > 0 && W % 4 == 0), FORGE_EINVAL, "%s: W=%d must be a multiple of 4", name, W);
+    FORGE_REQUIRE(kind != IN_DN4HW || (long long)D * H * W * ld < (1ll << 31), FORGE_EINVAL, "%s: a batch element of 2^31 floats or more (32-bit offsets inside it)", name);
     const bool ok = n > 0 && D > 0 && H > 0 && W > 0 && H % 2 == 0 && W % 2 == 0 && C > 0 && C % 4 == 0 && ld >= C && ld % 4 == 0 && ldv >= C && ldv % 4 == 0;
     if (kind == IN_DY)
         FORGE_REQUIRE(ok, FORGE_ESHAPE, "%s: n=%d D=%d H=%d W=%d C=%d ld=%d (H, W even; C, ld multiples of 4)", name, n, D, H, W, C, ld);
@@ -476,14 +650,17 @@
     WinoInArgs a;
     a.in = in; a.ld = ld; a.bs = bs > 0 ? bs : (long long)D * H * W; a.V = V; a.ldv = ldv; a.n = n; a.D = D; a.H = H; a.W = W; a.C = C;
     a.nsum = nsum; a.ss = sum_stride;
-    const long long R = (long long)n * (dn4 ? D / 4 : D) * (H / th) * (W / 2), rows = dn4 ? 6 * R : R;
+    const long long R = (long long)n * (dn4 ? D / 4 : D) * (H / th) * (W / tw), rows = dn4 ? 6 * R : R;
     a.ptv = ptv > 0 ? ptv : rows * ldv;
     a.dM = dM; a.ptm = dM ? R * C : 0;
     FORGE_REQUIRE(rows < (1ll << 31), FORGE_ESHAPE, dn4 ? "%s: more than 2^31 operand rows; split the batch" : "%s: more than 2^31 tiles; split the batch", name);
-    const long long total = R * (dn4 ? C : C / 4), grid = (total + 255) / 256;
+    const int per = kind == IN_DN4HW ? 64 : 256;
+    const long long total = R * (dn4 ? C : C / 4), grid = (total + per - 1) / per;
     FORGE_REQUIRE(grid < (1ll << 31), FORGE_ESHAPE, "%s: grid too large", name);
     const dim3 g((unsigned)grid), b(256);
-    if (kind == IN_DN4H) hipLaunchKernelGGL(wino_input_dn4_kernel<4>, g, b, 0, (hipStream_t)stream, a);
+    if (kind == IN_DN4HW && nsum > 1) hipLaunchKernelGGL(wino_input_dn4hw_kernel<true>, g, dim3(192), 0, (hipStream_t)stream, a);
+    else if (kind == IN_DN4HW) hipLaunchKernelGGL(wino_input_dn4hw_kernel<false>, g, dim3(192), 0, (hipStream_t)stream, a);
+    else if (kind == IN_DN4H) hipLaunchKernelGGL(wino_input_dn4_kernel<4>, g, b, 0, (hipStream_t)stream, a);
     else if (dn4) hipLaunchKernelGGL(wino_input_dn4_kernel<2>, g, b, 0, (hipStream_t)stream, a);
     else if (kind == IN_DY) hipLaunchKernelGGL(wino_input_kernel<true>, g, b, 0, (hipStream_t)stream, a);
     else hipLaunchKernelGGL(wino_input_kernel<false>, g, b, 0, (hipStream_t)stream, a);
@@ -504,6 +681,11 @@
 extern "C" int forge_wino_input_dn4h(const float* in, int ld, long long bs, float* V, int ldv, long long ptv, int n, int D, int H, int W, int C,
                                      int nsum, long long sum_stride, forge_stream_t stream) {
     return wino_input_impl("forge_wino_input_dn4h", IN_DN4H, in, ld, bs, V, ldv, ptv, nullptr, n, D, H, W, C, nsum, sum_stride, stream);
+}
+
+extern "C" int forge_wino_input_dn4hw(const float* in, int ld, long long bs, float* V, int ldv, long long ptv, int n, int D, int H, int W, int C,
+                                      int nsum, long long sum_stride, forge_stream_t stream) {
+    return wino_input_impl("forge_wino_input_dn4hw", IN_DN4HW, in, ld, bs, V, ldv, ptv, nullptr, n, D, H, W, C, nsum, sum_stride, stream);
 }
 
 extern "C" int forge_wino_input_dy(const float* dy, int ld, float* V, float* dM, int n, int D, int H, int W, int C, forge_stream_t stream) {
@@ -588,3 +770,28 @@
     FORGE_LAUNCH_CHECK("forge_wino_output_dn4h");
     return 0;
 }
+
+extern "C" int forge_wino_output_dn4hw(const float* Mm, const float* bias, const float* scale, const float* shift, const float* aux_h, const float* aux_z, float* out,
+                                       float* out2, float* out3, int n, int D, int H, int W, int Cout, int ldo, int epilogue, forge_stream_t stream) {
+    FORGE_REQUIRE(Mm && out && aux_h, FORGE_EINVAL, "forge_wino_output_dn4hw: null pointer argument");
+    FORGE_REQUIRE(n > 0 && D > 0 && H > 0 && W > 0 && H % 4 == 0 && W % 4 == 0, FORGE_EINVAL, "forge_wino_output_dn4hw: n=%d D=%d H=%d W=%d (H, W multiples of 4)", n, D, H, W);
+    FORGE_REQUIRE(Cout > 0 && Cout % 8 == 0 && ldo % 4 == 0, FORGE_ESHAPE, "forge_wino_output_dn4hw: Cout=%d ldo=%d (Cout multiple of 8; ldo of 4)", Cout, ldo);
+    FORGE_REQUIRE(epilogue == W_GRU_GATES || epilogue == W_GRU_OUT, FORGE_EINVAL, "forge_wino_output_dn4hw: epilogue %d is not a GRU tail (2, 3)", epilogue);
+    FORGE_REQUIRE(epilogue == W_GRU_GATES ? ldo == Cout / 2 : ldo >= Cout, FORGE_ESHAPE,
+                  "forge_wino_output_dn4hw: ldo=%d (epilogue 3: ldo >= Cout=%d; epilogue 2: ldo == Cout / 2)", ldo, Cout);
+    FORGE_REQUIRE(epilogue != W_GRU_GATES || out2, FORGE_EINVAL, "forge_wino_output_dn4hw: GRU gate epilogue needs out2");
+    FORGE_REQUIRE(epilogue != W_GRU_OUT || (aux_z && (!out2 || (scale && shift))), FORGE_EINVAL,
+                  "forge_wino_output_dn4hw: GRU out epilogue needs aux_z (and scale/shift with out2)");
+    WinoOutArgs a;
+    const long long R = (long long)n * D * (H / 4) * (W / 4);
+    a.Mm = Mm; a.ptm = R * Cout; a.Mm2 = nullptr; a.bs2 = 0; a.ptm2 = 0; a.bias = bias; a.scale = scale; a.shift = shift; a.slope = 1.f; a.residual = nullptr;
+    a.aux_h = aux_h; a.aux_z = aux_z; a.out = out; a.out2 = out2; a.out3 = out3; a.ldo = ldo; a.n = n; a.D = D; a.H = H; a.W = W; a.Cout = Cout; a.epi = epilogue;
+    FORGE_REQUIRE(R < (1ll << 31), FORGE_ESHAPE, "forge_wino_output_dn4hw: more than 2^31 tiles; split the batch");
+    const long long total = R * (Cout / 4), grid = (total + 127) / 128;
+    FORGE_REQUIRE(grid < (1ll << 31), FORGE_ESHAPE, "forge_wino_output_dn4hw: grid too large");
+    const dim3 g((unsigned)grid), b(256);
+    if (epilogue == W_GRU_GATES) hipLaunchKernelGGL(wino_output_dn4hw_kernel<W_GRU_GATES>, g, b, 0, (hipStream_t)stream, a);
+    else hipLaunchKernelGGL(wino_output_dn4hw_kernel<W_GRU_OUT>, g, b, 0, (hipStream_t)stream, a);
+    FORGE_LAUNCH_CHECK("forge_wino_output_dn4hw");
+    return 0;
+}
diff --git a/forge_amd/flopmeter.py b/forge_amd/flopmeter.py
--- a/forge_amd/flopmeter.py
+++ b/forge_amd/flopmeter.py
@@ -1,7 +1,7 @@
 import torch
 
 from . import _lib
-from .convops import WINO_DN4H, WINO_FORMS
+from .convops import WINO_DN4H, WINO_DN4HW, WINO_FORMS
 
 
 def _v(a):
@@ -59,7 +59,7 @@
     return 2.0 * _v(a[16]) * _v(a[17]) * _v(a[18]) * ((1 if dxn else 0) + (1 if _v(a[10]) else 0))
 
 
-_ENTRIES = {"forge_conv_igemm": _igemm, **{f.gemm: _wino_counter(f) for f in (*WINO_FORMS.values(), WINO_DN4H)}, "forge_conv_wgrad": _wgrad, "forge_wino_wgrad": _wino_wgrad,
+_ENTRIES = {"forge_conv_igemm": _igemm, **{f.gemm: _wino_counter(f) for f in (*WINO_FORMS.values(), WINO_DN4H, WINO_DN4HW)}, "forge_conv_wgrad": _wgrad, "forge_wino_wgrad": _wino_wgrad,
             "forge_attention_fwd": _attention, "forge_attention_fwd_lse": _attention_lse, "forge_attention_bwd": _attention_bwd,
             "forge_attention_mh_fwd": _attention_mh, "forge_attention_mh_bwd": _attention_mh_bwd,
             "forge_token_linear_fwd": _token_fwd, "forge_token_linear_bwd": _token_bwd}
diff --git a/forge_amd/fusion.py b/forge_amd/fusion.py
--- a/forge_amd/fusion.py
+++ b/forge_amd/fusion.py
@@ -199,7 +199,7 @@
 def _step_scratch(R, C, dev, form=None, conv0=None):
     F = co.WINO_FORMS
     P2, P1 = ((form or F["half" if co.wino_half_applies(R, c, C) else "points"]) for c in (2 * C, C))
-    need = [f.P * (R * 2 // f.th) * c for f, c in ((P2, 2 * C), (P1, C))]
+    need = [f.P * (R * 4 // (f.th * f.tw)) * c for f, c in ((P2, 2 * C), (P1, C))]
     if form is not None:
         need.append((conv0 or F["half" if co.wino_half_applies(R, C, C) else "points"]).P * R * C)
     return torch.empty(max(need), dtype=torch.float32, device=dev)
@@ -382,7 +382,7 @@
                   epilogue=co.EPI_AFFINE_ACT)
 
 
-def _wino_step(geo, x, view, views, wg, wo, V, Mm, h, z, hr, hn, out=None, r=None, cand=None, calls=None, th=2):
+def _wino_step(geo, x, view, views, wg, wo, V, Mm, h, z, hr, hn, out=None, r=None, cand=None, calls=None, th=2, tw=2):
     b, D, H, W = geo
     C = h.shape[-1]
     transform, gemm = calls or co.wino_calls(co.WINO_FORMS["points"])
@@ -390,8 +390,8 @@
     def conv(src, U, Cout, i):
         Vs = transform(src, C, C, b, D, H, W, out=V)
         if isinstance(x, tuple):
-            return Vs, gemm(Vs, C, None, 0, U, Mm, b, D, H // th, W // 2, Cout), dict(Mm2=x[i], view=view, views=views)
-        return Vs, gemm(x, C, Vs, C, U, Mm, b, D, H // th, W // 2, Cout, view=view, views=views), {}
+            return Vs, gemm(Vs, C, None, 0, U, Mm, b, D, H // th, W // tw, Cout), dict(Mm2=x[i], view=view, views=views)
+        return Vs, gemm(x, C, Vs, C, U, Mm, b, D, H // th, W // tw, Cout, view=view, views=views), {}
 
     Vh, G, add = conv(h, wg[0], 2 * C, 0)
     co.wino_output(G, wg[1], None, None, 1.0, None, h, None, z, hr, r, *geo, 2 * C, C, co.EPI_GRU_GATES, **add)
@@ -411,9 +411,9 @@
     co.conv_igemm(*ops, *wo, 1.0, res, h, z, hn, out, grid, ig, C, C, taps, epilogue=co.EPI_GRU_OUT, bs1=bs, out3=cand)
 
 
-_WKEY = {None: "_U", co.WINO_FORMS["dn"]: "_Ud", co.WINO_FORMS["dn4"]: "_Ud4", co.WINO_DN4H: "_Ud4h"}
+_WKEY = {None: "_U", co.WINO_FORMS["dn"]: "_Ud", co.WINO_FORMS["dn4"]: "_Ud4", co.WINO_DN4H: "_Ud4h", co.WINO_DN4HW: "_Ud4hw"}
 _PACKS = ((None, ("gate", "out", "fc0", "fc3")), (co.WINO_FORMS["dn"], ("gate", "out", "fc0", "fc3")), (co.WINO_FORMS["dn4"], ("gate", "out")),
-          (co.WINO_DN4H, ("gate", "out")))
+          (co.WINO_DN4H, ("gate", "out")), (co.WINO_DN4HW, ("gate", "out")))
 
 
 def _fuse_eval(gru, xr, groups, wino, split, h0=None, keep=None, const0=None):
@@ -425,12 +425,15 @@
     if wino:
         R = b * D * (H // 2) * (W // 2)
         F = co.WINO_FORMS
-        both = lambda form: H % form.th == 0 and all(form.applies(R * 2 // form.th, D, H // form.th, W // 2, c, 2 * C) for c in (2 * C, C))
+        both = lambda form: H % form.th == 0 and W % form.tw == 0 and all(
+            form.applies(R * 4 // (form.th * form.tw), D, H // form.th, W // form.tw, c, 2 * C) for c in (2 * C, C))
         fits = lambda form: co.wino_fits(b, D, H, W, C, views=t, form=form)
         if not split and keep is None and const0 is None and both(F["dn"]):
             step = F["dn4"] if both(F["dn4"]) and fits(F["dn4"]) else F["dn"]
             if step is F["dn4"] and both(co.WINO_DN4H) and fits(co.WINO_DN4H):
                 step = co.WINO_DN4H
+            if step is co.WINO_DN4H and both(co.WINO_DN4HW) and fits(co.WINO_DN4HW):
+                step = co.WINO_DN4HW
             conv0 = F["dn"] if F["dn"].applies(R, D, H // 2, W // 2, C, C) else None
     p = gru._packed_halves(wino) if (split or const0 is not None) else gru._packed_wino(step) if wino else gru._packed()
     wk = _WKEY[step] if wino else "_w"
@@ -441,8 +444,10 @@
         X = calls[0](xr, C, C, b * t, D, H, W)
         if split:
             X = (_input_products(X, p["gate_Ux"], b * t, geo, 2 * C), _input_products(X, p["out_Ux"], b * t, geo, C))
-        Vs = torch.empty(step.points, int(R * 2 // step.th * step.rows), C, dtype=torch.float32, device=dev) if step else torch.empty(16, R, C, dtype=torch.float32, device=dev)
-        V = Vs.reshape(-1)[:16 * R * C].view(16, R, C)
+        srows = int(R * 4 // (step.th * step.tw) * step.rows) if step else R
+        buf = torch.empty(max(step.points * srows if step else 0, 16 * R) * C, dtype=torch.float32, device=dev)
+        V = buf[:16 * R * C].view(16, R, C)
+        Vs = buf[:step.points * srows * C].view(step.points, srows, C) if step else V
         Mm = _step_scratch(R, C, dev, step, conv0)
     elif split:
         X = {}
@@ -476,7 +481,7 @@
             elif const0 is not None and k == 0:
                 _wino_step(geo, (const0["MXg0"], const0["MXc0"]), 0, 1, *weights("h"), V, Mm, h, z, hr, hn, last, r, cand)
             else:
-                _wino_step(geo, X, ti, t, wg, wo, Vs, Mm, h, z, hr, hn, last, r, cand, calls=calls, th=step.th if step else 2)
+                _wino_step(geo, X, ti, t, wg, wo, Vs, Mm, h, z, hr, hn, last, r, cand, calls=calls, th=step.th if step else 2, tw=step.tw if step else 2)
             if keep is not None:
                 keep += [h, z, r, cand]
             h, hn = hn, h
diff --git a/include/forge_hip.h b/include/forge_hip.h
--- a/include/forge_hip.h
+++ b/include/forge_hip.h
@@ -99,6 +99,13 @@
                          long long pt2, const float* Ud, float* Mm, int n, int D, int Ht, int Wt, int Cout, int kd, forge_stream_t stream);
 int forge_wino_output_dn4h(const float* Mm, const float* bias, const float* scale, const float* shift, const float* aux_h, const float* aux_z, float* out,
                            float* out2, float* out3, int n, int D, int H, int W, int Cout, int ldo, int epilogue, forge_stream_t stream);
+int forge_wino_input_dn4hw(const float* in, int ld, long long bs, float* V, int ldv, long long ptv, int n, int D, int H, int W, int C,
+                           int nsum, long long sum_stride, forge_stream_t stream);
+int forge_wino_weights_dn4hw(const float* wp, float* Ud, int Cout, int Cin, forge_stream_t stream);
+int forge_wino_gemm_dn4hw(const float* V1, int C1, int ld1, long long bs1, long long pt1, const float* V2, int C2, int ld2, long long bs2,
+                          long long pt2, const float* Ud, float* Mm, int n, int D, int Ht, int Wt, int Cout, int kd, forge_stream_t stream);
+int forge_wino_output_dn4hw(const float* Mm, const float* bias, const float* scale, const float* shift, const float* aux_h, const float* aux_z, float* out,
+                            float* out2, float* out3, int n, int D, int H, int W, int Cout, int ldo, int epilogue, forge_stream_t stream);
 int forge_wino_gemm_tile(long long R, int Cout, int Cin);
 int forge_wino_output(const float* Mm, const float* Mm2, long long bs2, long long pt2, const float* bias, const float* scale, const float* shift, float slope, const float* residual,
                       const float* aux_h, const float* aux_z, float* out, float* out2, float* out3, int n, int D, int H, int W, int Cout,
```

New measurement: 1152 views/s (median of 6 runs). 1.07x the previous value.
